# KirillKryukov/naf

Hardware: AMD Instinct MI355X
Metric: unnaf GB/s (uncompressed bases out) on 100 GB synthetic FASTA (higher is better)
Workload: dtype u8; 1 GPU; unnaf decode of a 100.0 GB synthetic-ACGT FASTA archive on one GPU (the size BASELINE.json's metric is quoted on; configs[1] at 10 GB rides along as cfg10_*), 100 records, 80-col lines; archive made in-run by the GPU ennaf; .naf 24739662224 B -> FASTA 99999995684 B, text + archive + decoded text resident in HBM; parallelism=one archive, one GPU, no data-path collective

## Files before the change

### naf_amd/csrc/ctx.h

```cpp
#pragma once
#include "common.h"
#include "../../include/naf_gpu.h"
#include <hip/hip_runtime.h>
#include <stdio.h>
#include <stdarg.h>
#include <vector>
#include <functional>
#include <string>

struct ArenaChunk { u8 *base; size_t cap, used; };

struct KTime { const char *name; hipEvent_t a, b; };

#define ZSPLIT_MAX 8
struct ZSplit { int parts; hipEvent_t ev[ZSPLIT_MAX]; u64 out_end[ZSPLIT_MAX]; int done; void *status; };
struct FlatStream { u64 q0, A; };
#define FLAT_DECODED (~0ull)
struct ZFlat { const u8 *src; const FlatStream *si; u64 nslots; const u8 *sym; void *status; bool ready;
               const u8 *tail; u64 tail_q; u32 tail_n;
               const u8 *cls; u32 n_decoded; u32 n_walk;
               struct naf_gpu_ctx *aux; hipEvent_t decoded_ev; void *later; };
struct CtxOpts { std::vector<std::pair<std::string, std::string>> kv; std::string trace; bool tracing = false; };
struct naf_gpu_ctx {
    int device = 0;
    CtxOpts *opts = nullptr;
    naf_gpu_ctx *root = nullptr;
    hipStream_t stream = nullptr;
    bool own_stream = false;
    std::vector<ArenaChunk> chunks;
    size_t high_water = 0;
    u8 *h_stage = nullptr;
    size_t h_stage_cap = 0;
    void *d_predef = nullptr;
    void *d_seqctab = nullptr;
    char err[512] = {0};
    bool timing = false;
    std::vector<KTime> ktimes;
    std::vector<hipEvent_t> ev_pool;
    size_t ev_used = 0;
    std::vector<std::string> agg_names; std::vector<float> agg_ms; std::vector<int> agg_n;
    float stream_ms[5] = { 0, 0, 0, 0, 0 };
    naf_gpu_ctx *side = nullptr;
    naf_gpu_ctx *side2 = nullptr;
    naf_gpu_ctx *side3 = nullptr;
    naf_gpu_ctx *side4 = nullptr;
    void *sides_thread = nullptr; int sides_rc = 0;
    hipEvent_t fork_ev = nullptr;
    struct ZSplit *zsplit = nullptr;
    hipEvent_t split_ev[ZSPLIT_MAX + 2] = {};
    struct ZFlat *zflat = nullptr;
    void *io_pool = nullptr;
    void *shard_state = nullptr;
    struct HostWorker *worker = nullptr;
};

void ctx_worker_start(naf_gpu_ctx *x, std::function<void()> job);
void ctx_worker_join(naf_gpu_ctx *x);
int  ctx_sides_ready(naf_gpu_ctx *c);

int  ctx_fail(naf_gpu_ctx *c, int code, const char *fmt, ...);
const char *ctx_opt(const naf_gpu_ctx *c, const char *name);
static inline bool ctx_opt_is(const naf_gpu_ctx *c, const char *name, char v) { const char *e = ctx_opt(c, name); return e && e[0] == v; }
bool ctx_tracing(const naf_gpu_ctx *c);
void ctx_trace(naf_gpu_ctx *c, const char *fmt, ...);
#define HIP_TRY(c, call) do { hipError_t e_ = (call); if (e_ != hipSuccess) return ctx_fail((c), NAF_GPU_EHIP, "%s: %s (%s:%d)", #call, hipGetErrorString(e_), __FILE__, __LINE__); } while (0)

void  arena_reset(naf_gpu_ctx *c);
void *arena_alloc(naf_gpu_ctx *c, size_t bytes);
void  arena_settle(naf_gpu_ctx *c);
template <typename T> T *arena_new(naf_gpu_ctx *c, size_t n) { return (T *)arena_alloc(c, n * sizeof(T)); }
static inline std::vector<size_t> arena_mark(const naf_gpu_ctx *c) { std::vector<size_t> m; for (auto &ch : c->chunks) m.push_back(ch.used); return m; }
static inline void arena_release(naf_gpu_ctx *c, const std::vector<size_t> &m) { for (size_t k = 0; k < c->chunks.size(); k++) c->chunks[k].used = k < m.size() ? m[k] : 0; }

int ctx_readback(naf_gpu_ctx *c, void *h_dst, const void *d_src, size_t bytes);
int ctx_readback2(naf_gpu_ctx *c, void *h1, const void *d1, size_t n1, void *h2, const void *d2, size_t n2);
int ctx_readbackv(naf_gpu_ctx *c, int n, void *const *h, const void *const *d, const size_t *bytes);

void ktime_begin(naf_gpu_ctx *c, const char *name);
void ktime_end(naf_gpu_ctx *c);

#define LAUNCH(c, name, kern, grid, block, shmem, ...) do { \
    ktime_begin((c), name); \
    hipLaunchKernelGGL(kern, dim3(grid), dim3(block), (shmem), (c)->stream, __VA_ARGS__); \
    ktime_end((c)); } while (0)

static inline u32 cdiv(u64 a, u64 b) { return (u32)((a + b - 1) / b); }

int scan_exclusive_u64(naf_gpu_ctx *c, u64 *d_vals, size_t n, u64 *d_total);
int scan_inclusive_max_i32(naf_gpu_ctx *c, i32 *d_vals, size_t n);
int scan_inclusive_max_i64(naf_gpu_ctx *c, i64 *d_vals, size_t n);
int scan_exclusive_u64_multi(naf_gpu_ctx *c, u64 *const *arrs, int k, size_t n, u64 *const *totals);
int scan_inclusive_max_i64_multi(naf_gpu_ctx *c, i64 *const *arrs, int k, size_t n);

int zstd_decode(naf_gpu_ctx *c, const u8 *d_src, size_t src_len, int has_magic, u8 *d_dst, size_t dst_cap, size_t *out_len, const u8 *head = nullptr);
int zstd_init_tables(naf_gpu_ctx *c);
void ennaf_shard_state_free(naf_gpu_ctx *c);
void io_pool_free(naf_gpu_ctx *c);
struct EmitP;
int zstd_decode_fused_fasta(naf_gpu_ctx *c, const u8 *d_src, size_t src_len, int has_magic, size_t *out_len, const EmitP *P, u8 *text);
struct ZRange { u64 want_lo, want_hi, got_lo, got_hi; bool ranged; u8 *own_buf; };
int zstd_decode_range(naf_gpu_ctx *c, const u8 *d_src, size_t src_len, int has_magic, u8 *d_dst, size_t dst_cap, size_t *out_len, ZRange *rg, const u8 *head = nullptr);
int zstd_split_status(naf_gpu_ctx *c, const ZSplit *sp);
int zstd_flat_later(naf_gpu_ctx *c, ZFlat *zf);
void zstd_flat_drop(ZFlat *zf);
int zstd_small_batch(naf_gpu_ctx *c, int n, const u8 *const *src, const size_t *len, u8 *const *dst, const size_t *cap, bool *ok);
bool zstd_small_fits(size_t len, size_t cap);
int zstd_small_launch(naf_gpu_ctx *c, int n, const u8 *const *src, const size_t *len, u8 *const *dst, const size_t *cap, u32 **d_res_out);
enum { ZENC_PART = 16, ZENC_PART_FIRST = 32, ZENC_PART_LAST = 64, ZENC_PREFER_RAW = 128, ZENC_PREFER_FLAT = 256, ZENC_SHORT_CODES = 512, ZENC_FRAME_TREE = 1024 };
int zenc_level_window(int level);
int zenc_repeat_probe(naf_gpu_ctx *c, const u8 *d_src, size_t n, u32 *share_1024);
static inline u32 zenc_probe_every(u64 n) { u32 e = 64; while (((n >> 20) / e) > 128) e <<= 1; return e; }
struct ZencPlace { u8 *(*fn)(void *ud, size_t frame_len); void *ud; };
struct ZencJob;
#define ZENC_LOC_BND 20
struct ZencLoc { const u8 *loc; const i32 *blk_bnd; const u32 *blk_t0; u64 tiles; };
int zstd_encode_begin(naf_gpu_ctx *c, const u8 *d_src, size_t n, int level, int with_magic, int lz, int block_log_hint, int window_log, ZencJob **job, const u8 *direct = nullptr, u32 nd = 0, const ZencLoc *dloc = nullptr);
int zstd_encode_finish(naf_gpu_ctx *c, ZencJob *job, u8 *d_dst, size_t cap, size_t *out_len, const ZencPlace *place);
void zstd_encode_drop(ZencJob *job);
int zstd_encode_size(naf_gpu_ctx *c, ZencJob *job, size_t *frame_len);
const u64 *zstd_encode_total_ptr(const ZencJob *job);
void zstd_encode_set_total(ZencJob *job, u64 total);
int zstd_encode(naf_gpu_ctx *c, const u8 *d_src, size_t n, int level, u8 *d_dst, size_t cap, size_t *out_len, int with_magic, int lz = 0, int block_log_hint = 0, int window_log = 0, const ZencPlace *place = nullptr);
```

### naf_amd/csrc/emit.hip

```cpp
#include "ctx.h"
#include "wgscan.h"
#include "emit_core.h"
#include <thread>

__device__ __forceinline__ void st_text16(u8 *p, const uint4 &v, int nt)
{
    if (nt) {
        typedef unsigned int u32x4_t __attribute__((ext_vector_type(4)));
        u32x4_t nv; nv.x = v.x; nv.y = v.y; nv.z = v.z; nv.w = v.w;
        __builtin_nontemporal_store(nv, (u32x4_t *)p);
    } else *(uint4 *)p = v;
}

__global__ void k_len_flags(const u32 *units, u64 n, u64 *flag)
{
    u64 i = (u64)blockIdx.x * blockDim.x + threadIdx.x;
    if (i < n) flag[i] = units[i] != 0xFFFFFFFFu;
}
__global__ void k_len_acc(const u32 *units, u64 n, const u64 *ridx, u64 *rec_len, u64 N)
{
    u64 i = (u64)blockIdx.x * blockDim.x + threadIdx.x;
    if (i < n && ridx[i] < N) atomicAdd((unsigned long long *)&rec_len[ridx[i]], (unsigned long long)units[i]);
}

// ... 407 lines not shown
            if (FOURBIT) { const u8 *s = P.seq + (k.g0 >> 1); a = ld64(s); b = s[8]; }
            else { a = ld64(P.seq + k.g0); b = ld64(P.seq + k.g0 + 8); }
        }
    };
    auto finish = [&](const Chunk &k, u64 a, u64 b) {
        if (!k.live) return;
        u8 *o = out + (k.p0 - P.out_begin);
        if (k.qual_copy) { uint4 v; v.x = (u32)a; v.y = (u32)(a >> 32); v.z = (u32)b; v.w = (u32)(b >> 32); memcpy(o, &v, 16); return; }
        if (k.fast) {
            u64 lo, hi, g0 = k.g0;
            if (FOURBIT) { u64 nib = a; if (g0 & 1) nib = (nib >> 4) | (b << 60); expand16(P.lut, nib, lo, hi); }
            else {
                lo = a; hi = b;
                if (P.upper) {
                    auto up = [](u64 v) { u64 r = 0; for (int i = 0; i < 8; i++) { u32 c = (v >> (8 * i)) & 0xFF; if (c >= 'a' && c <= 'z') c -= 32; r |= (u64)c << (8 * i); } return r; };
                    lo = up(lo); hi = up(hi);
                }
            }
            if (any_toggle) {
                u64 kk = upper_bound_u64(P.toggles, klo, khi, g0);
                u32 state = (u32)(kk & 1), m16 = 0; u64 pos = g0;
                for (;;) {
                    u64 nxt = kk < khi ? P.toggles[kk] : ~0ull;
                    u64 end = nxt < g0 + 16 ? nxt : g0 + 16;
                    if (state && end > pos) m16 |= (u32)(((1u << (end - pos)) - 1) << (pos - g0));
                    if (nxt >= g0 + 16) break;
                    pos = nxt; state ^= 1; kk++;
                }
                lo += spread_bits8(m16 & 0xFF); hi += spread_bits8(m16 >> 8);
            } else if (P.masking && (klo & 1)) { lo += 0x2020202020202020ull; hi += 0x2020202020202020ull; }
            if (k.nl_b < 16) splice_newline(lo, hi, k.nl_b);
            u64 j15 = k.j0 + 15 - (15 > k.nl_b ? 1 : 0);
            if (j15 >= k.len) hi = (hi & 0x00FFFFFFFFFFFFFFull) | ((u64)'\n' << 56);
            uint4 v; v.x = (u32)lo; v.y = (u32)(lo >> 32); v.z = (u32)hi; v.w = (u32)(hi >> 32);
            memcpy(o, &v, 16);
            return;
        }
        for (u32 bb = 0; bb < k.nbytes; bb++) o[bb] = (u8)emit_byte<FOURBIT>(P, k.p0 + bb, rlo, rhi, klo, khi);
    };
    for (u64 tile = span_first; tile <= span_last; tile += 8192) {
        Chunk ka = prep(tile), kb = prep(tile + 4096);
        u64 a0, a1, b0, b1;
        fetch(ka, a0, a1); fetch(kb, b0, b1);
        finish(ka, a0, a1); finish(kb, b0, b1);
    }
}

#define ES_SPAN (32u * 1024u)
#define ES_CAP 1024

__device__ __forceinline__ void place16(u64 &lo, u64 &hi, u64 slo, u64 shi, u32 pos, u32 n)
{
    if (n <= 8) { shi = 0; slo &= low_bytes_mask((int)n); } else if (n < 16) shi &= low_bytes_mask((int)n - 8);
    if (pos == 0) { lo |= slo; hi |= shi; }
    else if (pos < 8) { lo |= slo << (8 * pos); hi |= (shi << (8 * pos)) | (slo >> (64 - 8 * pos)); }
    else if (pos == 8) hi |= slo;
    else hi |= slo << (8 * (pos - 8));
}

__device__ __forceinline__ void mask16_from(const u64 *tog, u32 n, u64 klo, u64 g0, u64 &lo, u64 &hi)
{
    u32 a = 0, b = n;
    while (a < b) { u32 mid = (a + b) >> 1; if (tog[mid] <= g0) a = mid + 1; else b = mid; }
    u32 kk = a, state = (u32)((klo + kk) & 1), m16 = 0; u64 pos = g0;
    for (;;) {
        u64 nxt = kk < n ? tog[kk] : ~0ull;
        u64 end = nxt < g0 + 16 ? nxt : g0 + 16;
        if (state && end > pos) m16 |= (u32)(((1u << (end - pos)) - 1) << (pos - g0));
        if (nxt >= g0 + 16) break;
        pos = nxt; state ^= 1; kk++;
    }
    lo += spread_bits8(m16 & 0xFF); hi += spread_bits8(m16 >> 8);
}
__device__ __forceinline__ void mask16(const EmitP &P, u64 klo, u64 khi, bool any_toggle, u64 g0, u64 &lo, u64 &hi)
{
    if (any_toggle) {
        if (khi - klo <= 0x7FFFFFFFull) mask16_from(P.toggles + klo, (u32)(khi - klo), klo, g0, lo, hi);
        else {
            u64 kk = upper_bound_u64(P.toggles, klo, khi, g0);
            u32 state = (u32)(kk & 1), m16 = 0; u64 pos = g0;
            for (;;) {
                u64 nxt = kk < khi ? P.toggles[kk] : ~0ull;
                u64 end = nxt < g0 + 16 ? nxt : g0 + 16;
                if (state && end > pos) m16 |= (u32)(((1u << (end - pos)) - 1) << (pos - g0));
                if (nxt >= g0 + 16) break;
                pos = nxt; state ^= 1; kk++;
            }
            lo += spread_bits8(m16 & 0xFF); hi += spread_bits8(m16 >> 8);
        }
    } else if (P.masking && (klo & 1)) { lo += 0x2020202020202020ull; hi += 0x2020202020202020ull; }
}

__device__ __forceinline__ void span_windows(const EmitP &P, u64 span_first, u64 span_last, u64 *sh)
{
    if (threadIdx.x < 2 && P.mode != EM_SEQ) {
        u64 p = threadIdx.x == 0 ? span_first : span_last;
        sh[threadIdx.x] = upper_bound_u64(P.rec_out, 0, P.N + 1, p) - 1;
    }
    __syncthreads();
    if (threadIdx.x < 2) {
        u64 k = 0;
        if (P.masking) {
            u64 g;
            if (P.mode == EM_SEQ) g = threadIdx.x == 0 ? span_first : span_last + 1;
            else g = threadIdx.x == 0 ? P.rec_base[sh[0]] : P.rec_base[sh[1] + 1];
            if (P.mode != EM_SEQ && threadIdx.x == 0) {
                u64 r = sh[0], off = span_first - P.rec_out[r], hl = P.hdr_len[r];
                if (off > hl) { u64 q = off - hl; u64 j = (P.mode == EM_FASTA && P.L) ? (q / (P.L + 1)) * P.L : (P.mode == EM_FASTQ ? 0 : q); if (j > P.rec_len[r]) j = P.rec_len[r]; g += j; }
            }
            k = upper_bound_u64(P.toggles, 0, P.n_toggles, g);
        }
        sh[2 + threadIdx.x] = k;
    }
    __syncthreads();
}

__global__ void k_hdr_len64(const u32 *hdr_len, u64 r0, u64 n, u64 *out)
{
    u64 i = (u64)blockIdx.x * blockDim.x + threadIdx.x;
    if (i < n) out[i] = hdr_len[r0 + i];
}
__device__ __forceinline__ void store_upto16(u8 *p, u64 lo, u64 hi, u32 n)
{
    if (n >= 16) { uint4 v; v.x = (u32)lo; v.y = (u32)(lo >> 32); v.z = (u32)hi; v.w = (u32)(hi >> 32); memcpy(p, &v, 16); return; }
    if (n & 8) { st64(p, lo); p += 8; lo = hi; }
    if (n & 4) { st32(p, (u32)lo); p += 4; lo >>= 32; }
    if (n & 2) { p[0] = (u8)lo; p[1] = (u8)(lo >> 8); p += 2; lo >>= 16; }
    if (n & 1) p[0] = (u8)lo;
}
template <u32 LANES = 16>
__device__ __forceinline__ void group_copy(u8 *dst, const u8 *src, u64 n, u32 g)
{
    for (u64 i = (u64)g * 16; i < n; i += LANES * 16) {
        u64 lo = ld64(src + i), hi = ld64(src + i + 8);
        store_upto16(dst + i, lo, hi, n - i < 16 ? (u32)(n - i) : 16u);
    }
}

__global__ __launch_bounds__(256) void k_hdr_build(EmitP P, u64 r0, u64 n, const u64 *hdr_off, u8 *text)
{
    u64 i = (u64)blockIdx.x * 32 + (threadIdx.x >> 3);
    u32 g = threadIdx.x & 7;
    if (i >= n) return;
    u64 r = r0 + i; u32 hl = P.hdr_len[r];
    u8 *o = text + hdr_off[i];
    u64 ids0 = 0, idl = 0, nm0 = 0, nml = 0;
    if (P.has_ids) { ids0 = r ? P.idz[r - 1] + 1 : 0; idl = P.idz[r] - ids0; }
    if (P.has_names) { nm0 = r ? P.nmz[r - 1] + 1 : 0; nml = P.nmz[r] - nm0; }
    if (g == 0) { o[0] = P.hdr_char; o[hl - 1] = '\n'; }
    if (P.has_ids) {
        group_copy<8>(o + 1, P.ids + ids0, idl, g);
        if (P.has_names && nml) { if (g == 0) o[1 + idl] = P.sep; group_copy<8>(o + 2 + idl, P.names + nm0, nml, g); }
    } else group_copy<8>(o + 1, P.names + nm0, nml, g);
}

template <bool FOURBIT, typename Geo>
__device__ __forceinline__ void compose_chunk(const EmitP &P, Geo &geo, u64 p0, u32 nbytes, u64 r, u64 klo, u64 khi, bool any_toggle, u32 Lp1_32, u8 *o)
{
    const bool hdrs = P.hdr_text != nullptr;
    u64 ro, rn, len, base, ho; u32 hl;
    geo(r, ro, rn, len, base, ho, hl);
    u64 lo = 0, hi = 0; u32 pos = 0;
    while (pos < nbytes) {
        u64 p = p0 + pos;
        while (p >= rn) { r++; geo(r, ro, rn, len, base, ho, hl); }
        u64 off = p - ro;
        const u8 *src = nullptr; u64 g = 0; bool is_bases = false;
        u64 n_main = 0; u32 tc = 0, n_tc = 0;
        if (off < hl) { src = P.hdr_text + ho + off; n_main = hl - off; }
        else {
            u64 q = off - hl;
            if (P.mode == EM_FASTQ) {
                if (q < len + 3) {
                    u64 skip = 0;
                    if (q < len) { is_bases = true; g = base + q; n_main = len - q; } else skip = q - len;
                    tc = 0x0A2B0Au >> (8 * (u32)skip); n_tc = 3 - (u32)skip;
                } else { src = P.qual + base + (q - len - 3); n_main = 2 * len + 3 - q; tc = '\n'; n_tc = 1; }
            } else {
                tc = '\n'; n_tc = 1;
                if (P.mode == EM_SEQUENCES || P.L == 0) { if (q < len) { is_bases = true; g = base + q; n_main = len - q; } }
                else {
                    u64 line, col;
                    if (Lp1_32 && (q >> 32) == 0) { u32 l32 = (u32)q / Lp1_32; line = l32; col = (u32)q - l32 * Lp1_32; }
                    else { line = q / (P.L + 1); col = q - line * (P.L + 1); }
                    u64 j = line * P.L + col;
                    if (col != P.L && j < len) { is_bases = true; g = base + j; n_main = len - j < P.L - col ? len - j : P.L - col; }
                }
            }
        }
        u32 rem = nbytes - pos;
        u32 n1 = n_main < rem ? (u32)n_main : rem;
        if (n1) {
            u64 slo, shi;
            if (is_bases) { bases16<FOURBIT>(P, g, slo, shi); if (P.mode != EM_FASTQ) mask16(P, klo, khi, any_toggle, g, slo, shi); }
            else if (!hdrs && off < hl) {
                slo = shi = 0;
                for (u32 b = 0; b < n1; b++) { u64 ch = header_char(P, r, off + b, hl); if (b < 8) slo |= ch << (8 * b); else shi |= ch << (8 * (b - 8)); }
            }
            else { slo = ld64(src); shi = n1 > 8 ? ld64(src + 8) : 0; }
            place16(lo, hi, slo, shi, pos, n1);
            pos += n1; rem -= n1;
        }
        if (n1 == n_main && rem && n_tc) { u32 n2 = n_tc < rem ? n_tc : rem; place16(lo, hi, tc, 0, pos, n2); pos += n2; }
    }
    if (nbytes == 16) { uint4 v; v.x = (u32)lo; v.y = (u32)(lo >> 32); v.z = (u32)hi; v.w = (u32)(hi >> 32); memcpy(o, &v, 16); }
    else for (u32 b = 0; b < nbytes; b++) o[b] = (u8)((b < 8 ? lo >> (8 * b) : hi >> (8 * (b - 8))) & 0xFF);
}

struct GeoGlobal {
    const EmitP &P;
    __device__ GeoGlobal(const EmitP &p) : P(p) {}
    __device__ __forceinline__ void operator()(u64 r, u64 &ro, u64 &rn, u64 &len, u64 &base, u64 &ho, u32 &hl) const
    { ro = P.rec_out[r]; rn = P.rec_out[r + 1]; len = P.rec_len[r]; base = P.rec_base[r]; hl = P.hdr_len[r]; ho = P.hdr_text ? P.hdr_off[r - P.hdr_r0] : 0; }
};

template <bool FOURBIT>
__global__ __launch_bounds__(256) void k_emit_short(EmitP P, u8 *out)
{
    __shared__ u64 sh[4];
    __shared__ u64 s_ro[ES_CAP + 1], s_len[ES_CAP], s_base[ES_CAP], s_ho[ES_CAP];
    __shared__ u32 s_hl[ES_CAP];
    u64 span_first = P.out_begin + (u64)blockIdx.x * ES_SPAN, span_last = span_first + ES_SPAN - 1;
    if (span_last >= P.out_end) span_last = P.out_end - 1;
    span_windows(P, span_first, span_last, sh);
    const u64 rlo = sh[0], rhi = sh[1], klo = sh[2], khi = sh[3];
    const bool any_toggle = P.masking && klo < khi;
    const u64 nrec = rhi - rlo + 1;
    const bool in_lds = nrec <= ES_CAP;
    const bool hdrs = P.hdr_text != nullptr;
    if (in_lds) {
        for (u32 i = threadIdx.x; i < (u32)nrec; i += 256) {
            u64 r = rlo + i; s_ro[i] = P.rec_out[r]; s_len[i] = P.rec_len[r]; s_base[i] = P.rec_base[r]; s_hl[i] = P.hdr_len[r];
            s_ho[i] = hdrs ? P.hdr_off[r - P.hdr_r0] : 0;
        }
        if (threadIdx.x == 0) s_ro[nrec] = P.rec_out[rhi + 1];
        __syncthreads();
    }
    const u32 Lp1_32 = (P.L + 1) >> 32 ? 0 : (u32)(P.L + 1);
    auto geo_lds = [&](u64 r, u64 &ro, u64 &rn, u64 &len, u64 &base, u64 &ho, u32 &hl) {
        u32 i = (u32)(r - rlo); ro = s_ro[i]; rn = s_ro[i + 1]; len = s_len[i]; base = s_base[i]; hl = s_hl[i]; ho = s_ho[i];
    };
    GeoGlobal geo_g(P);
    for (u64 tile = span_first; tile <= span_last; tile += 4096) {
        u64 p0 = tile + (u64)threadIdx.x * 16;
        if (p0 > span_last) continue;
        u32 nbytes = P.out_end - p0 < 16 ? (u32)(P.out_end - p0) : 16;
        u8 *o = out + (p0 - P.out_begin);
        if (in_lds) {
            u32 lo_ = 0, hi_ = (u32)nrec; while (lo_ < hi_) { u32 mid = (lo_ + hi_) >> 1; if (s_ro[mid] <= p0) lo_ = mid + 1; else hi_ = mid; }
            compose_chunk<FOURBIT>(P, geo_lds, p0, nbytes, rlo + lo_ - 1, klo, khi, any_toggle, Lp1_32, o);
        } else {
            u64 r = upper_bound_u64(P.rec_out, rlo, rhi + 1, p0) - 1;
            compose_chunk<FOURBIT>(P, geo_g, p0, nbytes, r, klo, khi, any_toggle, Lp1_32, o);
        }
    }
}

#define ER_STAGE 24576u
template <bool FOURBIT, u32 ER_LANES, u32 WGT>
__global__ __launch_bounds__(WGT) void k_emit_fastq_records(EmitP P, u8 *out)
{
    constexpr u32 ER_READS = WGT / ER_LANES, STAGE = ER_STAGE / (256u / WGT);
    __shared__ __attribute__((aligned(16))) u8 stage[STAGE + 32];
    const u32 g = threadIdx.x & (ER_LANES - 1);
    const u64 r0 = (u64)blockIdx.x * ER_READS, r = r0 + threadIdx.x / ER_LANES;
    const u64 rend = r0 + ER_READS < P.N ? r0 + ER_READS : P.N;
    const u64 wbase = P.rec_out[r0], wspan = P.rec_out[rend] - wbase;
    const bool in_lds = wspan <= STAGE;
    if (r < P.N) {
        const u64 len = P.rec_len[r], base = P.rec_base[r];
        const u32 hl = P.hdr_len[r];
        u8 *o = in_lds ? stage + (P.rec_out[r] - wbase) : out + P.rec_out[r];
        u64 ids0 = 0, idl = 0, nm0 = 0, nml = 0;
        if (P.has_ids) { ids0 = r ? P.idz[r - 1] + 1 : 0; idl = P.idz[r] - ids0; }
        if (P.has_names) { nm0 = r ? P.nmz[r - 1] + 1 : 0; nml = P.nmz[r] - nm0; }
        if (g == 0) { o[0] = P.hdr_char; o[hl - 1] = '\n'; }
        if (P.has_ids) {
            group_copy<ER_LANES>(o + 1, P.ids + ids0, idl, g);
            if (P.has_names && nml) { if (g == 0) o[1 + idl] = P.sep; group_copy<ER_LANES>(o + 2 + idl, P.names + nm0, nml, g); }
        } else group_copy<ER_LANES>(o + 1, P.names + nm0, nml, g);
        u8 *os = o + hl;
        for (u64 i = (u64)g * 16; i < len; i += 16 * ER_LANES) {
            u64 lo, hi; bases16<FOURBIT>(P, base + i, lo, hi);
            store_upto16(os + i, lo, hi, len - i < 16 ? (u32)(len - i) : 16u);
        }
        if (g == 0) { os[len] = '\n'; os[len + 1] = '+'; os[len + 2] = '\n'; os[2 * len + 3] = '\n'; }
        group_copy<ER_LANES>(os + len + 3, P.qual + base, len, g);
    }
    if (!in_lds) return;
    __syncthreads();
    u8 *dst = out + wbase; const u32 n = (u32)wspan;
    u32 head = (u32)((16 - ((uintptr_t)dst & 15)) & 15); if (head > n) head = n;
    if (threadIdx.x < head) dst[threadIdx.x] = stage[threadIdx.x];
    u32 words = (n - head) >> 4;
    for (u32 w = threadIdx.x; w < words; w += WGT) {
        u64 a, b2; __builtin_memcpy(&a, stage + head + 16 * w, 8); __builtin_memcpy(&b2, stage + head + 16 * w + 8, 8);
        uint4 v; v.x = (u32)a; v.y = (u32)(a >> 32); v.z = (u32)b2; v.w = (u32)(b2 >> 32);
        st_text16(dst + head + 16 * w, v, P.nt_store);
    }
    for (u32 k = head + 16 * words + threadIdx.x; k < n; k += WGT) dst[k] = stage[k];
}

#define EMIT_TOG_LDS 256u
struct TileIdx { u64 gline, k, khi; u32 col, fast; };
#define TI_HDR 0xFFFFFFFFu
struct TileFlat { u64 q0, A, q1, A1, q2, qf; };
struct TileFlatE { u64 base, a1_addr; u32 a1_sh, K0, K1, d1, d2, qoff, par0, pad; };
static_assert(sizeof(TileFlatE) == sizeof(TileFlat), "the derived record replaces the raw one in place");
#define FLAT_QM 4096
#define TILE_WG 255
__global__ __launch_bounds__(256) void k_tile_index(EmitP P, u64 ntiles, TileIdx *ti, u64 *tr, u32 *list, u32 *count, TileFlat *tsig, u32 spare, u32 *list2)
{
    __shared__ u64 s_k[256], s_r[256];
    const u64 t = (u64)blockIdx.x * TILE_WG + threadIdx.x;
    const u64 p = P.out_begin + t * 4096;
    TileIdx x; x.fast = 0; x.gline = 0; x.khi = 0; x.k = P.n_toggles; x.col = TI_HDR;
    TileFlat f; f.q0 = f.A = f.q1 = f.A1 = f.q2 = f.qf = 0;
    u64 r = ~0ull; u32 cbits = 1;
    const bool inside = t < ntiles && p < P.out_end;
    if (inside) {
        u64 g;
        if (P.mode == EM_SEQ) { r = 0; x.col = 0; g = p; x.gline = p; }
        else {
            r = upper_bound_u64(P.rec_out, 0, P.N + 1, p) - 1;
            u64 off = p - P.rec_out[r], hl = P.hdr_len[r], len = P.rec_len[r], j = 0;
            if (off >= hl) {
                u64 q = off - hl;
                if (P.mode == EM_FASTA && P.L) {
                    u64 line = q / (P.L + 1), col = q - line * (P.L + 1);
                    j = line * P.L + (col < P.L ? col : P.L);
                    if (P.L < 0xFFFFFFF0ull) { x.gline = P.rec_base[r] + line * P.L; x.col = (u32)col; }
                } else if (P.mode != EM_FASTQ) { j = q; x.col = 0; x.gline = P.rec_base[r] + q; }
                if (j > len) j = len;
            }
            g = P.rec_base[r] + j;
        }
        x.k = P.masking ? upper_bound_u64(P.toggles, 0, P.n_toggles, g) : 0;
        if (tsig) {
            const FlatStream *si = (const FlatStream *)P.fsi;
            const u64 q = g >> 1;
            u64 lo, hi, gs = q >> 13; if (gs >= P.fslots) gs = P.fslots - 1;
            if (si[gs].q0 <= q) { lo = gs; hi = gs + 1; u64 st = 1; while (hi < P.fslots && si[hi].q0 <= q) { lo = hi; st <<= 1; hi = lo + st; } if (hi > P.fslots) hi = P.fslots; }
            else { hi = gs; u64 st = 1; lo = gs - 1; while (lo > 0 && si[lo].q0 > q) { hi = lo; st <<= 1; lo = lo > st ? lo - st : 0; } }
            while (hi - lo > 1) { const u64 mid = (lo + hi) >> 1; if (si[mid].q0 <= q) lo = mid; else hi = mid; }
            f.q0 = si[lo].q0; f.A = si[lo].A; f.qf = q;
            if (P.fcls) {
                u32 c = 3; u64 b = lo >> 2; const u64 nb = P.fslots >> 2, qe = q + 2048 + 16;
                for (u32 k = 0; k < 6 && b < nb && si[4 * b].q0 <= qe; k++, b++) c &= P.fcls[b];
                if (b < nb && si[4 * b].q0 <= qe) c = 0;
                cbits = c;
            }
            u64 cs = lo + 1;
            while (cs < P.fslots && si[cs + 1].q0 == si[cs].q0) cs++;
            f.q1 = si[cs].q0; f.A1 = cs < P.fslots ? si[cs].A : 0;
            u64 ce = cs < P.fslots ? cs + 1 : cs;
            while (ce < P.fslots && si[ce + 1].q0 == si[ce].q0) ce++;
            f.q2 = si[ce].q0;
        }
    }
    s_k[threadIdx.x] = x.k; s_r[threadIdx.x] = r;
    __syncthreads();
    if (threadIdx.x == TILE_WG) return;
    TileFlatE e; e.base = (u64)P.fsrc; e.a1_addr = (u64)P.fsrc; e.a1_sh = 4; e.K0 = e.K1 = 0; e.d1 = e.d2 = 0x7FFFFFFFu; e.qoff = 0; e.par0 = 0; e.pad = 0;
    if (t >= ntiles) {
        if (t == ntiles) { tr[t] = ~0ull; ti[t] = x; if (tsig && spare) *(TileFlatE *)&tsig[t] = e; }
        else if (tsig && t < ntiles + spare) { ti[t].fast = 0; *(TileFlatE *)&tsig[t] = e; }
        return;
    }
    tr[t] = r;
    if (!inside) { ti[t] = x; if (tsig) *(TileFlatE *)&tsig[t] = e; list[atomicAdd(count, 1u)] = (u32)t; return; }
    const u64 r_next = s_r[threadIdx.x + 1];
    x.khi = s_k[threadIdx.x + 1];
    const bool wrap = P.mode == EM_FASTA && P.L != 0;
    bool fast = x.col != TI_HDR && r == r_next && P.out_begin + (t + 1) * 4096 <= P.out_end && !P.force_slow && (!wrap || P.L >= 16);
    bool packed = false;
    if (tsig) {
        packed = fast && (cbits & 2);
        if (fast && !(cbits & 1)) fast = false;
        if (fast) {
            fast = f.qf + 2048 + 16 < f.q2 || f.q2 == f.q1;
            if (P.ftail && f.qf + 2048 + 16 >= P.ftail_q) fast = false;
            if (f.q2 != f.q1 && (f.A1 > f.A ? f.A1 - f.A : f.A - f.A1) >= (1ull << 29)) fast = false;
        }
        if (fast) {
            const u64 gline = x.gline;
            const u64 dd1 = f.q1 - f.qf, dd2 = f.q2 - f.qf;
            e.d1 = dd1 > 0x7FFFFFFFull ? 0x7FFFFFFFu : (u32)dd1; e.d2 = dd2 > 0x7FFFFFFFull ? 0x7FFFFFFFu : (u32)dd2;
            const u64 T0 = f.A - 4 * (f.qf - f.q0), T1 = f.A1 + 4 * (u64)e.d1;
            const bool two = f.q2 != f.q1;
            const u64 tmin = two && T1 < T0 ? T1 : T0;
            const u64 ub = (tmin - 40 - 4 * (u64)FLAT_QM) & ~7ull;
            e.base = (u64)P.fsrc + (u64)((i64)ub >> 3);
            e.K0 = (u32)(T0 - 40 - ub); e.K1 = two ? (u32)(T1 - 40 - ub) : e.K0;
            e.qoff = (u32)((gline >> 1) - f.qf); e.par0 = (u32)gline & 1u;
            const u64 t1 = (f.A1 < 40 ? 40 : f.A1) - 40;
            e.a1_addr = (u64)P.fsrc + (t1 >> 3); e.a1_sh = (u32)(t1 & 7) + 4;
        }
        *(TileFlatE *)&tsig[t] = e;
    }
    x.fast = fast ? 1u : (packed ? 2u : 0u);
    ti[t] = x;
    if (!fast) { if (packed) list2[atomicAdd(count + 1, 1u)] = (u32)t; else list[atomicAdd(count, 1u)] = (u32)t; }
}

template <bool FOURBIT>
__device__ __forceinline__ void emit_tile_body(const EmitP &P, const TileIdx &a, u8 *out_tile)
{
    __shared__ u64 s_tog[EMIT_TOG_LDS];
    const u32 ntog = (u32)(a.khi - a.k < EMIT_TOG_LDS ? a.khi - a.k : EMIT_TOG_LDS);
    const bool use_tog = P.masking && a.k < a.khi && a.khi - a.k <= EMIT_TOG_LDS;
    if (use_tog) { for (u32 i = threadIdx.x; i < ntog; i += 256) s_tog[i] = P.toggles[a.k + i]; __syncthreads(); }
    const u32 lane16 = threadIdx.x * 16;
    u64 g0; u32 nl_b = 64;
    if (P.mode == EM_FASTA && P.L != 0) {
        const u32 Lp1 = (u32)P.L + 1;
        u32 c = a.col + lane16, dl;
        if (Lp1 < 32768) dl = __umulhi(c, P.Ldiv_magic); else dl = c >= Lp1 ? 1u : 0u;
        u32 col = c - dl * Lp1;
        g0 = a.gline + (u64)dl * (u32)P.L + col;
        u32 d = (u32)P.L - col;
        nl_b = d < 16 ? d : 64;
    } else g0 = a.gline + lane16;
    u64 lo, hi;
    if (FOURBIT) {
        u64 addr = (u64)P.seq + (g0 >> 1);
        const uint4 q = ldg_at<uint4>(addr & ~7ull);
        u64 q0 = (u64)q.x | ((u64)q.y << 32), q1 = (u64)q.z | ((u64)q.w << 32);
        u32 sh = (u32)(addr & 7) * 8 + (u32)(g0 & 1) * 4;
        expand16(P.lut, sh ? (q0 >> sh) | (q1 << (64 - sh)) : q0, lo, hi);
    } else bases16<false>(P, g0, lo, hi);
    if (use_tog) mask16_from(s_tog, ntog, a.k, g0, lo, hi);
    else mask16(P, a.k, a.khi, P.masking && a.k < a.khi, g0, lo, hi);
    if (nl_b < 16) splice_newline(lo, hi, (int)nl_b);
    uint4 v; v.x = (u32)lo; v.y = (u32)(lo >> 32); v.z = (u32)hi; v.w = (u32)(hi >> 32);
    st_text16(out_tile + lane16, v, P.nt_store);
}
template <bool FOURBIT>
__global__ __launch_bounds__(256) void k_emit_tile(EmitP P, const TileIdx *ti, u8 *out)
{
    const TileIdx a = ti[blockIdx.x];
    if (a.fast != 1) return;
    emit_tile_body<FOURBIT>(P, a, out + (u64)blockIdx.x * 4096);
}
template <bool FOURBIT, u32 TW>
__device__ __forceinline__ void emit_tiles_wave(const EmitP &P, const TileIdx *ti, u8 *out, const u64 (&tn)[TW], u32 want, u64 (*s_tog)[EMIT_TOG_LDS])
{
    const u32 lane = threadIdx.x;
    TileIdx A[TW]; bool live[TW];
#pragma unroll
    for (u32 j = 0; j < TW; j++) { A[j] = ti[tn[j] == ~0ull ? 0 : tn[j]]; live[j] = tn[j] != ~0ull && A[j].fast == want; }
    u64 g0s[TW][4]; u32 nls[TW][4]; uint4 Q[TW][4];
#pragma unroll
    for (u32 j = 0; j < TW; j++) {
        const TileIdx &a = A[j];
#pragma unroll
        for (u32 r = 0; r < 4; r++) {
            const u32 lane16 = (r * 64 + lane) * 16;
            u64 g0; u32 nl_b = 64;
            if (P.mode == EM_FASTA && P.L != 0) {
                const u32 Lp1 = (u32)P.L + 1;
                u32 c = a.col + lane16, dl;
                if (Lp1 < 32768) dl = __umulhi(c, P.Ldiv_magic); else dl = c >= Lp1 ? 1u : 0u;
                u32 col = c - dl * Lp1;
                g0 = a.gline + (u64)dl * (u32)P.L + col;
                u32 d = (u32)P.L - col;
                nl_b = d < 16 ? d : 64;
            } else g0 = a.gline + lane16;
            g0s[j][r] = g0; nls[j][r] = nl_b;
            if (FOURBIT) Q[j][r] = live[j] ? ldg_at<uint4>(((u64)P.seq + (g0 >> 1)) & ~7ull) : make_uint4(0, 0, 0, 0);
        }
    }
    if (P.masking) {
#pragma unroll
        for (u32 j = 0; j < TW; j++) {
            const u64 nt = A[j].khi - A[j].k;
            for (u32 i = lane; i < EMIT_TOG_LDS; i += 64) s_tog[j][i] = (live[j] && i < nt && nt <= EMIT_TOG_LDS) ? P.toggles[A[j].k + i] : 0ull;
        }
        __syncthreads();
    }
#pragma unroll
    for (u32 j = 0; j < TW; j++) {
        if (!live[j]) continue;
        const TileIdx &a = A[j];
        const u32 ntog = (u32)(a.khi - a.k < EMIT_TOG_LDS ? a.khi - a.k : EMIT_TOG_LDS);
        const bool use_tog = P.masking && a.k < a.khi && a.khi - a.k <= EMIT_TOG_LDS;
#pragma unroll
        for (u32 r = 0; r < 4; r++) {
            const u64 g0 = g0s[j][r];
            u64 lo, hi;
            if (FOURBIT) {
                const u64 addr = (u64)P.seq + (g0 >> 1);
                const uint4 q = Q[j][r];
                const u64 q0 = (u64)q.x | ((u64)q.y << 32), q1 = (u64)q.z | ((u64)q.w << 32);
                const u32 sh = (u32)(addr & 7) * 8 + (u32)(g0 & 1) * 4;
                expand16(P.lut, sh ? (q0 >> sh) | (q1 << (64 - sh)) : q0, lo, hi);
            } else bases16<false>(P, g0, lo, hi);
            if (use_tog) mask16_from(s_tog[j], ntog, a.k, g0, lo, hi);
            else mask16(P, a.k, a.khi, P.masking && a.k < a.khi, g0, lo, hi);
            if (nls[j][r] < 16) splice_newline(lo, hi, (int)nls[j][r]);
            uint4 v; v.x = (u32)lo; v.y = (u32)(lo >> 32); v.z = (u32)hi; v.w = (u32)(hi >> 32);
            st_text16(out + tn[j] * 4096 + (r * 64 + lane) * 16, v, P.nt_store);
        }
    }
}
template <bool FOURBIT, u32 TW>
__global__ __launch_bounds__(64) void k_emit_tile_wave(EmitP P, const TileIdx *ti, u8 *out, u64 ntiles)
{
    __shared__ u64 s_tog[TW][EMIT_TOG_LDS];
    u64 tn[TW];
#pragma unroll
    for (u32 j = 0; j < TW; j++) { const u64 t = (u64)blockIdx.x * TW + j; tn[j] = t < ntiles ? t : ~0ull; }
    emit_tiles_wave<FOURBIT, TW>(P, ti, out, tn, 1u, s_tog);
}
template <bool FOURBIT>
__global__ __launch_bounds__(64) void k_emit_tile_list_wave(EmitP P, const TileIdx *ti, const u32 *list, const u32 *count, u8 *out)
{
    __shared__ u64 s_tog[1][EMIT_TOG_LDS];
    const u32 n = *count;
    for (u32 i = blockIdx.x; i < n; i += gridDim.x) {
        const u64 tn[1] = { list[i] };
        emit_tiles_wave<FOURBIT, 1>(P, ti, out, tn, 2u, s_tog);
        __syncthreads();
    }
}
template <bool FOURBIT>
__global__ __launch_bounds__(256) void k_emit_tile_list(EmitP P, const TileIdx *ti, const u32 *list, const u32 *count, u8 *out)
{
    const u32 n = *count;
    for (u32 i = blockIdx.x; i < n; i += gridDim.x) {
        const u32 t = list[i];
        const TileIdx a = ti[t];
        emit_tile_body<FOURBIT>(P, a, out + (u64)t * 4096);
        __syncthreads();
    }
}

__global__ void k_flat_pair(EmitP P, u32 *pair)
{
    const u32 t = threadIdx.x;
    {
        const u32 pa = P.fsym[t >> 4], pb = P.fsym[t & 15];
        pair[16 + t] = expand_codes4(P.lut, (pa & 15u) | ((pa >> 4) << 8) | ((pb & 15u) << 16) | ((pb >> 4) << 24));
        if (t < 16) {
            const u32 d = t; u32 sel[4], orv[4];
            for (u32 i = 0; i < 4; i++) {
                sel[i] = 0; orv[i] = 0;
                for (u32 j = 0; j < 4; j++) { const u32 q = 4 * i + j; sel[i] |= (q < d ? 4 + j : (q == d ? 0x0Cu : 3 + j)) << (8 * j); if (q == d) orv[i] |= 0x0Au << (8 * j); }
            }
            for (u32 i = 0; i < 4; i++) { pair[272 + 8 * d + i] = sel[i]; pair[272 + 8 * d + 4 + i] = orv[i]; }
        }
    }
    if (t >= 12) return;
    const u8 *lut = (const u8 *)P.lut;
    u32 v = 0;
    for (u32 k = 0; k < 4; k++) {
        const u32 pk = P.fsym[4 * (t & 3) + k];
        const u32 b = t < 4 ? pk : (t < 8 ? lut[pk & 15] : lut[pk >> 4]);
        v |= b << (8 * k);
    }
    pair[t] = v;
}
#define FLAT_TPW 8
template <u32 TPW>
__global__ __launch_bounds__(256) void k_emit_tile_flat(EmitP P, const TileIdx *ti, const TileFlat *tsig, u8 *out, u64 ntiles, u32 xcd_chunk)
{
    u32 wg = blockIdx.x;
    if (xcd_chunk) { wg = (blockIdx.x & 7u) * xcd_chunk + (blockIdx.x >> 3); if ((u64)wg * TPW >= ntiles) return; }
    __shared__ u64 s_tog[TPW][EMIT_TOG_LDS];
    __shared__ uint4 s_spl[32];
    if (threadIdx.x < 16) {
        const u32 d = threadIdx.x; u32 sel[4], orv[4];
        for (u32 i = 0; i < 4; i++) {
            sel[i] = 0; orv[i] = 0;
            for (u32 j = 0; j < 4; j++) { const u32 p = 4 * i + j; sel[i] |= (p < d ? 4 + j : (p == d ? 0x0Cu : 3 + j)) << (8 * j); if (p == d) orv[i] |= 0x0Au << (8 * j); }
        }
        s_spl[2 * d] = make_uint4(sel[0], sel[1], sel[2], sel[3]); s_spl[2 * d + 1] = make_uint4(orv[0], orv[1], orv[2], orv[3]);
    }
    __shared__ u32 s_pair[256];
    {
        const u32 pa = P.fsym[threadIdx.x >> 4], pb = P.fsym[threadIdx.x & 15];
        s_pair[threadIdx.x] = expand_codes4(P.lut, (pa & 15u) | ((pa >> 4) << 8) | ((pb & 15u) << 16) | ((pb >> 4) << 24));
    }
    const u32 lane16 = threadIdx.x * 16;
    TileIdx A[TPW]; TileFlatE F[TPW]; bool live[TPW];
    {
        static_assert(sizeof(TileIdx) == 32 && sizeof(TileFlatE) == 48, "records are read as 16-byte words");
        const u64 t0 = (u64)wg * TPW;
        const uint4 *pa = (const uint4 *)(ti + t0), *pf = (const uint4 *)(tsig + t0);
        uint4 ra[2 * TPW], rf[3 * TPW];
#pragma unroll
        for (u32 i = 0; i < 2 * TPW; i++) ra[i] = pa[i];
#pragma unroll
        for (u32 i = 0; i < 3 * TPW; i++) rf[i] = pf[i];
#pragma unroll
        for (u32 j = 0; j < TPW; j++) {
            __builtin_memcpy(&A[j], &ra[2 * j], 32); __builtin_memcpy(&F[j], &rf[3 * j], 48);
            live[j] = t0 + j < ntiles && A[j].fast == 1;
        }
    }
    u64 X[TPW]; u32 offs[TPW], grels[TPW], nls[TPW], haves[TPW];
#pragma unroll
    for (u32 j = 0; j < TPW; j++) {
        const TileIdx &a = A[j]; const TileFlatE &e = F[j];
        u32 grel, nl_b = 64;
        if (P.mode == EM_FASTA && P.L != 0) {
            const u32 Lp1 = (u32)P.L + 1;
            u32 c = a.col + lane16, dl;
            if (Lp1 < 32768) dl = __umulhi(c, P.Ldiv_magic); else dl = c >= Lp1 ? 1u : 0u;
            u32 col = c - dl * Lp1;
            grel = dl * (u32)P.L + col;
            u32 d = (u32)P.L - col;
            nl_b = d < 16 ? d : 64;
        } else grel = lane16;
        grels[j] = grel; nls[j] = nl_b;
        const u32 par = e.par0 + grel;
        const u32 need = 8 + (par & 1u);
        const u32 qrel = (par >> 1) + e.qoff;
        const bool second = qrel >= e.d1;
        const u32 qm = live[j] ? ~0u : 0u;
        const u32 off = (second ? e.K1 : e.K0) - ((4 * qrel) & qm);
        const u32 rem = (second ? e.d2 : e.d1) - qrel;
        X[j] = ldg_at_unaligned<u64>(e.base + (off >> 3));
        offs[j] = off;
        haves[j] = need > rem ? rem : 16u;
    }
    if (P.masking) {
        u64 tg[TPW];
#pragma unroll
        for (u32 j = 0; j < TPW; j++) {
            const u64 nt = A[j].khi - A[j].k;
            tg[j] = (live[j] && threadIdx.x < nt && nt <= EMIT_TOG_LDS) ? P.toggles[A[j].k + threadIdx.x] : 0ull;
        }
#pragma unroll
        for (u32 j = 0; j < TPW; j++) s_tog[j][threadIdx.x] = tg[j];
    }
    __syncthreads();
#pragma unroll
    for (u32 j = 0; j < TPW; j++) {
        const u64 t = (u64)wg * TPW + j;
        if (!live[j]) continue;
        const TileIdx &a = A[j];
        const u64 g0 = a.gline + grels[j];
        u64 h36 = X[j] >> ((offs[j] & 7) + 4);
        if (haves[j] < 9) {
            const u64 y = ldg_at_unaligned<u64>(F[j].a1_addr);
            const u64 n36 = (y >> F[j].a1_sh) & 0xFFFFFFFFFull;
            const u32 keep = 4 * haves[j];
            h36 = (h36 & ~(0xFFFFFFFFFull >> keep)) | (n36 >> keep);
        }
        const u32 h = (u32)(h36 >> 4), n9 = (u32)h36 & 15u;
        u64 lo, hi;
        {
            u32 w0 = s_pair[h >> 24], w1 = s_pair[(h >> 16) & 0xFFu], w2 = s_pair[(h >> 8) & 0xFFu], w3 = s_pair[h & 0xFFu];
            if (g0 & 1) {
                const u32 c9 = s_pair[n9 << 4];
                w0 = __builtin_amdgcn_alignbyte(w1, w0, 1); w1 = __builtin_amdgcn_alignbyte(w2, w1, 1);
                w2 = __builtin_amdgcn_alignbyte(w3, w2, 1); w3 = __builtin_amdgcn_alignbyte(c9, w3, 1);
            }
            lo = (u64)w0 | ((u64)w1 << 32); hi = (u64)w2 | ((u64)w3 << 32);
        }
        const u32 ntog = (u32)(a.khi - a.k < EMIT_TOG_LDS ? a.khi - a.k : EMIT_TOG_LDS);
        const bool use_tog = P.masking && a.k < a.khi && a.khi - a.k <= EMIT_TOG_LDS;
        if (use_tog) mask16_from(s_tog[j], ntog, a.k, g0, lo, hi);
        else mask16(P, a.k, a.khi, P.masking && a.k < a.khi, g0, lo, hi);
        uint4 v; v.x = (u32)lo; v.y = (u32)(lo >> 32); v.z = (u32)hi; v.w = (u32)(hi >> 32);
        if (nls[j] < 16) {
            const uint4 sel = s_spl[2 * nls[j]], orv = s_spl[2 * nls[j] + 1];
            const u32 x0 = v.x, x1 = v.y, x2 = v.z, x3 = v.w;
            v.x = __builtin_amdgcn_perm(x0, 0u, sel.x) | orv.x; v.y = __builtin_amdgcn_perm(x1, x0, sel.y) | orv.y;
            v.z = __builtin_amdgcn_perm(x2, x1, sel.z) | orv.z; v.w = __builtin_amdgcn_perm(x3, x2, sel.w) | orv.w;
        }
        st_text16(out + t * 4096 + lane16, v, P.nt_store);
    }
}

template <u32 TW>
__global__ __launch_bounds__(64) void k_emit_tile_flat_wave(EmitP P, const TileIdx *ti, const TileFlat *tsig, u8 *out, u64 ntiles, u32 xcd_chunk)
{
    u32 wg = blockIdx.x;
    if (xcd_chunk) { wg = (blockIdx.x & 7u) * xcd_chunk + (blockIdx.x >> 3); if ((u64)wg * TW >= ntiles) return; }
    __shared__ u64 s_tog[TW][EMIT_TOG_LDS];
    __shared__ uint4 s_spl[32];
    __shared__ u32 s_pair[256];
    const u32 lane = threadIdx.x;
    if (lane < 32) s_spl[lane] = ((const uint4 *)(P.fpair + 272))[lane];
    ((uint4 *)s_pair)[lane] = ((const uint4 *)(P.fpair + 16))[lane];
    TileIdx A[TW]; TileFlatE F[TW]; bool live[TW];
    {
        const u64 t0 = (u64)wg * TW;
        const uint4 *pa = (const uint4 *)(ti + t0), *pf = (const uint4 *)(tsig + t0);
        uint4 ra[2 * TW], rf[3 * TW];
#pragma unroll
        for (u32 i = 0; i < 2 * TW; i++) ra[i] = pa[i];
#pragma unroll
        for (u32 i = 0; i < 3 * TW; i++) rf[i] = pf[i];
#pragma unroll
        for (u32 j = 0; j < TW; j++) {
            __builtin_memcpy(&A[j], &ra[2 * j], 32); __builtin_memcpy(&F[j], &rf[3 * j], 48);
            live[j] = t0 + j < ntiles && A[j].fast == 1;
        }
    }
    u64 X[TW][4]; u32 grels[TW][4], pk[TW][4];
#pragma unroll
    for (u32 j = 0; j < TW; j++) {
        const TileIdx &a = A[j]; const TileFlatE &e = F[j];
#pragma unroll
        for (u32 r = 0; r < 4; r++) {
            const u32 lane16 = (r * 64 + lane) * 16;
            u32 grel, nl_b = 64;
            if (P.mode == EM_FASTA && P.L != 0) {
                const u32 Lp1 = (u32)P.L + 1;
                u32 c = a.col + lane16, dl;
                if (Lp1 < 32768) dl = __umulhi(c, P.Ldiv_magic); else dl = c >= Lp1 ? 1u : 0u;
                u32 col = c - dl * Lp1;
                grel = dl * (u32)P.L + col;
                u32 d = (u32)P.L - col;
                nl_b = d < 16 ? d : 64;
            } else grel = lane16;
            grels[j][r] = grel;
            const u32 par = e.par0 + grel;
            const u32 need = 8 + (par & 1u);
            const u32 qrel = (par >> 1) + e.qoff;
            const bool second = qrel >= e.d1;
            const u32 qm = live[j] ? ~0u : 0u;
            const u32 off = (second ? e.K1 : e.K0) - ((4 * qrel) & qm);
            const u32 rem = (second ? e.d2 : e.d1) - qrel;
            X[j][r] = ldg_at_unaligned<u64>(e.base + (off >> 3));
            pk[j][r] = nl_b | ((need > rem ? rem : 16u) << 8) | ((off & 7u) << 16);
        }
    }
    if (P.masking) {
#pragma unroll
        for (u32 j = 0; j < TW; j++) {
            const u64 nt = A[j].khi - A[j].k;
            for (u32 i = lane; i < EMIT_TOG_LDS; i += 64) s_tog[j][i] = (live[j] && i < nt && nt <= EMIT_TOG_LDS) ? P.toggles[A[j].k + i] : 0ull;
        }
    }
    __syncthreads();
#pragma unroll
    for (u32 j = 0; j < TW; j++) {
        const u64 t = (u64)wg * TW + j;
        if (!live[j]) continue;
        const TileIdx &a = A[j];
        const u32 ntog = (u32)(a.khi - a.k < EMIT_TOG_LDS ? a.khi - a.k : EMIT_TOG_LDS);
        const bool use_tog = P.masking && a.k < a.khi && a.khi - a.k <= EMIT_TOG_LDS;
#pragma unroll
        for (u32 r = 0; r < 4; r++) {
            const u64 g0 = a.gline + grels[j][r];
            const u32 nl = pk[j][r] & 0xFFu, have = (pk[j][r] >> 8) & 0xFFu;
            u64 h36 = X[j][r] >> ((pk[j][r] >> 16) + 4);
            if (have < 9) {
                const u64 y = ldg_at_unaligned<u64>(F[j].a1_addr);
                const u64 n36 = (y >> F[j].a1_sh) & 0xFFFFFFFFFull;
                const u32 keep = 4 * have;
                h36 = (h36 & ~(0xFFFFFFFFFull >> keep)) | (n36 >> keep);
            }
            const u32 h = (u32)(h36 >> 4), n9 = (u32)h36 & 15u;
            u64 lo, hi;
            {
                u32 w0 = s_pair[h >> 24], w1 = s_pair[(h >> 16) & 0xFFu], w2 = s_pair[(h >> 8) & 0xFFu], w3 = s_pair[h & 0xFFu];
                if (g0 & 1) {
                    const u32 c9 = s_pair[n9 << 4];
                    w0 = __builtin_amdgcn_alignbyte(w1, w0, 1); w1 = __builtin_amdgcn_alignbyte(w2, w1, 1);
                    w2 = __builtin_amdgcn_alignbyte(w3, w2, 1); w3 = __builtin_amdgcn_alignbyte(c9, w3, 1);
                }
                lo = (u64)w0 | ((u64)w1 << 32); hi = (u64)w2 | ((u64)w3 << 32);
            }
            if (use_tog) mask16_from(s_tog[j], ntog, a.k, g0, lo, hi);
            else mask16(P, a.k, a.khi, P.masking && a.k < a.khi, g0, lo, hi);
            uint4 v; v.x = (u32)lo; v.y = (u32)(lo >> 32); v.z = (u32)hi; v.w = (u32)(hi >> 32);
            if (nl < 16) {
                const uint4 sel = s_spl[2 * nl], orv = s_spl[2 * nl + 1];
                const u32 x0 = v.x, x1 = v.y, x2 = v.z, x3 = v.w;
                v.x = __builtin_amdgcn_perm(x0, 0u, sel.x) | orv.x; v.y = __builtin_amdgcn_perm(x1, x0, sel.y) | orv.y;
                v.z = __builtin_amdgcn_perm(x2, x1, sel.z) | orv.z; v.w = __builtin_amdgcn_perm(x3, x2, sel.w) | orv.w;
            }
            st_text16(out + t * 4096 + (r * 64 + lane) * 16, v, P.nt_store);
        }
    }
}

template <bool FOURBIT>
__device__ __forceinline__ void emit_rest_tile(const EmitP &P, const TileIdx *ti, const u64 *tr, u64 t, u8 *out, u32 chunk)
{
    const TileIdx a = ti[t];
    u64 p0 = P.out_begin + t * 4096 + chunk * 16;
    if (p0 >= P.out_end) return;
    u32 nbytes = P.out_end - p0 < 16 ? (u32)(P.out_end - p0) : 16;
    const u32 Lp1_32 = (P.L + 1) >> 32 ? 0 : (u32)(P.L + 1);
    u8 *o = out + (p0 - P.out_begin);
    if (P.mode == EM_SEQ) {
        for (u32 bb = 0; bb < nbytes; bb++) o[bb] = (u8)emit_byte<FOURBIT>(P, p0 + bb, 0, 0, a.k, a.khi);
        return;
    }
    u64 rlo = tr[t], rhi = tr[t + 1] == ~0ull ? P.N - 1 : tr[t + 1];
    u64 r = upper_bound_u64(P.rec_out, rlo, rhi + 1, p0) - 1;
    GeoGlobal geo_g(P);
    compose_chunk<FOURBIT>(P, geo_g, p0, nbytes, r, a.k, a.khi, P.masking && a.k < a.khi, Lp1_32, o);
}
#define EMIT_REST_GRID 4096
template <bool FOURBIT>
__global__ __launch_bounds__(64) void k_emit_rest(EmitP P, const TileIdx *ti, const u64 *tr, const u32 *list, const u32 *count, u8 *out)
{
    const u32 n = *count;
    for (u32 i = blockIdx.x; i < 4 * n; i += gridDim.x) emit_rest_tile<FOURBIT>(P, ti, tr, list[i >> 2], out, (i & 3) * 64 + threadIdx.x);
}

__global__ void k_range_bases(EmitP P, u64 *out2)
{
    if (threadIdx.x || blockIdx.x) return;
    if (P.mode == EM_SEQ) { out2[0] = P.out_begin; out2[1] = P.out_end; out2[2] = out2[3] = 0; return; }
    u64 pb = P.out_begin, pe = P.out_end - 1;
    u64 r0 = upper_bound_u64(P.rec_out, 0, P.N + 1, pb) - 1, r1 = upper_bound_u64(P.rec_out, 0, P.N + 1, pe) - 1;
    out2[2] = r0; out2[3] = r1;
    auto lower = [&](u64 r, u64 p) -> u64 {
        u64 off = p - P.rec_out[r], hl = P.hdr_len[r], len = P.rec_len[r];
        if (off <= hl) return 0;
        u64 q = off - hl, j;
        if (P.mode == EM_FASTQ) j = 0;
        else if (P.mode == EM_FASTA && P.L) j = (q / (P.L + 1)) * P.L;
        else j = q;
        return j > len ? len : j;
    };
    auto upper = [&](u64 r, u64 p) -> u64 {
        u64 off = p - P.rec_out[r], hl = P.hdr_len[r], len = P.rec_len[r];
        if (off < hl) return 0;
        u64 q = off - hl, j;
        if (P.mode == EM_FASTQ) j = len;
        else if (P.mode == EM_FASTA && P.L) j = (q / (P.L + 1) + 1) * P.L;
        else j = q + 1;
        return j > len ? len : j;
    };
    out2[0] = P.rec_base[r0] + lower(r0, pb);
    out2[1] = P.rec_base[r1] + upper(r1, pe);
}

__global__ void k_last_nonempty(const u64 *rec_len, u64 N, unsigned long long *out)
{
    u64 r = (u64)blockIdx.x * blockDim.x + threadIdx.x;
    if (r < N && rec_len[r]) atomicMax(out, (unsigned long long)(r + 1));
}
template <bool FOURBIT>
__global__ void k_emit_surplus(EmitP P, u64 base0, u64 S, u64 cc, u64 L, int wrap, u64 lo, u64 hi, u8 *out)
{
    const u64 j = lo + (u64)blockIdx.x * blockDim.x + threadIdx.x;
    if (j >= hi) return;
    u64 g; bool nl = false;
    if (!wrap || L == 0 || S <= cc) g = base0 + j;
    else if (j < cc) g = base0 + j;
    else if (j == cc) { nl = true; g = 0; }
    else { const u64 j2 = j - cc - 1, line = j2 / (L + 1), col = j2 - line * (L + 1); if (col == L) { nl = true; g = 0; } else g = base0 + cc + line * L + col; }
    u32 ch = '\n';
    if (!nl) { ch = base_char<FOURBIT>(P, g); if (P.masking && base_masked(P, g, 0, P.n_toggles)) ch += 32; }
    out[j - lo] = (u8)ch;
}

static int zero_positions(naf_gpu_ctx *c, const u8 *d_buf, u64 n, u64 N, u64 **out, bool names)
{
    u64 *pos = arena_new<u64>(c, N + 1);
    if (!pos) return NAF_GPU_ENOMEM;
    u64 tiles = (n + ZT_TILE - 1) / ZT_TILE;
    u64 *cnt = arena_new<u64>(c, tiles + 2);
    if (!cnt) return NAF_GPU_ENOMEM;
    u64 *d_total = cnt + tiles + 1;
    if (tiles) LAUNCH(c, "unnaf_zero_count", k_zero_count, tiles, 256, 0, d_buf, n, cnt);
    int rc = scan_exclusive_u64(c, cnt, tiles, d_total); if (rc) return rc;
    u64 total = 0;
    rc = ctx_readback(c, &total, d_total, 8); if (rc) return rc;
    if (total < N) return ctx_fail(c, NAF_GPU_EFORMAT, names ? "corrupted names - can't read name %llu\n" : "currupted ids - can't read id %llu\n", (unsigned long long)total);
    if (tiles) LAUNCH(c, "unnaf_zero_scatter", k_zero_scatter, tiles, 256, 0, d_buf, n, (const u64 *)cnt, pos, N);
    *out = pos;
    return 0;
}

enum { H_OK = 0, H_EMPTY, H_TRUNC, H_MAGIC, H_VERSION, H_SEQTYPE, H_SEPARATOR, H_VLE_LEAD, H_VLE_OVERFLOW, H_SANE_SECTION , H_SANE_COUNT = H_SANE_SECTION + 6 };
struct ContainerOut { naf_gpu_header h; int code; u8 frame_head[6][24]; };
NAF_HD int naf_parse_container(const u8 *p, size_t len, naf_gpu_header *h)
{
    size_t pos = 0;
    memset(h, 0, sizeof *h);
    if (len == 0) return H_EMPTY;
    if (len < 3) return H_TRUNC;
    if (p[0] != 0x01 || p[1] != 0xF9 || p[2] != 0xEC) return H_MAGIC;
    pos = 3;
    if (pos >= len) return H_TRUNC;
    h->version = p[pos++];
    if (h->version < 1 || h->version > 2) return H_VERSION;
    h->seq_type = NAF_SEQ_DNA;
    if (h->version > 1) {
        if (pos >= len) return H_TRUNC;
        int t = p[pos++];
        h->seq_type = t;
        if (t < 1 || t > 3) return H_SEQTYPE;
    }
    if (len - pos < 2) return H_TRUNC;
    h->flags = p[pos++]; h->separator = p[pos++];
    if (h->separator < 0x20 || h->separator > 0x7E) return H_SEPARATOR;
    int e = 0;
    auto rd = [&](u64 *v) -> int {
        u64 a = 0; if (pos >= len) return H_TRUNC;
        u8 ch = p[pos++];
        if (ch == 128) return H_VLE_LEAD;
        while (ch & 128) { if (a & (127ull << 57)) return H_VLE_OVERFLOW; a = (a << 7) | (ch & 127); if (pos >= len) return H_TRUNC; ch = p[pos++]; }
        if (a & (127ull << 57)) return H_VLE_OVERFLOW;
        *v = (a << 7) | ch; return 0;
    };
    if ((e = rd(&h->line_length)) || (e = rd(&h->n_sequences))) return e;
    if (h->flags & 0x40) { if ((e = rd(&h->title_len))) return e; h->title_off = pos; if (h->title_len > len - pos) return H_TRUNC; pos += h->title_len; }
    const int bit[6] = { 0x20, 0x10, 0x08, 0x04, 0x02, 0x01 };
    for (int i = 0; i < 6; i++) {
        if (!(h->flags & bit[i])) continue;
        if ((e = rd(&h->orig_size[i])) || (e = rd(&h->comp_size[i]))) return e;
        if (h->comp_size[i] > len - pos) return H_TRUNC;
        h->payload_off[i] = pos; pos += h->comp_size[i];
    }
    for (int i = 0; i < 6; i++) {
        const u64 cs = h->comp_size[i] + 4;
        const u64 lim = cs > (1ull << 46) ? ~0ull : cs << (i == 4 ? 17 : 16);
        if (h->orig_size[i] > lim) return H_SANE_SECTION + i;
    }
    if (h->n_sequences > ((u64)len << 16)) return H_SANE_COUNT;
    return H_OK;
}
static void container_error_text(int code, const naf_gpu_header *h, char *buf, size_t cap)
{
    static const char *what[6] = { "can't decompress ids\n", "can't decompress names\n", "can't decompress lengths\n", "can't decompress mask\n",
                                   "can't decompress sequence\n", "can't decompress quality\n" };
    switch (code) {
    case H_EMPTY: snprintf(buf, cap, "empty input"); break;
    case H_TRUNC: snprintf(buf, cap, "incomplete or truncated input\n"); break;
    case H_MAGIC: snprintf(buf, cap, "not a NAF format\n"); break;
    case H_VERSION: snprintf(buf, cap, "unknown version (%d) of NAF format\n", h->version); break;
    case H_SEQTYPE: snprintf(buf, cap, "unknown sequence type (%d) found in NAF file\n", h->seq_type); break;
    case H_SEPARATOR: snprintf(buf, cap, "unsupported name separator character\n"); break;
    case H_VLE_LEAD: snprintf(buf, cap, "invalid input: error parsing variable length encoded number\n"); break;
    case H_VLE_OVERFLOW: snprintf(buf, cap, "invalid input: overflow reading a variable length encoded number\n"); break;
    case H_SANE_COUNT: snprintf(buf, cap, "corrupted header: more sequences than the archive can describe\n"); break;
    default: if (code >= H_SANE_SECTION && code < H_SANE_SECTION + 6) snprintf(buf, cap, "%s", what[code - H_SANE_SECTION]); else snprintf(buf, cap, "malformed NAF header\n");
    }
}

extern "C" int naf_gpu_parse_header_host(const void *h_naf, size_t len, naf_gpu_header *h, char errbuf[128])
{
    if (!h) return NAF_GPU_EARG;
    const int code = naf_parse_container((const u8 *)h_naf, len, h);
    if (!code) return 0;
    if (errbuf) container_error_text(code, h, errbuf, 128);
    return NAF_GPU_EFORMAT;
}

__global__ void k_parse_container(const u8 *d, u64 len, ContainerOut *out)
{
    if (threadIdx.x || blockIdx.x) return;
    out->code = naf_parse_container(d, (size_t)len, &out->h);
    for (int i = 0; i < 6; i++) {
        const u64 n = out->code ? 0 : (out->h.comp_size[i] < 24 ? out->h.comp_size[i] : 24);
        for (u64 k = 0; k < 24; k++) out->frame_head[i][k] = k < n ? d[out->h.payload_off[i] + k] : 0;
    }
}

static int parse_container_device(naf_gpu_ctx *c, const void *d_naf, size_t len, ContainerOut *co)
{
    ContainerOut *d_co = arena_new<ContainerOut>(c, 1); if (!d_co) return NAF_GPU_ENOMEM;
    LAUNCH(c, "unnaf_parse_container", k_parse_container, 1, 64, 0, (const u8 *)d_naf, (u64)len, d_co);
    int rc = ctx_readback(c, co, d_co, sizeof *co); if (rc) return rc;
    if (co->code) { char buf[160]; container_error_text(co->code, &co->h, buf, sizeof buf); return ctx_fail(c, NAF_GPU_EFORMAT, "%s", buf); }
    return 0;
}

extern "C" int naf_gpu_parse_header(naf_gpu_ctx *c, const void *d_naf, size_t len, naf_gpu_header *h)
{
    if (!c || !h) return NAF_GPU_EARG;
    arena_reset(c);
    ContainerOut co;
    int rc = parse_container_device(c, d_naf, len, &co);
    *h = co.h;
    return rc;
}

enum { S_IDS = 0, S_NAMES, S_LEN, S_MASK, S_SEQ, S_QUAL };

struct UnnafPlan {
    naf_gpu_header h; u8 frame_head[6][24]; EmitP P; u64 total; bool fourbit; bool empty;
    u64 seq_bytes; bool need_qual;
    u64 main_total, surplus, sur_c, sur_base0;
};

static int load_section(naf_gpu_ctx *c, const u8 *d_naf, const naf_gpu_header &h, int i, u64 expect, const char *what, u8 **out, const u8 *head = nullptr)
{
    u8 *buf = (u8 *)arena_alloc(c, expect + 32);
    if (!buf) return NAF_GPU_ENOMEM;
    size_t n = 0;
    int rc = zstd_decode(c, d_naf + h.payload_off[i], h.comp_size[i], 0, buf, expect, &n, head);
    if (rc == NAF_GPU_ECAP || (rc == 0 && n != expect)) return ctx_fail(c, NAF_GPU_EFORMAT, "can't decompress %s\n", what);
    if (rc) return rc;
    *out = buf;
    return 0;
}

static int unnaf_prepare(naf_gpu_ctx *c, const u8 *d_naf, size_t naf_len, const naf_gpu_unnaf_opts *o, UnnafPlan &pl)
{
    ContainerOut co;
    int rc = parse_container_device(c, d_naf, naf_len, &co); if (rc) return rc;
    pl.h = co.h; memcpy(pl.frame_head, co.frame_head, sizeof pl.frame_head);
    const naf_gpu_header &h = pl.h;
    EmitP &P = pl.P; memset(&P, 0, sizeof P);
    int has_mask = (h.flags >> 2) & 1, has_data = (h.flags >> 1) & 1, has_qual = h.flags & 1;
    int mode = o->out_type == NAF_OUT_DEFAULT ? (has_qual ? NAF_OUT_FASTQ : NAF_OUT_FASTA) : o->out_type;
    pl.empty = false; pl.total = 0; pl.need_qual = false; pl.main_total = pl.surplus = pl.sur_c = pl.sur_base0 = 0;
    pl.fourbit = h.seq_type <= NAF_SEQ_RNA;
    u64 N = h.n_sequences, T = h.orig_size[S_SEQ];
    pl.seq_bytes = pl.fourbit ? (T + 1) / 2 : T;
    if (N == 0 || !has_data) { pl.empty = true; return 0; }
    if (mode == NAF_OUT_FASTQ && !has_qual) return ctx_fail(c, NAF_GPU_EFORMAT, "FASTQ output requested, but input has no qualities\n");
    if (mode == NAF_OUT_4BIT) {
        if (!pl.fourbit) return ctx_fail(c, NAF_GPU_EFORMAT, "input has no 4-bit encoded data, but %s sequences\n", h.seq_type == NAF_SEQ_PROTEIN ? "protein" : "text");
        P.mode = -1; pl.total = pl.main_total = pl.seq_bytes; return 0;
    }
    P.mode = mode == NAF_OUT_FASTA ? EM_FASTA : mode == NAF_OUT_FASTQ ? EM_FASTQ : mode == NAF_OUT_SEQ ? EM_SEQ : EM_SEQUENCES;
    P.N = N; P.T = T;
    P.L = o->line_length >= 0 ? (u64)o->line_length : h.line_length;
    P.sep = h.separator; P.hdr_char = P.mode == EM_FASTQ ? '@' : '>';
    P.masking = o->use_mask && has_mask && P.mode != EM_FASTQ && pl.fourbit;
    P.upper = !pl.fourbit && !o->use_mask;
    const char *tab = h.seq_type == NAF_SEQ_RNA ? "-UGKCYSBAWRDMHVN" : "-TGKCYSBAWRDMHVN";
    memcpy(P.lut, tab, 16);
    for (u32 k = 0; k < 16; k++) ((u8 *)P.lutc)[k] = (u8)tab[((k & 1) << 3) | ((k & 2) << 1) | ((k & 4) >> 1) | (k >> 3)];
    const char *fs = ctx_opt(c, "FORCE_SLOW"); P.force_slow = fs && fs[0] == '1';
    P.nt_store = 1;
    pl.need_qual = P.mode == EM_FASTQ;

    return 0;
}

template <typename Hook>
static int unnaf_sections_main(naf_gpu_ctx *c, const u8 *d_naf, UnnafPlan &pl, naf_gpu_ctx *aux, Hook early, bool early_has_work, naf_gpu_ctx *aux_names)
{
    const naf_gpu_header &h = pl.h;
    EmitP &P = pl.P;
    int has_ids = (h.flags >> 5) & 1, has_names = (h.flags >> 4) & 1, has_len = (h.flags >> 3) & 1;
    u64 N = h.n_sequences, T = h.orig_size[S_SEQ];
    int rc;
    if (P.mode == EM_SEQ) {
        pl.total = pl.main_total = T;
    } else {
        if (!has_len) return ctx_fail(c, NAF_GPU_EFORMAT, "archive has no lengths");
        P.has_ids = 0; P.has_names = 0;
        const bool want_names = P.mode == EM_FASTA || P.mode == EM_FASTQ;
        if (want_names) { P.has_ids = has_ids; P.has_names = has_names; }
        u8 *pre[3] = { nullptr, nullptr, nullptr };
        auto small3 = [&](naf_gpu_ctx *x) -> int {
            const int sec[3] = { S_IDS, S_NAMES, S_LEN }; const bool wanted[3] = { want_names && has_ids != 0, want_names && has_names != 0, true };
            const u8 *src[3]; size_t len[3], cap[3]; u8 *dst[3]; bool ok[3]; int idx[3], m = 0;
            for (int k = 0; k < 3; k++) {
                if (!wanted[k] || h.orig_size[sec[k]] == 0) continue;
                u8 *b = (u8 *)arena_alloc(x, h.orig_size[sec[k]] + 32); if (!b) return NAF_GPU_ENOMEM;
                src[m] = d_naf + h.payload_off[sec[k]]; len[m] = h.comp_size[sec[k]]; dst[m] = b; cap[m] = h.orig_size[sec[k]]; idx[m++] = k;
            }
            if (!m) return 0;
            int r = zstd_small_batch(x, m, src, len, dst, cap, ok); if (r) return r;
            for (int q = 0; q < m; q++) if (ok[q]) pre[idx[q]] = dst[q];
            return 0;
        };
        auto ids_names = [&](naf_gpu_ctx *x, int which = 3) -> int {
            int r;
            if ((which & 1) && want_names && has_ids) {
                u8 *b = pre[0]; u64 *z = nullptr;
                if (h.orig_size[S_IDS] == 0) return ctx_fail(x, NAF_GPU_EFORMAT, "corrupted ids - not 0-terminated\n");
                if (!b && (r = load_section(x, d_naf, h, S_IDS, h.orig_size[S_IDS], "ids", &b, pl.frame_head[S_IDS]))) return r;
                if ((r = zero_positions(x, b, h.orig_size[S_IDS], N, &z, false))) return r;
                P.ids = b; P.idz = z;
            }
            if ((which & 2) && want_names && has_names) {
                u8 *b = pre[1]; u64 *z = nullptr;
                if (h.orig_size[S_NAMES] == 0) return ctx_fail(x, NAF_GPU_EFORMAT, "corrupted names - not 0-terminated\n");
                if (!b && (r = load_section(x, d_naf, h, S_NAMES, h.orig_size[S_NAMES], "names", &b, pl.frame_head[S_NAMES]))) return r;
                if ((r = zero_positions(x, b, h.orig_size[S_NAMES], N, &z, true))) return r;
                P.names = b; P.nmz = z;
            }
            return 0;
        };
        u64 *rec_len = nullptr;
// ... 37 lines not shown
                    J.res = d_res; J.n_jobs = (u32)m;
                    J.ids = buf[0]; J.ids_n = h.orig_size[S_IDS]; J.names = buf[1]; J.names_n = h.orig_size[S_NAMES];
                    J.lens = (const u32 *)buf[2]; J.n_len = h.orig_size[S_LEN] / 4;
                    J.N = N; J.L = P.L; J.has_ids = P.has_ids; J.has_names = P.has_names; J.mode = P.mode;
                    J.idz = P.has_ids ? arena_new<u64>(x, N + 1) : nullptr; J.nmz = P.has_names ? arena_new<u64>(x, N + 1) : nullptr;
                    J.rec_len = arena_new<u64>(x, N + 1); J.hdr_len = arena_new<u32>(x, N + 1);
                    J.rec_out = arena_new<u64>(x, N + 2); J.rec_base = arena_new<u64>(x, N + 2); J.status = arena_new<u64>(x, 8);
                    if ((P.has_ids && !J.idz) || (P.has_names && !J.nmz) || !J.rec_len || !J.hdr_len || !J.rec_out || !J.rec_base || !J.status) return NAF_GPU_ENOMEM;
                    LAUNCH(x, "unnaf_side_tables", k_side_tables, 1, 256, 0, J);
                    if ((r = ctx_readback(x, st, J.status, sizeof st))) return r;
                    if (st[0] != 1) return 0;
                    P.ids = buf[0]; P.idz = J.idz; P.names = buf[1]; P.nmz = J.nmz;
                    P.rec_len = J.rec_len; P.hdr_len = J.hdr_len; P.rec_out = J.rec_out; P.rec_base = J.rec_base;
                    fused_done = true;
                    return 0;
                };
                int rf = 0;
                if (aux) { ctx_worker_start(aux, [&] { rf = fused(aux); }); early(); ctx_worker_join(aux); if (rf) memcpy(c->err, aux->err, sizeof c->err); }
                else rf = fused(c);
                if (rf) return rf;
                if (fused_done) {
                    if (st[3] < N) return ctx_fail(c, NAF_GPU_EFORMAT, "corrupted lengths: %llu records described, %llu expected", (unsigned long long)st[3], (unsigned long long)N);
                    if (P.has_ids && st[1] < N) return ctx_fail(c, NAF_GPU_EFORMAT, "currupted ids - can't read id %llu\n", (unsigned long long)st[1]);
                    if (P.has_names && st[2] < N) return ctx_fail(c, NAF_GPU_EFORMAT, "corrupted names - can't read name %llu\n", (unsigned long long)st[2]);
                    tot[0] = st[4]; tot[1] = st[5];
                }
            }
        }
        if (fused_done) rec_len = (u64 *)P.rec_len;
        else {
        const bool aux_run = aux && want_names && (has_ids || has_names);
        int rc_aux = 0, rc_len = 0;
        const bool len_on_aux = aux_run && early_has_work;
        int rc_small = 0;
        if (aux_run && !len_on_aux) rc_small = small3(c);
        bool names_beside = aux_run && aux_names && !len_on_aux && has_ids && has_names && h.orig_size[S_IDS] >= (1u << 20) && h.orig_size[S_NAMES] >= (1u << 20);
        { const char *nb = ctx_opt(c, "NAMES_BESIDE"); if (nb && nb[0] == '0') names_beside = false; }
        int rc_names = 0;
        if (names_beside) ctx_worker_start(aux_names, [&] { rc_names = ids_names(aux_names, 2); });
        if (aux_run) ctx_worker_start(aux, [&] { if (len_on_aux) rc_small = small3(aux); rc_aux = rc_small ? rc_small : ids_names(aux, names_beside ? 1 : 3); if (len_on_aux && !rc_small) rc_len = lengths(aux); });
        early();
        if (!aux_run) rc_small = small3(c);
        if (!len_on_aux) rc_len = rc_small ? rc_small : lengths(c);
        if (aux_run) { ctx_worker_join(aux); hipStreamSynchronize(aux->stream); }
        if (names_beside) { ctx_worker_join(aux_names); hipStreamSynchronize(aux_names->stream); }
        if (rc_len) { if (len_on_aux) memcpy(c->err, aux->err, sizeof c->err); return rc_len; }
        if (!aux_run) rc_aux = ids_names(c);
        else if (rc_aux) memcpy(c->err, aux->err, sizeof c->err);
        if (rc_aux) return rc_aux;
        if (rc_names) { memcpy(c->err, aux_names->err, sizeof c->err); return rc_names; }
        P.rec_len = rec_len;
        u32 *hdr_len = arena_new<u32>(c, N + 1);
        u64 *rec_out = arena_new<u64>(c, N + 2), *rec_base = arena_new<u64>(c, N + 2);
        if (!hdr_len || !rec_out || !rec_base) return NAF_GPU_ENOMEM;
        LAUNCH(c, "unnaf_rec_sizes", k_rec_sizes, cdiv(N, 256), 256, 0, N, (const u64 *)rec_len, P.idz, P.nmz, P.has_ids, P.has_names, P.mode, P.L, hdr_len, rec_out, rec_base);
        HIP_TRY(c, hipMemsetAsync(rec_out + N, 0, 8, c->stream));
        HIP_TRY(c, hipMemsetAsync(rec_base + N, 0, 8, c->stream));
        if ((rc = scan_exclusive_u64(c, rec_out, N + 1, (u64 *)nullptr))) return rc;
        if ((rc = scan_exclusive_u64(c, rec_base, N + 1, (u64 *)nullptr))) return rc;
        if ((rc = ctx_readback2(c, &tot[0], rec_out + N, 8, &tot[1], rec_base + N, 8))) return rc;
        P.hdr_len = hdr_len; P.rec_out = rec_out; P.rec_base = rec_base;
        }
        if (tot[1] > T) return ctx_fail(c, NAF_GPU_EFORMAT, "sum of lengths (%llu) exceeds the stored sequence length (%llu)", (unsigned long long)tot[1], (unsigned long long)T);
        if (P.mode == EM_FASTQ && h.orig_size[S_QUAL] < tot[1])
            return ctx_fail(c, NAF_GPU_EFORMAT, "corrupted quality: %llu quality codes stored for %llu bases\n", (unsigned long long)h.orig_size[S_QUAL], (unsigned long long)tot[1]);
        if (P.mode == EM_SEQUENCES && T == 0) tot[0] = 0;
        pl.total = pl.main_total = tot[0]; pl.surplus = 0; pl.sur_c = 0;
        if (tot[1] < T && P.mode != EM_FASTQ) {
            const u64 S = T - tot[1];
            u64 tail = S;
            if (P.mode == EM_FASTA) {
                unsigned long long *d_last = arena_new<unsigned long long>(c, 2); if (!d_last) return NAF_GPU_ENOMEM;
                HIP_TRY(c, hipMemsetAsync(d_last, 0, 16, c->stream));
                LAUNCH(c, "unnaf_last_nonempty", k_last_nonempty, cdiv(N, 256), 256, 0, (const u64 *)rec_len, N, d_last);
                u64 last1 = 0; if ((rc = ctx_readback(c, &last1, d_last, 8))) return rc;
                if (last1 == 0) tail = 0;
                else {
                    u64 len_last = 0; if ((rc = ctx_readback(c, &len_last, rec_len + (last1 - 1), 8))) return rc;
                    const u64 L = P.L;
                    const u64 cc = L ? ((len_last % L) ? L - len_last % L : 0) : 0;
                    pl.sur_c = cc;
                    if (L && S > cc) { const u64 R = S - cc; tail = cc + 1 + R + (R - 1) / L; }
                }
            }
            pl.surplus = tail ? S : 0; pl.sur_base0 = tot[1];
            pl.total = pl.main_total + tail;
        }
    }
    return 0;
}

static int unnaf_sections(naf_gpu_ctx *c, const u8 *d_naf, UnnafPlan &pl, naf_gpu_ctx *aux = nullptr, naf_gpu_ctx *aux_mask = nullptr, naf_gpu_ctx *aux_names = nullptr)
{
    const naf_gpu_header &h = pl.h;
    EmitP &P = pl.P;
    auto mask_part = [&](naf_gpu_ctx *x) -> int {
        int r;
        u8 *mu = nullptr; u64 n_mask = h.orig_size[S_MASK];
        {
            const char *mr = ctx_opt(c, "MASK_RLE");
            const u64 cs = h.comp_size[S_MASK];
            if (cs >= 4 && cs <= MASK_RLE_SRC && n_mask >= 2 * cs && !(mr && mr[0] == '0')) {
                const u8 fhd = pl.frame_head[S_MASK][0];
                const u32 fcs_flag = fhd >> 6, single = (fhd >> 5) & 1;
                struct { u32 hdr_size; bool ok; } fh;
                fh.hdr_size = 1 + (single ? 0 : 1) + (fcs_flag == 0 ? single : (fcs_flag == 1 ? 2 : (fcs_flag == 2 ? 4 : 8)));
                fh.ok = !(fhd & 0x0F);
                if (fh.ok && fh.hdr_size < cs) {
                    u64 *tg = arena_new<u64>(x, MASK_RLE_TOG + 1), *d_res = arena_new<u64>(x, 4);
                    if (!tg || !d_res) return NAF_GPU_ENOMEM;
                    LAUNCH(x, "unnaf_mask_rle", k_mask_rle_frame, 1, 256, (u32)((cs + 15) & ~15ull), d_naf + h.payload_off[S_MASK], (u32)cs, fh.hdr_size, n_mask, tg, MASK_RLE_TOG, d_res);
                    u64 res[3] = { 0, 0, 0 };
                    if ((r = ctx_readback(x, res, d_res, 24))) return r;
                    if (res[0] == 1) { P.toggles = tg; P.n_toggles = res[1]; return 0; }
                }
            }
        }
        if ((r = load_section(x, d_naf, h, S_MASK, n_mask, "mask", &mu, pl.frame_head[S_MASK]))) return r;
        u64 tiles = (n_mask + MT_TILE - 1) / MT_TILE;
        u64 *ts = arena_new<u64>(x, tiles + 2), *tc = arena_new<u64>(x, tiles + 2);
        if (!ts || !tc) return NAF_GPU_ENOMEM;
        if (tiles) LAUNCH(x, "unnaf_mask_count", k_mask_count, tiles, 256, 0, (const u8 *)mu, n_mask, ts, tc);
        if ((r = scan_exclusive_u64(x, ts, tiles, (u64 *)nullptr))) return r;
        if ((r = scan_exclusive_u64(x, tc, tiles, tc + tiles + 1))) return r;
        u64 ntog = 0;
        if ((r = ctx_readback(x, &ntog, tc + tiles + 1, 8))) return r;
        u64 *tg = arena_new<u64>(x, ntog + 1);
        if (!tg) return NAF_GPU_ENOMEM;
        if (tiles) LAUNCH(x, "unnaf_mask_scatter", k_mask_scatter, tiles, 256, 0, (const u8 *)mu, n_mask, (const u64 *)ts, (const u64 *)tc, tg, ntog);
        P.toggles = tg; P.n_toggles = ntog;
        return 0;
    };
    int rc_mask = 0;
    const bool mask_started = P.masking && aux_mask;
    if (mask_started) ctx_worker_start(aux_mask, [&] { rc_mask = mask_part(aux_mask); });
    bool mask_early = false; char mask_err[sizeof c->err];
    auto early = [&]() {
        if (P.masking && !mask_started && P.mode != EM_SEQ && aux) { mask_early = true; rc_mask = mask_part(c); if (rc_mask) memcpy(mask_err, c->err, sizeof c->err); }
    };
    int rc = unnaf_sections_main(c, d_naf, pl, aux, early, P.masking && !mask_started && P.mode != EM_SEQ && aux != nullptr, aux_names);
    if (mask_started) { ctx_worker_join(aux_mask); hipStreamSynchronize(aux_mask->stream); }
    if (rc) return rc;
    if (mask_started && rc_mask) { memcpy(c->err, aux_mask->err, sizeof c->err); return rc_mask; }
    if (mask_early) { if (rc_mask) { memcpy(c->err, mask_err, sizeof c->err); return rc_mask; } }
    else if (P.masking && !mask_started && (rc = mask_part(c))) return rc;
    return 0;
}

#include "payload.h"

static int unnaf_run(naf_gpu_ctx *c, const u8 *d_naf, size_t naf_len, const naf_gpu_unnaf_opts *o,
                     u64 out_begin, u64 out_end, bool whole, u8 *d_out, size_t out_cap, size_t *out_len, bool size_only)
{
    if (!c || !d_naf || !o || !out_len) return NAF_GPU_EARG;
    arena_reset(c);
    if (whole && !size_only) { int rs = ctx_sides_ready(c); if (rs) return rs; }
    UnnafPlan pl;
    int rc = unnaf_prepare(c, d_naf, naf_len, o, pl); if (rc) return rc;
    if (pl.empty) { *out_len = 0; return 0; }
    const naf_gpu_header &h = pl.h;
    bool ranged = false; u64 s_lo = 0, s_hi = 0, q_lo = 0, q_hi = 0;
    auto payload_seq = [&]() -> int {
        PayloadSpan sp;
        int r = payload_range(c, d_naf, pl, S_SEQ, s_lo, s_hi, ranged ? PAYLOAD_RANGE : PAYLOAD_WHOLE, &sp);
        if (!r) pl.P.seq = sp.base;
        return r;
    };
    auto payload_qual = [&](naf_gpu_ctx *qc) -> int {
        PayloadSpan sp;
        int r = payload_range(qc, d_naf, pl, S_QUAL, q_lo, q_hi, ranged ? PAYLOAD_RANGE : PAYLOAD_WHOLE, &sp);
        if (!r) pl.P.qual = sp.base;
        return r;
    };
    auto payload = [&]() -> int { int r = payload_seq(); if (r) return r; return pl.need_qual ? payload_qual(c) : 0; };
    const char *fuse = ctx_opt(c, "FUSE");
    const bool fuse_on = fuse && fuse[0] == '1';
    const bool par = whole && !size_only && pl.P.mode != -1 && c->side && !fuse_on;
    bool payload_done = false;
    ZSplit split; split.parts = 0; split.done = 0; split.status = nullptr;
    ZFlat zflat; memset(&zflat, 0, sizeof zflat);
    struct FlatGuard { ZFlat *z; ~FlatGuard() { zstd_flat_drop(z); } } flat_guard{ &zflat };
    const char *ff = ctx_opt(c, "FLAT_FUSE"), *ek0 = ctx_opt(c, "EMIT");
    const bool try_flat = !size_only && pl.fourbit && !fuse_on && !pl.P.force_slow && !(ff && ff[0] == '0') && !(ek0 && ek0[0]) &&
                          (pl.P.mode == EM_FASTA || pl.P.mode == EM_SEQ || pl.P.mode == EM_SEQUENCES) && pl.P.N && h.orig_size[S_SEQ] / pl.P.N >= 16384 &&
                          (pl.P.mode != EM_FASTA || pl.P.L == 0 || pl.P.L >= 16);
    if (par) {
        arena_reset(c->side);
        HIP_TRY(c, hipEventRecord(c->fork_ev, c->stream));
        HIP_TRY(c, hipStreamWaitEvent(c->side->stream, c->fork_ev, 0));
        int rc_side = 0, rc_q = 0;
        const bool qpar = pl.need_qual && c->side2;
        if (qpar) { arena_reset(c->side2); HIP_TRY(c, hipStreamWaitEvent(c->side2->stream, c->fork_ev, 0)); }
        if (c->side3) { arena_reset(c->side3); HIP_TRY(c, hipStreamWaitEvent(c->side3->stream, c->fork_ev, 0)); }
        if (c->side4) { arena_reset(c->side4); HIP_TRY(c, hipStreamWaitEvent(c->side4->stream, c->fork_ev, 0)); }
        ctx_worker_start(c->side, [&] { rc_side = unnaf_sections(c->side, d_naf, pl, c->side3, nullptr, c->side4); });
        if (qpar) ctx_worker_start(c->side2, [&] { rc_q = payload_qual(c->side2); });
        const char *nsp = ctx_opt(c, "SPLIT");
        const int nparts = nsp ? atoi(nsp) : 4;
        if (!pl.need_qual && c->side2 && nparts >= 2 && nparts <= ZSPLIT_MAX && pl.P.mode != -1) {
            split.parts = nparts; split.done = 0;
            for (int k = 0; k < nparts; k++) split.ev[k] = c->split_ev[k];
            c->zsplit = &split;
            arena_reset(c->side2);
        }
        if (try_flat) { zflat.ready = false; zflat.aux = c->zsplit ? c->side2 : nullptr; c->zflat = &zflat; }
        rc = payload_seq();
        c->zsplit = nullptr; c->zflat = nullptr;
        if (!rc && pl.need_qual && !qpar) rc = payload_qual(c);
        ctx_worker_join(c->side);
        if (qpar) ctx_worker_join(c->side2);
        if (rc_side) { memcpy(c->err, c->side->err, sizeof c->err); return rc_side; }
        if (rc) return rc;
        if (rc_q) { memcpy(c->err, c->side2->err, sizeof c->err); return rc_q; }
        HIP_TRY(c, hipStreamSynchronize(c->side->stream));
        if (qpar) HIP_TRY(c, hipStreamSynchronize(c->side2->stream));
        payload_done = true;
    } else if (pl.P.mode != -1) {
        if ((rc = unnaf_sections(c, d_naf, pl))) return rc;
    }
    if (whole) { out_begin = 0; out_end = pl.total; }
    if (out_end > pl.total) out_end = pl.total;
    if (out_begin > out_end) out_begin = out_end;
    *out_len = out_end - out_begin;
    if (size_only) { *out_len = pl.total; return 0; }
    if (*out_len > out_cap) return ctx_fail(c, NAF_GPU_ECAP, "unnaf output needs %llu bytes, capacity %zu", (unsigned long long)*out_len, out_cap);
    if (*out_len == 0) return 0;
    const u64 m_begin = out_begin < pl.main_total ? out_begin : pl.main_total, m_end = out_end < pl.main_total ? out_end : pl.main_total;
    const bool has_main = m_end > m_begin, has_tail = out_end > pl.main_total;
    pl.P.out_begin = m_begin; pl.P.out_end = m_end;
    u64 rec0 = 0, rec1 = pl.P.N ? pl.P.N - 1 : 0;
    if (!whole && pl.P.mode != -1) {
        u64 g[4] = { pl.sur_base0, pl.sur_base0, rec1, rec1 };
        if (has_main) {
            u64 *d_g = arena_new<u64>(c, 4); if (!d_g) return NAF_GPU_ENOMEM;
            LAUNCH(c, "unnaf_range_bases", k_range_bases, 1, 64, 0, pl.P, d_g);
            if ((rc = ctx_readback(c, g, d_g, 32))) return rc;
        }
        rec0 = g[2]; rec1 = g[3];
        if (g[1] < g[0]) g[1] = g[0];
        if (has_tail) g[1] = pl.P.T;
        s_lo = pl.fourbit ? g[0] / 2 : g[0]; s_hi = pl.fourbit ? (g[1] + 1) / 2 : g[1];
        q_lo = g[0]; q_hi = g[1];
        ranged = true;
    }
    if (whole && pl.P.mode == EM_FASTA && pl.fourbit && (pl.P.L == 0 || pl.P.L >= 16) && !pl.P.force_slow && fuse_on && !pl.surplus) {
        size_t n2 = 0;
        rc = zstd_decode_fused_fasta(c, d_naf + h.payload_off[S_SEQ], h.comp_size[S_SEQ], 0, &n2, &pl.P, d_out);
        if (rc == 0) {
            if (n2 != pl.seq_bytes) return ctx_fail(c, NAF_GPU_EFORMAT, "can't decompress sequence\n");
            return 0;
        }
        if (rc != -100) return rc;
    }
    if (!payload_done) {
        if (try_flat) { zflat.ready = false; c->zflat = &zflat; }
        rc = payload();
        c->zflat = nullptr;
        if (rc) return rc;
    }
    if (zflat.ready) { pl.P.fsrc = zflat.src; pl.P.fsi = zflat.si; pl.P.fslots = zflat.nslots; pl.P.fsym = zflat.sym; pl.P.ftail = zflat.tail; pl.P.ftail_q = zflat.tail_q; pl.P.ftail_n = zflat.tail_n; pl.P.fcls = zflat.cls; }
    if (pl.P.mode == -1) {
        HIP_TRY(c, hipMemcpyAsync(d_out, pl.P.seq + out_begin, out_end - out_begin, hipMemcpyDeviceToDevice, c->stream));
        return 0;
    }
    if (has_main) {
        const char *ek = ctx_opt(c, "EMIT");
        bool short_rec = pl.P.mode != EM_SEQ && pl.total / pl.P.N < 16384;
        if (ek && !strcmp(ek, "short")) short_rec = pl.P.mode != EM_SEQ;
        if (ek && !strcmp(ek, "long")) short_rec = false;
        if (pl.P.force_slow) { short_rec = false; ek = "span"; }
        const bool emit_wave = !ctx_opt_is(c, "EMIT_WAVE", '0');
        if (whole && pl.P.mode == EM_FASTQ && !pl.P.force_slow && !(ek && ek[0])) {
            {
                const u64 avg = pl.P.N ? (pl.P.out_end - pl.P.out_begin) / pl.P.N + 1 : 1;
                const u32 lanes = avg * 64 <= ER_STAGE * 7 / 8 ? 4u : avg * 32 <= ER_STAGE * 7 / 8 ? 8u : 16u;
                const bool w1 = emit_wave;
                const u32 wgt = w1 ? 64u : 256u, grid = (u32)cdiv(pl.P.N, wgt / lanes);
#define ER_LAUNCH(FB, LN) do { if (w1) LAUNCH(c, "unnaf_emit_records", (k_emit_fastq_records<FB, LN, 64>), grid, 64, 0, pl.P, d_out); \
                               else LAUNCH(c, "unnaf_emit_records", (k_emit_fastq_records<FB, LN, 256>), grid, 256, 0, pl.P, d_out); } while (0)
                if (pl.fourbit) { if (lanes == 4) ER_LAUNCH(true, 4); else if (lanes == 8) ER_LAUNCH(true, 8); else ER_LAUNCH(true, 16); }
                else { if (lanes == 4) ER_LAUNCH(false, 4); else if (lanes == 8) ER_LAUNCH(false, 8); else ER_LAUNCH(false, 16); }
#undef ER_LAUNCH
            }
        } else if (short_rec) {
            if (pl.P.mode == EM_FASTA || pl.P.mode == EM_FASTQ) {
                u64 nr = rec1 - rec0 + 1, htot = 0;
                u64 *ho = arena_new<u64>(c, nr + 2); if (!ho) return NAF_GPU_ENOMEM;
                LAUNCH(c, "unnaf_hdr_len64", k_hdr_len64, cdiv(nr, 256), 256, 0, pl.P.hdr_len, rec0, nr, ho);
                if ((rc = scan_exclusive_u64(c, ho, nr, ho + nr + 1))) return rc;
                if ((rc = ctx_readback(c, &htot, ho + nr + 1, 8))) return rc;
                u8 *ht = (u8 *)arena_alloc(c, htot + 32); if (!ht) return NAF_GPU_ENOMEM;
                LAUNCH(c, "unnaf_hdr_build", k_hdr_build, cdiv(nr, 32), 256, 0, pl.P, rec0, nr, (const u64 *)ho, ht);
                pl.P.hdr_off = ho; pl.P.hdr_text = ht; pl.P.hdr_r0 = rec0;
            }
            u32 grid = cdiv(m_end - m_begin, ES_SPAN);
            if (pl.fourbit) LAUNCH(c, "unnaf_emit_short", k_emit_short<true>, grid, 256, 0, pl.P, d_out);
            else LAUNCH(c, "unnaf_emit_short", k_emit_short<false>, grid, 256, 0, pl.P, d_out);
        } else if (ek && !strcmp(ek, "span")) {
            u32 grid = cdiv(m_end - m_begin, EMIT_SPAN);
            if (pl.fourbit) LAUNCH(c, "unnaf_emit", k_emit<true>, grid, 256, 0, pl.P, d_out);
            else LAUNCH(c, "unnaf_emit", k_emit<false>, grid, 256, 0, pl.P, d_out);
        } else {
            u64 ntiles = cdiv(m_end - m_begin, 4096);
            TileIdx *ti = arena_new<TileIdx>(c, ntiles + 2 + FLAT_TPW); u64 *tr = arena_new<u64>(c, ntiles + 2);
            u32 *list = arena_new<u32>(c, ntiles + 1), *cnt = arena_new<u32>(c, 2);
            u32 *list2 = (zflat.ready && zflat.cls) ? arena_new<u32>(c, ntiles + 1) : list;
            if (!ti || !tr || !list || !cnt || !list2) return NAF_GPU_ENOMEM;
            if (!split.done) HIP_TRY(c, hipMemsetAsync(cnt, 0, 8, c->stream));
            u64 Lp1 = pl.P.L + 1;
            pl.P.Ldiv_magic = (Lp1 >= 2 && Lp1 < 32768) ? (u32)((1ull << 32) / Lp1 + 1) : 0;
            naf_gpu_ctx *ic = split.done ? c->side2 : c;
            auto emit_tiles = [&](naf_gpu_ctx *x, u64 t0, u64 t1) {
                if (emit_wave && pl.fourbit) LAUNCH(x, "unnaf_emit", (k_emit_tile_wave<true, 2>), cdiv(t1 - t0, 2u), 64, 0, pl.P, (const TileIdx *)(ti + t0), d_out + t0 * 4096, (u64)(t1 - t0));
                else if (emit_wave) LAUNCH(x, "unnaf_emit", (k_emit_tile_wave<false, 2>), cdiv(t1 - t0, 2u), 64, 0, pl.P, (const TileIdx *)(ti + t0), d_out + t0 * 4096, (u64)(t1 - t0));
                else if (pl.fourbit) LAUNCH(x, "unnaf_emit", k_emit_tile<true>, (u32)(t1 - t0), 256, 0, pl.P, (const TileIdx *)(ti + t0), d_out + t0 * 4096);
                else LAUNCH(x, "unnaf_emit", k_emit_tile<false>, (u32)(t1 - t0), 256, 0, pl.P, (const TileIdx *)(ti + t0), d_out + t0 * 4096);
            };
            if (split.done) HIP_TRY(c, hipMemsetAsync(cnt, 0, 8, ic->stream));
            TileFlat *tsig = nullptr;
            if (zflat.ready) {
                tsig = arena_new<TileFlat>(c, ntiles + 2 + FLAT_TPW); u32 *fpair = arena_new<u32>(c, 400); if (!tsig || !fpair) return NAF_GPU_ENOMEM;
                LAUNCH(ic, "unnaf_flat_pair", k_flat_pair, 1, 256, 0, pl.P, fpair);
                pl.P.fpair = fpair;
            }
            LAUNCH(ic, "unnaf_tile_index", k_tile_index, cdiv(ntiles + 1 + FLAT_TPW, TILE_WG), 256, 0, pl.P, ntiles, ti, tr, list, cnt, tsig, (u32)FLAT_TPW, list2);
            naf_gpu_ctx *xc = c;
            const bool flat_job = zflat.ready && zflat.later;
            if (zflat.ready && zflat.aux) {
                HIP_TRY(c, hipEventRecord(c->split_ev[0], c->stream));
                if (!flat_job) { HIP_TRY(c, hipStreamWaitEvent(zflat.aux->stream, c->split_ev[0], 0)); xc = zflat.aux; }
            }
            u64 t_done = 0;
            if (split.done) {
                HIP_TRY(c, hipEventRecord(c->split_ev[ZSPLIT_MAX], ic->stream));
                for (int k = 0; k + 1 < split.parts; k++) {
                    u64 bases_ready = split.out_end[k] * (pl.fourbit ? 2u : 1u);
                    u64 t_hi = bases_ready / 4096; t_hi = t_hi > 1 ? t_hi - 1 : 0;
                    if (t_hi > ntiles) t_hi = ntiles;
                    if (t_hi <= t_done) continue;
                    HIP_TRY(c, hipStreamWaitEvent(ic->stream, split.ev[k], 0));
                    emit_tiles(ic, t_done, t_hi);
                    t_done = t_hi;
                }
                HIP_TRY(c, hipEventRecord(c->split_ev[ZSPLIT_MAX + 1], ic->stream));
                HIP_TRY(c, hipStreamWaitEvent(c->stream, c->split_ev[ZSPLIT_MAX], 0));
            }
            if (zflat.ready) {
                const u32 nwg = cdiv(ntiles, 4u), chunk = (nwg + 7) / 8;
                const bool mixed = flat_job || (zflat.cls && zflat.n_decoded);
                const bool wave = emit_wave && (!mixed || zflat.n_walk == 0);
                if (wave && pl.P.masking && pl.P.n_toggles >= ntiles) { const u32 ch = ((u32)ntiles + 7) / 8; LAUNCH(c, "unnaf_emit_flat", k_emit_tile_flat_wave<1>, ch * 8, 64, 0, pl.P, (const TileIdx *)ti, (const TileFlat *)tsig, d_out, (u64)ntiles, ch); }
                else if (wave) { const u32 ch = (cdiv(ntiles, 2u) + 7) / 8; LAUNCH(c, "unnaf_emit_flat", k_emit_tile_flat_wave<2>, ch * 8, 64, 0, pl.P, (const TileIdx *)ti, (const TileFlat *)tsig, d_out, (u64)ntiles, ch); }
                else
                LAUNCH(c, "unnaf_emit_flat", k_emit_tile_flat<4>, chunk * 8, 256, 0, pl.P, (const TileIdx *)ti, (const TileFlat *)tsig, d_out, (u64)ntiles, chunk);
                if (flat_job) {
                    if ((rc = zstd_flat_later(c, &zflat))) return rc;
                    if (zflat.aux) xc = zflat.aux;
                }
                if (zflat.cls && zflat.n_decoded) {
                    const u64 est = (u64)zflat.n_decoded * 64 + 64;
                    const u32 lgrid = (u32)(est < ntiles ? (est < 16384 ? est : 16384) : (ntiles < 16384 ? ntiles : 16384));
                    if (wave) LAUNCH(xc, "unnaf_emit", k_emit_tile_list_wave<true>, lgrid, 64, 0, pl.P, (const TileIdx *)ti, (const u32 *)list2, (const u32 *)(cnt + 1), d_out);
                    else LAUNCH(xc, "unnaf_emit", k_emit_tile_list<true>, lgrid, 256, 0, pl.P, (const TileIdx *)ti, (const u32 *)list2, (const u32 *)(cnt + 1), d_out);
                }
            }
            else if (t_done < ntiles) emit_tiles(c, t_done, ntiles);
            const u32 rest_grid = 4u * (u32)(ntiles < EMIT_REST_GRID ? ntiles : EMIT_REST_GRID);
            if (pl.fourbit) LAUNCH(xc, "unnaf_emit_rest", k_emit_rest<true>, rest_grid, 64, 0, pl.P, (const TileIdx *)ti, (const u64 *)tr, (const u32 *)list, (const u32 *)cnt, d_out);
            else LAUNCH(xc, "unnaf_emit_rest", k_emit_rest<false>, rest_grid, 64, 0, pl.P, (const TileIdx *)ti, (const u64 *)tr, (const u32 *)list, (const u32 *)cnt, d_out);
            if (xc != c) { HIP_TRY(c, hipEventRecord(c->split_ev[1], xc->stream)); HIP_TRY(c, hipStreamWaitEvent(c->stream, c->split_ev[1], 0)); }
            if (split.done) HIP_TRY(c, hipStreamWaitEvent(c->stream, c->split_ev[ZSPLIT_MAX + 1], 0));
            if (zflat.ready && ctx_tracing(c)) {
                u32 hc[2] = { 0, 0 };
                if (!ctx_readback(c, hc, cnt, 8)) ctx_trace(c, "[flat tiles] total %llu rest %u decoded %u\n", (unsigned long long)ntiles, hc[0], hc[1]);
            }
        }
    }
    if (has_tail) {
        const u64 lo = (out_begin > pl.main_total ? out_begin : pl.main_total) - pl.main_total, hi = out_end - pl.main_total;
        u8 *dst = d_out + (pl.main_total + lo - out_begin);
        const int wrap = pl.P.mode == EM_FASTA;
        if (pl.fourbit) LAUNCH(c, "unnaf_emit_surplus", k_emit_surplus<true>, cdiv(hi - lo, 256), 256, 0, pl.P, pl.sur_base0, pl.surplus, pl.sur_c, pl.P.L, wrap, lo, hi, dst);
        else LAUNCH(c, "unnaf_emit_surplus", k_emit_surplus<false>, cdiv(hi - lo, 256), 256, 0, pl.P, pl.sur_base0, pl.surplus, pl.sur_c, pl.P.L, wrap, lo, hi, dst);
    }
    HIP_TRY(c, hipGetLastError());
    if ((rc = zstd_split_status(c, &split))) return rc;
    if (zflat.ready) { ZSplit fs; fs.parts = 0; fs.done = 1; fs.status = zflat.status; if ((rc = zstd_split_status(c, &fs))) return rc; }
    return 0;
}

extern "C" int naf_gpu_unnaf_size(naf_gpu_ctx *c, const void *d_naf, size_t naf_len, const naf_gpu_unnaf_opts *o, size_t *out_len)
{
    return unnaf_run(c, (const u8 *)d_naf, naf_len, o, 0, 0, true, nullptr, 0, out_len, true);
}
extern "C" int naf_gpu_unnaf(naf_gpu_ctx *c, const void *d_naf, size_t naf_len, const naf_gpu_unnaf_opts *o, void *d_out, size_t out_cap, size_t *out_len)
{
    int rc = unnaf_run(c, (const u8 *)d_naf, naf_len, o, 0, 0, true, (u8 *)d_out, out_cap, out_len, false);
    if (c) arena_settle(c);
    return rc;
}
extern "C" int naf_gpu_unnaf_range(naf_gpu_ctx *c, const void *d_naf, size_t naf_len, const naf_gpu_unnaf_opts *o,
                                   uint64_t out_begin, uint64_t out_end, void *d_out, size_t out_cap, size_t *out_len)
{
    int rc = unnaf_run(c, (const u8 *)d_naf, naf_len, o, out_begin, out_end, false, (u8 *)d_out, out_cap, out_len, false);
    if (c) arena_settle(c);
    return rc;
}

#include "emit_select.h"
#include "locate.h"
#include "composition.h"

__global__ __launch_bounds__(256) void k_histogram(const u8 *p, u64 n, unsigned long long *counts)
{
    __shared__ u32 h[4][256];
    for (u32 i = threadIdx.x; i < 1024; i += 256) ((u32 *)h)[i] = 0;
    __syncthreads();
    u32 *my = h[threadIdx.x >> 6];
    const u64 per = 65536;
    u64 lo = (u64)blockIdx.x * per, hi = lo + per < n ? lo + per : n;
    for (u64 i = lo + (u64)threadIdx.x * 8; i < hi; i += 256 * 8) {
        if (i + 8 <= hi) { u64 w = ld64(p + i); for (int k = 0; k < 8; k++) atomicAdd(&my[(w >> (8 * k)) & 0xFF], 1u); }
        else for (u64 k = i; k < hi; k++) atomicAdd(&my[p[k]], 1u);
    }
    __syncthreads();
    u32 v = h[0][threadIdx.x] + h[1][threadIdx.x] + h[2][threadIdx.x] + h[3][threadIdx.x];
    if (v) atomicAdd(&counts[threadIdx.x], (unsigned long long)v);
}
extern "C" int naf_gpu_histogram(naf_gpu_ctx *c, const void *d_buf, size_t n, uint64_t counts[256])
{
    if (!c || !counts || (!d_buf && n)) return NAF_GPU_EARG;
    arena_reset(c);
    unsigned long long *d = arena_new<unsigned long long>(c, 256); if (!d) return NAF_GPU_ENOMEM;
    HIP_TRY(c, hipMemsetAsync(d, 0, 256 * 8, c->stream));
    if (n) LAUNCH(c, "histogram", k_histogram, cdiv(n, 65536), 256, 0, (const u8 *)d_buf, (u64)n, d);
    return ctx_readback(c, counts, d, 256 * 8);
}
```

### naf_amd/csrc/zstd_dec.hip

```cpp
#include <type_traits>
#include "ctx.h"
#include "wgscan.h"
#include "zstd_dec_core.h"
#include "emit_core.h"

struct ZStat {
    u32 nblk; u32 err; u64 end_off;
    u32 n_huf_def, n_seq_blk, max_huf_log, rep_slow;
    u32 huf_pool_used, fse_pool_used;
    u64 total_seq, total_out;
    u32 ticket, n_plain_huf;
    u32 max_seq_regen, n_flat;
    u32 n_huf_distinct, n_huf_built;
    u32 max_lit_regen, n_huf_pending;
    u32 last_raw, flat_main_inv;
    u32 n_exec_done, n_wave;
#ifdef NAF_EXEC_PROF
    unsigned long long prof[8];
#endif
};

static __device__ __forceinline__ void set_err(ZStat *st, u32 e) { if (e) atomicMax(&st->err, e); }
static __device__ __forceinline__ u64 shfl_u64(u64 v, int l) { u32 lo = __shfl((u32)v, l, 64), hi = __shfl((u32)(v >> 32), l, 64); return ((u64)hi << 32) | lo; }

// ... 3086 lines not shown
}

#define SMALL_SRC 16384u
#define SMALL_OUT 32768u
#define SMALL_SEQ 2048u
#define SMALL_TOO_BIG 100u
struct SmallRes { u32 err, out, pos; };
struct SmallWS { HufLdsWS H; ZBlock b; ZStat st; };
__device__ void small_frame_decode(const u8 *src, u32 len, u8 *dst, u32 cap, u8 *lit, u32 *sll, u32 *sml, u32 *sof, const FseE *predef,
                                   SmallWS &W, u16 *huf, FseE *fse, i16 *norm, u16 *nx, SmallRes *res, const u32 *llt, const u32 *mlt)
{
    const u32 lane = threadIdx.x;
    u32 err = 0, out = 0, pos = 0;
    ZFrameHdr fh = zstd_parse_frame_header(src, len);
    if (fh.err) { res->err = (u32)fh.err; res->out = 0; res->pos = 0; return; }
    pos = fh.hdr_size;
    u32 huf_log = 0; bool have_huf = false;
    SeqTab tab[3]; bool have_tab[3] = { false, false, false };
    const u32 fo[3] = { 0, 512, 768 }, po[3] = { 0, 64, 96 }, pl[3] = { 6, 5, 6 }, max_log[3] = { 9, 8, 9 }, max_sym[3] = { 35, 31, 52 };
    u32 rep[3] = { 1, 4, 8 };
    for (;;) {
        if (pos + 3 > len) { err = ZE_TRUNC; break; }
        const u32 h = ld24(src + pos), last = h & 1, type = (h >> 1) & 3, size = h >> 3;
        if (type == 3 || size > ZBLOCK_MAX) { err = ZE_CORRUPT; break; }
        const u32 csize = type == BT_RLE ? 1 : size;
        if (pos + 3 + csize > len) { err = ZE_TRUNC; break; }
        const u8 *c = src + pos + 3;
        pos += 3 + csize;
        if (type != BT_COMP) {
            if ((u64)out + size > cap) { err = SMALL_TOO_BIG; break; }
            if (type == BT_RAW) for (u32 k = lane; k < size; k += 64) dst[out + k] = c[k];
            else { const u8 v = c[0]; for (u32 k = lane; k < size; k += 64) dst[out + k] = v; }
            __syncthreads();
            out += size;
            if (last) break;
            continue;
        }
        ZBlock b; b.src_off = 0; b.bsize = size; b.btype = BT_COMP; b.last = (u8)last;
        zstd_parse_block(c, b);
        if (b.err) { err = b.err; break; }
        if ((u64)out + b.lit_regen > cap) { err = SMALL_TOO_BIG; break; }
        u8 *lp = b.nseq ? lit : dst + out;
        if (b.lit_type == LIT_RAW) for (u32 k = lane; k < b.lit_regen; k += 64) lp[k] = c[b.lit_off + k];
        else if (b.lit_type == LIT_RLE) { const u8 v = c[b.lit_off]; for (u32 k = lane; k < b.lit_regen; k += 64) lp[k] = v; }
        else {
            if (b.lit_type == LIT_HUF) {
                __syncthreads();
                if (lane == 0) { W.b = b; W.b.src_off = 0; }
                __syncthreads();
                build_huf_one_lds(c, &W.b, 0, nullptr, 0, &W.st, W.H, (u8 *)huf);
                __syncthreads();
                const u32 lg = W.H.log;
                if (!lg) { err = ZE_CORRUPT; break; }
                huf_log = lg; have_huf = true;
            } else if (!have_huf) { err = ZE_CORRUPT; break; }
            const u8 *sp = c + b.huf_streams_off;
            bool bad = false;
            if (b.nstreams == 1) { if (lane == 0) bad = huf_decode_stream(sp, b.huf_streams_size, (const u16 *)huf, huf_log, lp, b.lit_regen) != 0; }
            else {
                const u32 s1 = ld16(sp), s2 = ld16(sp + 2), s3 = ld16(sp + 4), tot = b.huf_streams_size - 6, per = (b.lit_regen + 3) / 4;
                if (s1 + s2 + s3 >= tot || !s1 || !s2 || !s3 || per * 3 > b.lit_regen) { err = ZE_CORRUPT; break; }
                if (lane < 4) {
                    const u32 k = lane;
                    const u32 o = k == 0 ? 0 : (k == 1 ? s1 : (k == 2 ? s1 + s2 : s1 + s2 + s3)), z = k == 0 ? s1 : (k == 1 ? s2 : (k == 2 ? s3 : tot - s1 - s2 - s3));
                    bad = huf_decode_stream(sp + 6 + o, z, (const u16 *)huf, huf_log, lp + k * per, k < 3 ? per : b.lit_regen - 3 * per) != 0;
                }
            }
            if (__ballot(bad)) { err = ZE_CORRUPT; break; }
        }
        __syncthreads();
        if (!b.nseq) { out += b.lit_regen; if (last) break; continue; }
        if (b.nseq > SMALL_SEQ) { err = SMALL_TOO_BIG; break; }
        u32 p = b.seq_off; bool tbad = false;
        for (int k = 0; k < 3 && !tbad; k++) {
            const u32 m = b.modes[k];
            if (m == SM_PREDEF) { tab[k].t = predef + po[k]; tab[k].log = pl[k]; tab[k].rle = false; tab[k].rle_sym = 0; have_tab[k] = true; }
            else if (m == SM_RLE) { tab[k].t = predef; tab[k].log = 0; tab[k].rle = true; tab[k].rle_sym = b.fse_tab[k]; have_tab[k] = true; p++; }
            else if (m == SM_FSE) {
                u32 nsym, lg;
                const u32 d = fse_read_ncount(c + p, b.bsize - p, max_log[k], max_sym[k], norm, &nsym, &lg);
                if (!d || lg != b.fse_log[k] || !fse_build_table(fse + fo[k], norm, nsym, lg, nx)) { tbad = true; break; }
                p += d; tab[k].t = fse + fo[k]; tab[k].log = lg; tab[k].rle = false; tab[k].rle_sym = 0; have_tab[k] = true;
            } else if (!have_tab[k]) tbad = true;
        }
        if (tbad || p != b.seq_bits_off) { err = ZE_CORRUPT; break; }
        u64 tl = 0, tm = 0; u32 ro[3];
        u8 e = 0xFF;
        if (b.modes[0] == SM_PREDEF && b.modes[1] == SM_PREDEF && b.modes[2] == SM_PREDEF)
            e = zstd_decode_sequences_predef<const FseE *, const u32 *, false>(c + b.seq_bits_off, b.seq_bits_size, b.nseq, predef, predef + 64, predef + 96, llt, mlt, sll, sml, sof, ro, &tl, &tm, nullptr);
        if (e == 0xFF) e = zstd_decode_sequences(c + b.seq_bits_off, b.seq_bits_size, b.nseq, tab, sll, sml, sof, ro, &tl, &tm);
        if (e) { err = e; break; }
        if (tl > b.lit_regen) { err = ZE_CORRUPT; break; }
        const u64 regen = b.lit_regen + tm;
        if (regen > ZBLOCK_MAX) { err = ZE_CORRUPT; break; }
        if ((u64)out + regen > cap) { err = SMALL_TOO_BIG; break; }
        __syncthreads();
        u32 op = out, l = 0; bool xbad = false;
        for (u32 q0 = 0; q0 < b.nseq && !xbad; q0 += 64) {
            const u32 q = q0 + lane; const bool on = q < b.nseq;
            const u32 ll = on ? sll[q] : 0, ml = on ? sml[q] : 0;
            const u32 ill = wave_scan_inclusive<u32, OpAdd>(ll), iml = wave_scan_inclusive<u32, OpAdd>(ml);
            const u32 my_l = l + ill - ll, my_op = op + (ill - ll) + (iml - ml);
            { u32 k = 0; for (; k + 8 <= ll; k += 8) st64(dst + my_op + k, ld64(lit + my_l + k)); for (; k < ll; k++) dst[my_op + k] = lit[my_l + k]; }
            __syncthreads();
            const u32 cnt = b.nseq - q0 < 64 ? b.nseq - q0 : 64;
            for (u32 j = 0; j < cnt; j++) {
                const u32 mop = (u32)__shfl((int)(my_op + ll), (int)j, 64), mlj = (u32)__shfl((int)ml, (int)j, 64), of = sym_resolve(sof[q0 + j], rep);
                if (of == 0 || of > mop) { xbad = true; break; }
                if (of >= mlj || of >= 64) for (u32 k0 = 0; k0 < mlj; k0 += 64) { const u32 k = k0 + lane; if (k < mlj) { const u8 v = dst[mop + k - of]; dst[mop + k] = v; } __syncthreads(); }
                else { for (u32 k = lane; k < mlj; k += 64) dst[mop + k] = dst[mop - of + k % of]; __syncthreads(); }
            }
            op += (u32)__shfl((int)(ill + iml), 63, 64); l += (u32)__shfl((int)ill, 63, 64);
        }
        if (xbad) { err = ZE_CORRUPT; break; }
        { const u32 rest = b.lit_regen - l; for (u32 k = lane; k < rest; k += 64) dst[op + k] = lit[l + k]; op += rest; }
        __syncthreads();
        { const u32 r0 = sym_resolve(ro[0], rep), r1 = sym_resolve(ro[1], rep), r2 = sym_resolve(ro[2], rep); rep[0] = r0; rep[1] = r1; rep[2] = r2; }
        out = op;
        if (last) break;
    }
    if (!err && fh.checksum) { if (pos + 4 > len) err = ZE_TRUNC; else pos += 4; }
    if (!err && fh.has_fcs && fh.content_size != out) err = ZE_CORRUPT;
    res->err = err; res->out = out; res->pos = pos;
}
__global__ __launch_bounds__(64) void k_small_frame(const u8 *src, u32 len, u8 *dst, u32 cap, const FseE *predef, u32 *res)
{
    __builtin_amdgcn_s_setprio(3);
    __shared__ __attribute__((aligned(16))) u8 s_src[SMALL_SRC + 16], s_out[SMALL_OUT + 16], s_lit[SMALL_OUT + 16];
    __shared__ u32 s_ll[SMALL_SEQ], s_ml[SMALL_SEQ], s_of[SMALL_SEQ];
    __shared__ SmallWS W;
    __shared__ __attribute__((aligned(16))) u16 huf[HUF_TAB_MAX / 2];
    __shared__ FseE fse[512 + 256 + 512];
    __shared__ FseE s_predef[160];
    __shared__ i16 norm[64];
    __shared__ u16 nx[64];
    __shared__ SmallRes r;
    __shared__ u32 s_llt[36], s_mlt[53];
    zstd_seq_code_tables(s_llt, s_mlt, threadIdx.x, 64);
    for (u32 k = threadIdx.x; k < len; k += 64) s_src[k] = src[k];
    for (u32 k = threadIdx.x; k < 16; k += 64) s_src[len + k] = 0;
    for (u32 k = threadIdx.x; k < 160; k += 64) s_predef[k] = predef[k];
    __syncthreads();
    small_frame_decode(s_src, len, s_out, cap < SMALL_OUT ? cap : SMALL_OUT, s_lit, s_ll, s_ml, s_of, s_predef, W, huf, fse, norm, nx, &r, s_llt, s_mlt);
    __syncthreads();
    if (r.err == 0) for (u32 k = threadIdx.x; k < r.out; k += 64) dst[k] = s_out[k];
    if (threadIdx.x == 0) { res[0] = r.err; res[1] = r.out; res[2] = r.pos; }
}

struct SmallJobs { const u8 *src[4]; u8 *dst[4]; u32 len[4], cap[4]; };
__global__ __launch_bounds__(64) void k_small_frames(SmallJobs J, const FseE *predef, u32 *res)
{
    __builtin_amdgcn_s_setprio(3);
    __shared__ __attribute__((aligned(16))) u8 s_src[SMALL_SRC + 16], s_out[SMALL_OUT + 16], s_lit[SMALL_OUT + 16];
    __shared__ u32 s_ll[SMALL_SEQ], s_ml[SMALL_SEQ], s_of[SMALL_SEQ];
    __shared__ SmallWS W;
    __shared__ __attribute__((aligned(16))) u16 huf[HUF_TAB_MAX / 2];
    __shared__ FseE fse[512 + 256 + 512];
    __shared__ FseE s_predef[160];
    __shared__ i16 norm[64];
    __shared__ u16 nx[64];
    __shared__ SmallRes r;
    __shared__ u32 s_llt[36], s_mlt[53];
    zstd_seq_code_tables(s_llt, s_mlt, threadIdx.x, 64);
    const u32 j = blockIdx.x;
    const u8 *src = J.src[j]; const u32 len = J.len[j], cap = J.cap[j]; u8 *dst = J.dst[j];
    for (u32 k = threadIdx.x; k < len; k += 64) s_src[k] = src[k];
    for (u32 k = threadIdx.x; k < 16; k += 64) s_src[len + k] = 0;
    for (u32 k = threadIdx.x; k < 160; k += 64) s_predef[k] = predef[k];
    __syncthreads();
    small_frame_decode(s_src, len, s_out, cap < SMALL_OUT ? cap : SMALL_OUT, s_lit, s_ll, s_ml, s_of, s_predef, W, huf, fse, norm, nx, &r, s_llt, s_mlt);
    __syncthreads();
    if (r.err == 0) for (u32 k = threadIdx.x; k < r.out; k += 64) dst[k] = s_out[k];
    if (threadIdx.x == 0) { res[4 * j] = r.err; res[4 * j + 1] = r.out; res[4 * j + 2] = r.pos; }
}
int zstd_small_batch(naf_gpu_ctx *c, int n, const u8 *const *src, const size_t *len, u8 *const *dst, const size_t *cap, bool *ok)
{
    SmallJobs J; memset(&J, 0, sizeof J); int m = 0, map[4];
    for (int k = 0; k < n && k < 4; k++) {
        ok[k] = false;
        if (len[k] == 0 || len[k] > SMALL_SRC || cap[k] > SMALL_OUT) continue;
        J.src[m] = src[k]; J.len[m] = (u32)len[k]; J.dst[m] = dst[k]; J.cap[m] = (u32)cap[k]; map[m++] = k;
    }
    if (!m) return 0;
    u32 *d_res = arena_new<u32>(c, 16); if (!d_res) return NAF_GPU_ENOMEM;
    LAUNCH(c, "zstd_small_frame", k_small_frames, m, 64, 0, J, (const FseE *)c->d_predef, d_res);
    u32 res[16]; int rc = ctx_readback(c, res, d_res, 16 * (size_t)m); if (rc) return rc;
    for (int q = 0; q < m; q++) ok[map[q]] = res[4 * q] == 0 && res[4 * q + 1] == J.cap[q] && res[4 * q + 2] == J.len[q];
    return 0;
}
bool zstd_small_fits(size_t len, size_t cap) { return len != 0 && len <= SMALL_SRC && cap <= SMALL_OUT; }
int zstd_small_launch(naf_gpu_ctx *c, int n, const u8 *const *src, const size_t *len, u8 *const *dst, const size_t *cap, u32 **d_res_out)
{
    SmallJobs J; memset(&J, 0, sizeof J);
    if (n < 1 || n > 4) return NAF_GPU_EARG;
    for (int k = 0; k < n; k++) { if (!zstd_small_fits(len[k], cap[k])) return NAF_GPU_EARG; J.src[k] = src[k]; J.len[k] = (u32)len[k]; J.dst[k] = dst[k]; J.cap[k] = (u32)cap[k]; }
    u32 *d_res = arena_new<u32>(c, 16); if (!d_res) return NAF_GPU_ENOMEM;
    LAUNCH(c, "zstd_small_frame", k_small_frames, n, 64, 0, J, (const FseE *)c->d_predef, d_res);
    *d_res_out = d_res;
    return 0;
}

int zstd_init_tables(naf_gpu_ctx *c)
{
    static const i16 LL[36] = { 4,3,2,2,2,2,2,2,2,2,2,2,2,1,1,1,2,2,2,2,2,2,2,2,2,3,2,1,1,1,1,1,-1,-1,-1,-1 };
    static const i16 OF[29] = { 1,1,1,1,1,1,2,2,2,1,1,1,1,1,1,1,1,1,1,1,1,1,1,1,-1,-1,-1,-1,-1 };
    static const i16 ML[53] = { 1,4,3,2,2,2,2,2,2,1,1,1,1,1,1,1,1,1,1,1,1,1,1,1,1,1,1,1,1,1,1,1,1,1,1,1,1,1,1,1,1,1,1,1,1,1,-1,-1,-1,-1,-1,-1,-1 };
    FseE tabs[64 + 32 + 64]; u16 next[64];
    if (!fse_build_table(tabs, LL, 36, 6, next) || !fse_build_table(tabs + 64, OF, 29, 5, next) || !fse_build_table(tabs + 96, ML, 53, 6, next))
        return ctx_fail(c, NAF_GPU_EZSTD, "predefined FSE tables");
    HIP_TRY(c, hipMalloc(&c->d_predef, sizeof tabs));
    HIP_TRY(c, hipMemcpy(c->d_predef, tabs, sizeof tabs, hipMemcpyHostToDevice));
    return 0;
}


static u32 huf_par_plog(const naf_gpu_ctx *c, u32 max_lit_regen, u64 n_blocks)
{
    const char *e = ctx_opt(c, "HUF_PAR");
    if (e && e[0] == '0') return 0;
    const char *t = ctx_opt(c, "HUF_PART");
    u32 target = t ? (u32)atoi(t) : 128u; if (target < 64) target = 64;
    const u32 nmax = (max_lit_regen + 3) / 4;
    u32 plog = 0;
    while (plog < 6 && (nmax >> (plog + 1)) >= target) plog++;
    if (e && e[0] >= '1' && e[0] <= '6') { const u32 f = (u32)(e[0] - '0'); return f < plog ? f : plog; }
    if (n_blocks * (u64)max_lit_regen >= (u64)nmax * 86016) return 0;
    const char *ll = ctx_opt(c, "HUF_LANES_LOG");
    const u32 lanes_log = ll && atoi(ll) >= 10 && atoi(ll) <= 24 ? (u32)atoi(ll) : (nmax >= 16384 ? 20u : 18u);
    while (plog && ((n_blocks * 4) << plog) > (1ull << lanes_log)) plog--;
    return plog;
}
static u32 huf_par_margin_env(const naf_gpu_ctx *c) { const char *m = ctx_opt(c, "HUF_MARGIN"); return m ? (u32)atoi(m) : 0u; }

#define ZSTD_NEED_TWO_PASS (-100)
static int launch_build_huf(naf_gpu_ctx *c, u32 count, const u8 *src, ZBlock *blk, u32 nblk, u8 *pool, u32 pool_cap, ZStat *st, u32 first, const u64 *range4, u32 always_table, const i32 *own_huf, u32 gate, u32 phase)
{
    const char *e = ctx_opt(c, "HUF_BUILD16");
    if (e && e[0] == '0') LAUNCH(c, "zstd_build_huf", k_build_huf, cdiv(count, 64), 64, 0, src, blk, nblk, pool, pool_cap, st, first, range4, always_table, own_huf, gate, phase);
    else if (ctx_opt_is(c, "HUF_BUILD_WG", '1')) LAUNCH(c, "zstd_build_huf", k_build_huf16<16>, cdiv(count, 16), 256, 0, src, blk, nblk, pool, pool_cap, st, first, range4, always_table, own_huf, gate, phase);
    else LAUNCH(c, "zstd_build_huf", k_build_huf16<4>, cdiv(count, 4), 64, 0, src, blk, nblk, pool, pool_cap, st, first, range4, always_table, own_huf, gate, phase);
    return 0;
}
static int zerr(naf_gpu_ctx *c, u32 e, const char *where)
{
    const char *m = e == ZE_TRUNC ? "truncated" : e == ZE_CORRUPT ? "corrupt" : e == ZE_UNSUP ? "unsupported feature" : "table pool";
    return ctx_fail(c, NAF_GPU_EZSTD, "zstd frame %s (%s)", m, where);
}

struct ZFrame {
    naf_gpu_ctx *c; const u8 *src; size_t src_len; u8 *dst; size_t dst_cap; size_t *out_len, *consumed; ZRange *rg; const EmitP *fuse; u8 *text;
    ZFrameHdr fh; u8 hb[18]; size_t hl;
    u32 always_table, spec_min; bool uni_wanted;
    ZStat *st, hs; ZBlock *blk; u32 nblk, g;
    i32 *own_huf, *own_ll, *own_of, *own_ml; u64 *seq_cnt, *sizes, *d_total_out; u32 n_seq_blk, n_huf_def, max_seq_regen;
    u8 *huf_pool; u32 pool_cap; bool spec, lit_only_spec, tables_built, ranged_build, two_phase, have_ends;
    u64 h4[5], hends[ZSPLIT_MAX];
    FseE *fse_pool; u32 *o_ll, *o_ml, *o_of, *seq_list; u64 *seq_rank;
    u32 b_first, b_count, huf_first, seq_t0, seq_t1; u64 bias; u32 *done; u8 *lit_scratch;
};
static_assert(std::is_trivially_copyable<ZFrame>::value, "ZFrame is copied into the deferred job");
#define Z_HANDED 1
[[maybe_unused]] static const void *const driver_kernels[] = { (const void *)k_spec_walk<false>, (const void *)k_spec_walk<true>, (const void *)k_copy_fill<64>, (const void *)k_flat_literals<64>,
    (const void *)k_huf_literals<false>, (const void *)k_huf_literals<true>, (const void *)k_copy_fill<256>, (const void *)k_flat_literals<256>, (const void *)k_huf_literals<false, true> };

struct LitPlan { u8 *dst, *lits; const u8 *cls; u8 *redo; bool wide, serial;
                 u32 flat_on, plog, slot, ipitch, generic, pending; };
static int launch_literals(naf_gpu_ctx *c, const ZFrame &F, u32 lo, u32 hi, const LitPlan &p)
{
    if (hi <= lo) return 0;
    const u32 n = hi - lo, huf_lds = p.slot * HUF_BLOCKS_PER_WG + 64 * p.ipitch + 64 * HUF_OROW + 512;
    const ZBlock *blk = F.blk; const i32 *own_huf = F.own_huf; const u8 *pool = F.huf_pool;
    EmitP ep; memset(&ep, 0, sizeof ep);
    if (p.flat_on && !p.wide) LAUNCH(c, "zstd_flat_literals", k_flat_literals<64>, 4 * n, 64, 0, F.src, blk, hi, own_huf, pool, p.dst, p.lits, F.st, lo, p.cls);
    else if (p.flat_on) LAUNCH(c, "zstd_flat_literals", k_flat_literals<256>, n, 256, 0, F.src, blk, hi, own_huf, pool, p.dst, p.lits, F.st, lo, p.cls);
    if (p.serial && p.plog)
        LAUNCH(c, "zstd_huf_literals", k_huf_par, cdiv((u64)n << (p.plog + 2), 64), 64, (p.plog >= 4 ? 1u : 16u >> p.plog) * p.slot,
               F.src, blk, hi, own_huf, pool, p.slot, p.dst, p.lits, F.st, lo, p.plog, p.cls, p.flat_on, huf_par_margin_env(c), p.pending, (u64)F.src_len);
    else if (p.serial) {
        if (p.redo) LAUNCH(c, "zstd_huf_literals", (k_huf_literals<false, true>), cdiv(n, HUF_BLOCKS_PER_WG), 64, huf_lds - p.slot * (HUF_BLOCKS_PER_WG - 1u),
               F.src, blk, hi, own_huf, pool, p.slot, p.dst, p.lits, F.st, lo, ep, (u8 *)nullptr, p.ipitch | p.generic, (u64)F.src_len, p.flat_on, p.cls, p.redo);
        LAUNCH(c, "zstd_huf_literals", (k_huf_literals<false>), cdiv(n, HUF_BLOCKS_PER_WG), 64, huf_lds,
               F.src, blk, hi, own_huf, pool, p.slot, p.dst, p.lits, F.st, lo, ep, (u8 *)nullptr, p.ipitch | p.generic, (u64)F.src_len, p.flat_on, p.redo ? (const u8 *)p.redo : p.cls);
    }
    return 0;
}
static int launch_exec(naf_gpu_ctx *c, const ZFrame &F, const u32 *list, u32 nx, const u8 *lits, u8 *dst, u32 *done)
{
    const u32 cap = (F.max_seq_regen + 1023u) & ~1023u;
    if (F.max_seq_regen > EXEC_LDS || ctx_opt_is(c, "EXEC_LDS", '0'))
        return launch_lz_exec(c, (const ZBlock *)F.blk, list, nx, (const u64 *)F.sizes, (const u64 *)F.seq_cnt, F.nblk, F.hs.total_seq, F.o_ll, F.o_ml, F.o_of, lits, dst, done, F.st);
    LAUNCH(c, "zstd_exec_seq", k_exec_seq_lds, nx, 64, cap + 64u + 2u * EXEC_PJ_MAX, (const ZBlock *)F.blk, list, nx, (const u64 *)F.sizes, F.nblk,
           (const u32 *)F.o_ll, (const u32 *)F.o_ml, (const u32 *)F.o_of, lits, dst, done, F.st, cap);
    return 0;
}
static int build_huf_rest(naf_gpu_ctx *c, const ZFrame &F, ZStat *hs)
{
    int rc = launch_build_huf(c, F.nblk, F.src, F.blk, F.nblk, F.huf_pool, F.pool_cap, F.st, 0u, (const u64 *)nullptr, 0u, (const i32 *)F.own_huf, 1u, 2u);
    if (rc || (rc = ctx_readback(c, hs, F.st, sizeof *hs))) return rc;
    return hs->err ? zerr(c, hs->err, "Huffman tables") : 0;
}
static u32 split_part_end(u32 n, int parts, int k) { return k + 1 == parts ? n : (u32)((u64)n * (k + 1) / parts) & ~(HUF_BLOCKS_PER_WG - 1u); }

struct FlatMixed { const u8 *cls; u32 n_decoded, n_walk; void *later; };
static int flat_handoff(const ZFrame &F, const FlatStream *si, u64 nslots, const u8 *sym, u64 end_off, u64 total_out, u32 last_raw, const FlatMixed *mixed)
{
    naf_gpu_ctx *c = F.c; ZFlat *zf = c->zflat;
    if (mixed) { zf->cls = mixed->cls; zf->n_decoded = mixed->n_decoded; zf->n_walk = mixed->n_walk; zf->decoded_ev = nullptr; zf->later = mixed->later; }
    const size_t frame_end = end_off + (F.fh.checksum ? 4 : 0);
    if (frame_end > F.src_len) return zerr(c, ZE_TRUNC, "checksum");
    *F.consumed = frame_end;
    const u32 tn = last_raw & 0x7FFFFFFFu; const bool rle = (last_raw >> 31) != 0;
    zf->src = F.src; zf->si = si; zf->nslots = nslots; zf->sym = sym; zf->status = F.st; zf->ready = true;
    zf->tail = last_raw ? F.src + (end_off - (rle ? 1u : tn)) : nullptr; zf->tail_q = total_out - (last_raw ? tn : 0u);
    zf->tail_n = last_raw ? (rle ? tn | 0x80000000u : tn) : 0u;
    if (F.rg) { F.rg->got_lo = 0; F.rg->got_hi = total_out; F.rg->ranged = false; }
    *F.out_len = total_out;
    if (F.fh.has_fcs && F.fh.content_size != total_out) return zerr(c, ZE_CORRUPT, "content size mismatch");
    return Z_HANDED;
}

static u32 first_block_header(const ZFrame &F) { const u8 *p = F.hb + F.fh.hdr_size; return (u32)p[0] | ((u32)p[1] << 8) | ((u32)p[2] << 16); }
struct SpecIdx { u32 chunk, win1, win2, nchunks; u64 *first, *land, *G, *start, *cnt; };
static void spec_geometry(const ZFrame &F, SpecIdx &X)
{
    X.chunk = SPEC_CHUNK; X.win1 = SPEC_WINDOW1; X.win2 = SPEC_WINDOW;
    if (F.src_len <= 4ull * SPEC_CHUNK) {
        X.chunk = 256; while (X.chunk < SPEC_CHUNK_SMALL && (u64)X.chunk * 128 < F.src_len) X.chunk *= 2;
        X.win1 = X.win2 = X.chunk;
    } else if (F.src_len <= 256ull * SPEC_CHUNK && F.fh.hdr_size + 3 <= F.hl) {
        const u32 h0 = first_block_header(F);
        const u32 b0 = ((h0 >> 1) & 3) == 1 ? 4u : (h0 >> 3) + 3;
        u32 want = SPEC_CHUNK_SMALL; while (want < SPEC_CHUNK && want < 16 * b0) want *= 2;
        if (want < SPEC_CHUNK) { X.chunk = want; if (X.win1 > X.chunk) X.win1 = X.chunk; if (X.win2 > X.chunk) X.win2 = X.chunk; }
    }
    X.nchunks = (u32)((F.src_len + X.chunk - 1) / X.chunk);
}
static int index_stride_runs(ZFrame &F, u32 S, u32 h0, u32 nmax, const u32 *sres)
{
    naf_gpu_ctx *c = F.c; int rc; const u8 *d_src = F.src;
    UniRuns *R = arena_new<UniRuns>(c, 1); ZBlock *odd = arena_new<ZBlock>(c, STRIDE_TAIL + 1), *ublk0 = arena_new<ZBlock>(c, 1);
    u32 *probe = arena_new<u32>(c, 2); UniInfo *U2 = arena_new<UniInfo>(c, 1);
    FlatStream *usi2 = arena_new<FlatStream>(c, 4 * ((size_t)nmax + USEG_MAX) + 1); u8 *usym2 = (u8 *)arena_alloc(c, 16);
    if (!R || !odd || !ublk0 || !probe || !U2 || !usi2 || !usym2) return NAF_GPU_ENOMEM;
    for (u32 r = 0; r <= URUN_MAX; r++) {
        LAUNCH(c, "zstd_index_stride", k_runs_next, 1, 64, 0, d_src, (u64)F.src_len, (u64)F.fh.hdr_size, S, h0, sres, R, odd, probe, r == 0 ? 1 : 0);
        if (r < URUN_MAX) LAUNCH(c, "zstd_index_stride", k_runs_probe, cdiv(nmax, 256), 256, 0, d_src, (u64)F.src_len, S, h0, (const UniRuns *)R, probe);
    }
    LAUNCH(c, "zstd_flat_uniform", k_uni_head_runs, 1, 64, 0, d_src, (u64)F.fh.hdr_size, h0, R, odd, U2, ublk0, F.spec_min);
    LAUNCH(c, "zstd_flat_uniform", k_uni_streams_runs, cdiv(4ull * ((u64)nmax + USEG_MAX) + 1, 256) + 1, 256, 0, d_src, S, (const UniRuns *)R, (const ZBlock *)odd, (const ZBlock *)ublk0, U2, usi2, usym2);
    UniInfo hu2; memset(&hu2, 0, sizeof hu2);
    if ((rc = ctx_readback(c, &hu2, U2, sizeof hu2))) return rc;
    if (ctx_tracing(c)) ctx_trace(c, "[runs?] ok %u bad %u first run %u blocks %u huffman %u total %llu\n", hu2.ok, hu2.bad, hu2.np, hu2.nblk, hu2.nhb, (unsigned long long)hu2.total_out);
    if (!(hu2.ok && !hu2.bad)) return 0;
    return flat_handoff(F, usi2, 4ull * hu2.nhb, usym2, hu2.end_off, hu2.total_out, hu2.last_raw, nullptr);
}
static int index_stride(ZFrame &F, const SpecIdx &X)
{
    naf_gpu_ctx *c = F.c; int rc; const u8 *d_src = F.src; const size_t src_len = F.src_len; const ZFrameHdr &fh = F.fh; ZStat *st = F.st;
    if (ctx_tracing(c)) ctx_trace(c, "[stride?] len %zu hdr %u hl %zu first %02x %02x %02x\n", src_len, fh.hdr_size, F.hl, F.hb[fh.hdr_size], F.hb[fh.hdr_size + 1], F.hb[fh.hdr_size + 2]);
    if (!(src_len > 4ull * SPEC_CHUNK && fh.hdr_size + 3 <= F.hl) || ctx_opt_is(c, "STRIDE_INDEX", '0')) return 0;
    const u32 h0 = first_block_header(F), S = 3 + (h0 >> 3);
    const u64 nmax64 = (src_len - fh.hdr_size) / S;
    if (!(((h0 >> 1) & 3) == BT_COMP && !(h0 & 1) && (h0 >> 3) <= ZBLOCK_MAX && S >= 256 && nmax64 >= 64 && nmax64 < 0x7FFFFF00ull)) return 0;
    const u32 nmax = (u32)nmax64;
    u32 *sres = (u32 *)(X.cnt + X.nchunks + 2); ZBlock *sblk = arena_new<ZBlock>(c, (size_t)nmax + STRIDE_TAIL);
    if (!sblk) return NAF_GPU_ENOMEM;
    HIP_TRY(c, hipMemsetAsync(sres, 0xFF, 8, c->stream));
    LAUNCH(c, "zstd_index_stride", k_stride_probe, cdiv(nmax, 256), 256, 0, d_src, (u64)src_len, (u64)fh.hdr_size, S, h0, nmax, sres);
    LAUNCH(c, "zstd_index_stride", k_stride_tail, 1, 64, 0, d_src, (u64)src_len, (u64)fh.hdr_size, S, nmax, sres, sblk, st);
    UniInfo *U = nullptr; FlatStream *usi = nullptr; u8 *usym = nullptr;
    if (F.uni_wanted) {
        U = arena_new<UniInfo>(c, 1); ZBlock *ublk = arena_new<ZBlock>(c, STRIDE_TAIL + 1);
        usi = arena_new<FlatStream>(c, 4 * ((size_t)nmax + STRIDE_TAIL) + 1); usym = (u8 *)arena_alloc(c, 16);
        if (!U || !ublk || !usi || !usym) return NAF_GPU_ENOMEM;
        LAUNCH(c, "zstd_flat_uniform", k_uni_head, 1, 64, 0, d_src, (u64)fh.hdr_size, S, h0, nmax, (const u32 *)sres, (const ZBlock *)sblk, (const ZStat *)st, U, ublk, F.spec_min);
        LAUNCH(c, "zstd_flat_uniform", k_uni_streams, cdiv(4ull * ((u64)nmax + STRIDE_TAIL) + 1, 256) + 1, 256, 0, d_src, (u64)fh.hdr_size, S, (const ZBlock *)ublk, U, usi, usym);
    }
    LAUNCH(c, "zstd_index_stride", k_stride_write, cdiv(nmax, 256), 256, 0, (u64)fh.hdr_size, S, h0, (const u32 *)sres, sblk, (const u32 *)U);
    u32 res2[2] = { 0, 0 }; UniInfo hu; memset(&hu, 0, sizeof hu); ZStat &hs = F.hs;
    if (U) { void *hp[3] = { &hs, res2, &hu }; const void *dp[3] = { st, sres, U }; const size_t nb[3] = { sizeof hs, 8, sizeof hu }; rc = ctx_readbackv(c, 3, hp, dp, nb); }
    else rc = ctx_readback2(c, &hs, st, sizeof hs, res2, sres, 8);
    if (rc) return rc;
    if (ctx_tracing(c)) ctx_trace(c, "[stride] len %zu S %u nmax %u prefix %u verdict %u err %u nblk %u\n", src_len, S, nmax, res2[0], res2[1], hs.err, hs.nblk);
    if (ctx_tracing(c) && U) ctx_trace(c, "[uniform?] ok %u bad %u prefix %u blocks %u huffman %u regen %u total %llu\n", hu.ok, hu.bad, hu.np, hu.nblk, hu.nhb, hu.regen0, (unsigned long long)hu.total_out);
    if (res2[1] == 1u && !hs.err && hs.nblk && hu.ok && !hu.bad) return flat_handoff(F, usi, 4ull * hu.nhb, usym, hs.end_off, hu.total_out, hu.last_raw, nullptr);
    if (res2[1] == 1u && !hs.err && hs.nblk) F.blk = sblk;
    if (res2[1] == 2u && !hs.err && F.uni_wanted && !ctx_opt_is(c, "STRIDE_RUNS", '0')) return index_stride_runs(F, S, h0, nmax, sres);
    return 0;
}
static int index_speculative(ZFrame &F, const SpecIdx &X)
{
    naf_gpu_ctx *c = F.c; int rc; const u8 *d_src = F.src; const u64 len = (u64)F.src_len; ZStat *st = F.st;
    const u32 nchunks = X.nchunks, chunk = X.chunk, win1 = X.win1, win2 = X.win2, gl = cdiv(nchunks, 64);
    u64 *first = X.first, *land = X.land, *G = X.G, *start = X.start, *cnt = X.cnt; const u32 *skip = nullptr;
    const u32 win0 = chunk == SPEC_CHUNK ? SPEC_WINDOW0 : win1;
    LAUNCH(c, "zstd_index_find", k_spec_find, cdiv(win0, 256 * 16) * (nchunks - 1), 256, 0, d_src, len, nchunks, first, 0u, win0, chunk, skip);
    if (win1 > win0) LAUNCH(c, "zstd_index_find2", k_spec_find, cdiv(win1 - win0, 256 * 16) * (nchunks - 1), 256, 0, d_src, len, nchunks, first, win0, win1, chunk, skip);
    if (win2 > win1) LAUNCH(c, "zstd_index_find2", k_spec_find, cdiv(win2 - win1, 256 * 16) * (nchunks - 1), 256, 0, d_src, len, nchunks, first, win1, win2, chunk, skip);
    LAUNCH(c, "zstd_index_land", k_spec_land, gl, 64, 0, d_src, len, (const u64 *)first, nchunks, land, chunk, skip);
    LAUNCH(c, "zstd_index_land2", k_spec_land2, gl, 64, 0, d_src, len, (const u64 *)first, (const u64 *)land, nchunks, G, chunk, skip);
    LAUNCH(c, "zstd_index_resolve", k_spec_resolve, 1, 64, 0, d_src, len, (const u64 *)land, (const u64 *)G, nchunks, start, st, chunk, skip);
    LAUNCH(c, "zstd_index_count", (k_spec_walk<false>), gl, 64, 0, d_src, len, (const u64 *)start, nchunks, cnt, (ZBlock *)nullptr, st, skip);
    u64 *d_tot = cnt + nchunks + 1, tot = 0;
    if ((rc = scan_exclusive_u64(c, cnt, nchunks, d_tot))) return rc;
    if ((rc = ctx_readback2(c, &F.hs, st, sizeof F.hs, &tot, d_tot, 8))) return rc;
    if (!F.hs.err && tot > 0 && tot < 0x7FFFFFFFull) {
        if (!(F.blk = arena_new<ZBlock>(c, tot))) return NAF_GPU_ENOMEM;
        LAUNCH(c, "zstd_index_write", (k_spec_walk<true>), gl, 64, 0, d_src, len, (const u64 *)start, nchunks, cnt, F.blk, st, (const u32 *)nullptr);
        F.hs.nblk = (u32)tot;
    } else HIP_TRY(c, hipMemsetAsync(st, 0, sizeof(ZStat), c->stream));
    return 0;
}
static int index_parallel(ZFrame &F)
{
    naf_gpu_ctx *c = F.c; int rc; SpecIdx X; spec_geometry(F, X);
    const u32 nchunks = X.nchunks;
    X.first = arena_new<u64>(c, nchunks + 1); X.land = arena_new<u64>(c, nchunks + 2); X.G = arena_new<u64>(c, nchunks + 1);
    X.start = arena_new<u64>(c, nchunks + 2); X.cnt = arena_new<u64>(c, (size_t)nchunks + 4);
    if (!X.first || !X.land || !X.G || !X.start || !X.cnt) return NAF_GPU_ENOMEM;
    HIP_TRY(c, hipMemsetAsync(X.first, 0xFF, (size_t)nchunks * 8, c->stream));
    u64 *h0 = (u64 *)c->h_stage; *h0 = F.fh.hdr_size;
    HIP_TRY(c, hipMemcpyAsync(X.first, h0, 8, hipMemcpyHostToDevice, c->stream));
    if ((rc = index_stride(F, X)) || F.blk) return rc;
    return index_speculative(F, X);
}
static int index_serial(ZFrame &F)
{
    naf_gpu_ctx *c = F.c; int rc;
    u32 cap = (u32)(F.src_len / 16 + 1024);
    for (int attempt = 0; attempt < 2; attempt++) {
        if (!(F.blk = arena_new<ZBlock>(c, cap))) return NAF_GPU_ENOMEM;
        const u32 win = F.src_len < SCAN_WIN ? (u32)((F.src_len + 15) & ~15ull) + 16 : SCAN_WIN;
        LAUNCH(c, "zstd_scan_blocks", k_scan_blocks, 1, 64, win + 16, F.src, (u64)F.src_len, (u64)F.fh.hdr_size, F.blk, cap, F.st, win);
        if ((rc = ctx_readback(c, &F.hs, F.st, sizeof F.hs))) return rc;
        if (F.hs.err) return zerr(c, F.hs.err, "block headers");
        if (F.hs.nblk <= cap) break;
        cap = F.hs.nblk;
    }
    return 0;
}
static int spec_continuation(ZFrame &F)
{
    naf_gpu_ctx *c = F.c; int rc; const u8 *d_src = F.src; ZBlock *blk = F.blk; const u32 nblk = F.nblk; ZStat *st = F.st; ZRange *rg = F.rg;
    u64 *r4 = nullptr; bool late_build = false;
    if ((rc = scan_exclusive_u64(c, F.sizes, nblk, F.d_total_out))) return rc;
    u64 *extra = arena_new<u64>(c, 8 + ZSPLIT_MAX); if (!extra) return NAF_GPU_ENOMEM;
    if (rg && rg->want_hi > rg->want_lo) {
        r4 = extra;
        LAUNCH(c, "zstd_find_range", k_find_range, 1, 64, 0, (const u64 *)F.sizes, nblk, (const u64 *)F.d_total_out, rg->want_lo, rg->want_hi, (const i32 *)F.own_huf, r4);
        F.ranged_build = true;
    }
    const u64 want_pool = (u64)nblk * HUF_TAB_MAX + 4096;
    F.pool_cap = want_pool > 0xFFFFF000ull ? 0xFFFFF000u : (u32)want_pool;
    if (!(F.huf_pool = (u8 *)arena_alloc(c, F.pool_cap))) return NAF_GPU_ENOMEM;
    if (nblk <= 16384) {
        LAUNCH(c, "zstd_build_huf", k_build_huf_lds, nblk, 64, 0, d_src, blk, nblk, F.huf_pool, F.pool_cap, st, 0u, (const i32 *)F.own_huf);
    } else {
        LAUNCH(c, "zstd_build_huf", k_build_huf_few, 1024, 64, 0, d_src, blk, nblk, F.huf_pool, F.pool_cap, st, (const u64 *)r4, (const i32 *)F.own_huf);
        F.two_phase = c->zflat && !rg && !F.always_table;
        if (F.two_phase) LAUNCH(c, "zstd_build_huf", k_flat_find_main, FIND_MAIN_TREES, 64, 0, d_src, blk, nblk, F.huf_pool, F.pool_cap, st, (const i32 *)F.own_huf);
        else late_build = true;
    }
    ZSplit *sp = c->zsplit;
    if (sp && !rg && sp->parts >= 2) {
        F.have_ends = true;
        for (int k = 0; k + 1 < sp->parts; k++)
            HIP_TRY(c, hipMemcpyAsync(extra + 8 + k, F.sizes + split_part_end(nblk, sp->parts, k), 8, hipMemcpyDeviceToDevice, c->stream));
    }
    u64 hx[8 + ZSPLIT_MAX];
    if ((rc = ctx_readback2(c, &F.hs, st, sizeof F.hs, hx, extra, sizeof hx))) return rc;
    memcpy(F.h4, hx, sizeof F.h4); memcpy(F.hends, hx + 8, sizeof F.hends);
    if (late_build && !F.hs.err && F.hs.n_huf_distinct > HUF_FEW &&
        ((rc = launch_build_huf(c, nblk, d_src, blk, nblk, F.huf_pool, F.pool_cap, st, 0u, (const u64 *)r4, F.always_table, (const i32 *)F.own_huf, 1u, 0u)) || (rc = ctx_readback(c, &F.hs, st, sizeof F.hs)))) return rc;
    F.tables_built = true;
    return 0;
}
static int parse_ownership(ZFrame &F)
{
    naf_gpu_ctx *c = F.c; int rc; const u32 nblk = F.nblk, g = F.g; ZStat *st = F.st;
    i32 *own = arena_new<i32>(c, (size_t)nblk * 4);
    F.seq_cnt = arena_new<u64>(c, (size_t)nblk + 1); F.sizes = arena_new<u64>(c, (size_t)nblk + 1);
    if (!own || !F.seq_cnt || !F.sizes) return NAF_GPU_ENOMEM;
    F.own_huf = own; F.own_ll = own + nblk; F.own_of = own + 2 * (size_t)nblk; F.own_ml = own + 3 * (size_t)nblk;
    LAUNCH(c, "zstd_parse_blocks", k_parse_blocks, g, 64, 0, F.src, F.blk, nblk, F.own_huf, F.own_ll, F.own_of, F.own_ml, F.seq_cnt, F.sizes, st);
    LAUNCH(c, "zstd_huf_dedup", k_huf_dedup, g, 64, 0, F.src, (const ZBlock *)F.blk, nblk, F.own_huf, st);
    if ((rc = scan_inclusive_max_i32(c, F.own_huf, nblk))) return rc;
    F.d_total_out = (u64 *)((u8 *)st + offsetof(ZStat, total_out));
    F.spec = nblk > F.spec_min && !F.fuse;
    if (F.spec) rc = spec_continuation(F);
    else rc = ctx_readback(c, &F.hs, st, sizeof F.hs);
    if (rc) return rc;
    if (F.hs.err) return zerr(c, F.hs.err, "block parse");
    F.n_seq_blk = F.hs.n_seq_blk; F.n_huf_def = F.hs.n_huf_def;
    if (F.fuse && !(F.n_seq_blk == 0 && F.hs.n_plain_huf == nblk && nblk > 0)) return ZSTD_NEED_TWO_PASS;
    F.lit_only_spec = F.spec && F.n_seq_blk == 0;
    if (F.spec && F.n_seq_blk && F.ranged_build) {
        F.tables_built = false;
        for (size_t o : { offsetof(ZStat, huf_pool_used), offsetof(ZStat, max_huf_log), offsetof(ZStat, n_flat), offsetof(ZStat, n_huf_built) })
            HIP_TRY(c, hipMemsetAsync((u8 *)st + o, 0, 4, c->stream));
    }
    return 0;
}
static int exit_all_flat(ZFrame &F)
{
    naf_gpu_ctx *c = F.c; const ZStat &hs = F.hs; const u32 nblk = F.nblk;
    const bool flat_tail = hs.last_raw != 0 && nblk >= 2 && hs.n_plain_huf == nblk - 1;
    if (ctx_tracing(c) && c->zflat) ctx_trace(c, "[flat?] spec %d nblk %u seq_blk %u distinct %u built %u n_flat %u log %u plain %u last_raw %u always %u\n", (int)F.spec, nblk, F.n_seq_blk, hs.n_huf_distinct, hs.n_huf_built, hs.n_flat, hs.max_huf_log, hs.n_plain_huf, hs.last_raw, F.always_table);
    if (!(c->zflat && F.lit_only_spec && nblk > 0 && hs.n_huf_distinct == 1 && hs.n_huf_built == 1 && hs.n_flat == 1 && hs.max_huf_log == 4 && (hs.n_plain_huf == nblk || flat_tail) && !F.always_table)) return 0;
    const u32 nhb = flat_tail ? nblk - 1 : nblk;
    FlatStream *si = arena_new<FlatStream>(c, 4 * (size_t)nhb + 1); u8 *d_sym = (u8 *)arena_alloc(c, 16);
    if (!si || !d_sym) return NAF_GPU_ENOMEM;
    LAUNCH(c, "zstd_set_offsets", k_set_offsets, F.g, 64, 0, F.blk, nblk, (const u64 *)F.sizes, (u32 *)nullptr, (u32 *)nullptr, (u32 *)nullptr);
    LAUNCH(c, "zstd_flat_streams", k_flat_streams, cdiv(4ull * nhb, 256), 256, 0, F.src, (const ZBlock *)F.blk, nhb, (const i32 *)F.own_huf, (const u8 *)F.huf_pool, si, d_sym, F.st, (const u64 *)F.d_total_out, flat_tail ? (u64)(hs.last_raw & 0x7FFFFFFFu) : 0ull);
    return flat_handoff(F, si, 4ull * nhb, d_sym, hs.end_off, hs.total_out, flat_tail ? hs.last_raw : 0u, nullptr);
}
struct FlatClass { FlatStream *si; u8 *sym, *cls, *lits; u32 *done2; u32 n_dec, n_walk; };
static int flat_classify(ZFrame &F, bool with_sequences, FlatClass &K)
{
    naf_gpu_ctx *c = F.c; int rc; const u32 nblk = F.nblk, g = F.g, main = 0xFFFFFFFFu - F.hs.flat_main_inv;
    K.si = arena_new<FlatStream>(c, 4 * (size_t)nblk + 1); K.sym = (u8 *)arena_alloc(c, 16);
    u8 *cls0 = (u8 *)arena_alloc(c, nblk); K.cls = (u8 *)arena_alloc(c, nblk); u32 *d_nx = arena_new<u32>(c, 2);
    K.done2 = with_sequences ? arena_new<u32>(c, nblk) : nullptr; K.lits = with_sequences ? (u8 *)arena_alloc(c, F.hs.total_out + 16) : nullptr;
    if (!K.si || !K.sym || !cls0 || !K.cls || !d_nx || (with_sequences && (!K.done2 || !K.lits))) return NAF_GPU_ENOMEM;
    HIP_TRY(c, hipMemsetAsync(d_nx, 0, 8, c->stream));
    LAUNCH(c, "zstd_set_offsets", k_set_offsets, g, 64, 0, F.blk, nblk, (const u64 *)F.sizes, K.done2, (u32 *)nullptr, (u32 *)nullptr);
    LAUNCH(c, "zstd_flat_class", k_flat_mark_owner, g, 64, 0, F.src, F.blk, nblk, (const i32 *)F.own_huf, main, !with_sequences && F.two_phase ? 1u : 0u);
    LAUNCH(c, "zstd_flat_class", k_flat_sym, 1, 256, 0, F.src, (const ZBlock *)F.blk, main, (const u8 *)F.huf_pool, K.sym);
    LAUNCH(c, "zstd_flat_class", k_flat_class, g, 64, 0, (const ZBlock *)F.blk, nblk, (const i32 *)F.own_huf, cls0, d_nx + 1);
    if (with_sequences) LAUNCH(c, "zstd_flat_class", k_seq_sources, cdiv(F.n_seq_blk, 64), 64, 0, (const ZBlock *)F.blk, (const u32 *)F.seq_list, F.n_seq_blk, (const u64 *)F.sizes, (const u32 *)F.o_ll, (const u32 *)F.o_ml, (const u32 *)F.o_of, cls0);
    LAUNCH(c, "zstd_flat_class", k_flat_class2, g, 64, 0, (const u8 *)cls0, nblk, K.cls, d_nx);
    u32 nx2[2] = { 0, 0 };
    if ((rc = ctx_readback(c, nx2, d_nx, 8))) return rc;
    K.n_dec = nx2[0]; K.n_walk = nx2[1];
    if (ctx_tracing(c) && with_sequences) ctx_trace(c, "[flat mixed] nblk %u decoded %u main %u (blocks with sequences %u)\n", nblk, K.n_dec, main, F.n_seq_blk);
    else if (ctx_tracing(c)) ctx_trace(c, "[flat mixed] nblk %u decoded %u main %u\n", nblk, K.n_dec, main);
    return 0;
}
struct FlatJob { ZFrame F; const u8 *cls; u8 *lits; u32 *done2; u32 n_walk; bool pending; };
static int flat_job_steps(naf_gpu_ctx *c, const FlatJob &J)
{
    const ZFrame &F = J.F; const ZStat &hs0 = F.hs; const u32 nblk = F.nblk; const bool with_sequences = F.n_seq_blk != 0; int rc;
    if (c != F.c) HIP_TRY(c, hipStreamWaitEvent(c->stream, F.c->split_ev[0], 0));
    const u32 plog = J.n_walk ? huf_par_plog(c, hs0.max_lit_regen, J.n_walk) : 0u;
    u32 max_log = hs0.max_huf_log;
    if (J.pending && J.n_walk && !plog) {
        ZStat h2; if ((rc = build_huf_rest(c, F, &h2))) return rc;
        max_log = h2.max_huf_log;
    }
    if (with_sequences || hs0.n_plain_huf != nblk) LAUNCH(c, "zstd_copy_fill", k_copy_fill<64>, 4 * nblk, 64, 0, F.src, (const ZBlock *)F.blk, nblk, F.dst, J.lits, 0u, J.cls);
    LitPlan p; memset(&p, 0, sizeof p);
    p.dst = F.dst; p.lits = J.lits; p.cls = J.cls; p.serial = J.n_walk != 0; p.flat_on = 1u; p.plog = plog; p.pending = J.pending ? 1u : 0u;
    p.slot = plog && J.pending ? (u32)HUF_TAB_MAX : huf_slot_bytes(max_log); p.ipitch = max_log > 7 ? HUF_IROW_BIG : HUF_IROW;
    if ((rc = launch_literals(c, F, 0u, nblk, p))) return rc;
    return with_sequences ? launch_exec(c, F, (const u32 *)F.seq_list, F.n_seq_blk, (const u8 *)J.lits, F.dst, J.done2) : 0;
}
int zstd_flat_later(naf_gpu_ctx *, ZFlat *zf)
{
    if (!zf || !zf->later) return 0;
    FlatJob *j = (FlatJob *)zf->later; zf->later = nullptr;
    naf_gpu_ctx *mc = j->F.c, *c = zf->aux ? zf->aux : mc;
    const int rc = flat_job_steps(c, *j); delete j;
    if (rc && c != mc) memcpy(mc->err, c->err, sizeof mc->err);
    return rc;
}
void zstd_flat_drop(ZFlat *zf) { if (zf && zf->later) { delete (FlatJob *)zf->later; zf->later = nullptr; } }
static bool mostly_flat_wanted(const ZFrame &F)
{
    return F.c->zflat && F.spec && !F.always_table && !F.rg && F.hs.flat_main_inv && F.dst && F.hs.total_out <= F.dst_cap && !ctx_opt_is(F.c, "FLAT_MIXED", '0');
}
static int exit_mostly_flat(ZFrame &F, bool with_sequences)
{
    naf_gpu_ctx *c = F.c; int rc; const u32 nblk = F.nblk; FlatClass K;
    if ((rc = flat_classify(F, with_sequences, K))) return rc;
    if ((u64)K.n_dec * 2 > nblk) return 0;
    LAUNCH(c, "zstd_flat_streams", k_flat_streams_mixed, cdiv(4ull * nblk, 256), 256, 0, F.src, (const ZBlock *)F.blk, nblk, (const u8 *)K.cls, K.si, F.st, (const u64 *)F.d_total_out);
    FlatMixed M = { K.cls, K.n_dec, K.n_walk, nullptr };
    if (with_sequences || K.n_dec) M.later = new FlatJob{ F, K.cls, K.lits, K.done2, K.n_walk, !with_sequences && F.two_phase && F.hs.n_huf_distinct > HUF_FEW };
    return flat_handoff(F, K.si, 4ull * nblk, K.sym, F.hs.end_off, F.hs.total_out, 0u, &M);
}

static int seq_tables(ZFrame &F)
{
    naf_gpu_ctx *c = F.c; int rc; const u32 nblk = F.nblk, g = F.g; ZStat *st = F.st;
    for (i32 *own : { F.own_ll, F.own_of, F.own_ml }) if ((rc = scan_inclusive_max_i32(c, own, nblk))) return rc;
    if ((rc = scan_exclusive_u64(c, F.seq_cnt, nblk, (u64 *)((u8 *)st + offsetof(ZStat, total_seq))))) return rc;
    u32 fse_cap = F.n_seq_blk * (512 + 256 + 512);
    if (!(F.fse_pool = arena_new<FseE>(c, fse_cap))) return NAF_GPU_ENOMEM;
    LAUNCH(c, "zstd_build_fse", k_build_fse, cdiv(3 * (u64)nblk, 64), 64, 0, F.src, F.blk, nblk, F.fse_pool, fse_cap, st);
    if ((rc = ctx_readback(c, &F.hs, st, sizeof F.hs))) return rc;
    if (F.hs.err) return zerr(c, F.hs.err, "table build");
    size_t ns = F.hs.total_seq ? F.hs.total_seq : 1;
    F.o_ll = arena_new<u32>(c, ns); F.o_ml = arena_new<u32>(c, ns); F.o_of = arena_new<u32>(c, ns);
    if (!F.o_ll || !F.o_ml || !F.o_of) return NAF_GPU_ENOMEM;
    F.seq_list = arena_new<u32>(c, F.n_seq_blk);
    u64 *flag = arena_new<u64>(c, (size_t)nblk + 1); F.seq_rank = flag;
    if (!F.seq_list || !flag) return NAF_GPU_ENOMEM;
    LAUNCH(c, "zstd_seq_flag", k_seq_flag, g, 64, 0, (const ZBlock *)F.blk, nblk, flag);
    if ((rc = scan_exclusive_u64(c, flag, nblk, (u64 *)nullptr))) return rc;
    LAUNCH(c, "zstd_seq_list", k_seq_list, g, 64, 0, (const ZBlock *)F.blk, nblk, (const u64 *)flag, F.seq_list);
    return 0;
}
static int sequences(ZFrame &F)
{
    naf_gpu_ctx *c = F.c; int rc; const u8 *d_src = F.src; ZBlock *blk = F.blk; const u32 nblk = F.nblk, n_seq_blk = F.n_seq_blk; ZStat *st = F.st;
    if (n_seq_blk && (rc = seq_tables(F))) return rc;
    if (F.lit_only_spec) return 0;
    const u32 dsl = nblk < 32768 ? 16u : 64u;
    const u32 all_wave = ctx_opt_is(c, "SEQ_WAVE", 'a') ? 1u : 0u;
    const u32 own_tabs = (n_seq_blk && !ctx_opt_is(c, "SEQ_WAVE", '0')) ? 1u + all_wave : 0u;
    u32 *wave_list = own_tabs ? arena_new<u32>(c, n_seq_blk) : nullptr;
    if (own_tabs && !wave_list) return NAF_GPU_ENOMEM;
    LAUNCH(c, "zstd_decode_seq", k_decode_seq, cdiv(nblk, dsl), dsl, 0, d_src, blk, nblk, (const i32 *)F.own_ll, (const i32 *)F.own_of, (const i32 *)F.own_ml,
           (const u64 *)F.seq_cnt, (const FseE *)F.fse_pool, (const FseE *)c->d_predef, F.o_ll, F.o_ml, F.o_of, F.sizes, st, own_tabs, wave_list);
    const u32 wgrid = n_seq_blk < 8192u ? n_seq_blk : 8192u;
    if (own_tabs && ctx_opt_is(c, "SEQ_WAVE", 'l'))
        LAUNCH(c, "zstd_decode_seq", k_decode_seq_wave, wgrid, 64, 0, d_src, blk, (const u32 *)wave_list, (const i32 *)F.own_ll, (const i32 *)F.own_of, (const i32 *)F.own_ml,
               (const u64 *)F.seq_cnt, (const FseE *)F.fse_pool, (const FseE *)c->d_predef, F.o_ll, F.o_ml, F.o_of, F.sizes, st);
    else if (own_tabs)
        LAUNCH(c, "zstd_decode_seq", k_decode_seq_wave2, wgrid, 64, 0, d_src, blk, (const u32 *)wave_list, (const i32 *)F.own_ll, (const i32 *)F.own_of, (const i32 *)F.own_ml,
               (const u64 *)F.seq_cnt, (const FseE *)F.fse_pool, (const FseE *)c->d_predef, F.o_ll, F.o_ml, F.o_of, F.sizes, st, all_wave | (ctx_opt_is(c, "SEQ_REP", 'w') ? 2u : 0u));
    if (n_seq_blk) LAUNCH(c, "zstd_rep_fast", k_rep_fast, cdiv(n_seq_blk, 256), 256, 0, blk, (const u32 *)F.seq_list, n_seq_blk, st);
    if ((rc = scan_exclusive_u64(c, F.sizes, nblk, F.d_total_out))) return rc;
    if ((rc = ctx_readback(c, &F.hs, st, sizeof F.hs))) return rc;
    return F.hs.err ? zerr(c, F.hs.err, "sequences") : 0;
}
static int range_select(ZFrame &F)
{
    naf_gpu_ctx *c = F.c; int rc; const u32 nblk = F.nblk, n_seq_blk = F.n_seq_blk; ZRange *rg = F.rg; const ZStat &hs = F.hs; u64 *h4 = F.h4;
    F.b_count = nblk; F.seq_t1 = n_seq_blk;
    if (F.fuse) { F.dst = nullptr; F.dst_cap = ~(size_t)0; }
    if (rg) { rg->got_lo = 0; rg->got_hi = hs.total_out; rg->ranged = false; rg->own_buf = nullptr; }
    if (rg && n_seq_blk == 0 && nblk > 0 && rg->want_hi > rg->want_lo) {
        if (!F.lit_only_spec) {
            u64 *r4b = arena_new<u64>(c, 5); if (!r4b) return NAF_GPU_ENOMEM;
            LAUNCH(c, "zstd_find_range", k_find_range, 1, 64, 0, (const u64 *)F.sizes, nblk, (const u64 *)F.d_total_out, rg->want_lo, rg->want_hi, (const i32 *)F.own_huf, r4b);
            if ((rc = ctx_readback(c, h4, r4b, 40))) return rc;
        }
        F.huf_first = (u32)h4[4];
        F.b_first = (u32)h4[0]; F.b_count = (u32)(h4[1] - h4[0]); F.bias = h4[2];
        rg->got_lo = h4[2]; rg->got_hi = h4[3]; rg->ranged = true;
        if (h4[3] - h4[2] > F.dst_cap) return ctx_fail(c, NAF_GPU_ECAP, "zstd range output needs %llu bytes, capacity %zu", (unsigned long long)(h4[3] - h4[2]), F.dst_cap);
        F.dst -= F.bias;
    } else if (rg && n_seq_blk && nblk > 0 && rg->want_hi > rg->want_lo && !ctx_opt_is(c, "RANGE_CLOSURE", '0')) {
        u32 *f = arena_new<u32>(c, nblk); u64 *r4b = arena_new<u64>(c, 5 + 8); if (!f || !r4b) return NAF_GPU_ENOMEM;
        LAUNCH(c, "zstd_find_range", k_find_range, 1, 64, 0, (const u64 *)F.sizes, nblk, (const u64 *)F.d_total_out, rg->want_lo, rg->want_hi, (const i32 *)F.own_huf, r4b);
        LAUNCH(c, "zstd_range_closure", k_iota_u32, F.g, 64, 0, f, nblk);
        LAUNCH(c, "zstd_range_closure", k_seq_reach, cdiv(n_seq_blk, 64), 64, 0, (const ZBlock *)F.blk, (const u32 *)F.seq_list, n_seq_blk, (const u64 *)F.sizes, (const u32 *)F.o_ll, (const u32 *)F.o_ml, (const u32 *)F.o_of, f);
        LAUNCH(c, "zstd_range_closure", k_range_closure, 1, 64, 0, (const u32 *)f, (const u64 *)F.sizes, nblk, (const u64 *)F.d_total_out, (const u64 *)r4b, (const i32 *)F.own_huf, (const u64 *)F.seq_rank, n_seq_blk, r4b + 5);
        u64 h7[7]; if ((rc = ctx_readback(c, h7, r4b + 5, sizeof h7))) return rc;
        const u64 need = h7[3] - h7[2];
        if (ctx_tracing(c)) ctx_trace(c, "[range] want %llu..%llu -> blocks %llu..%llu (bytes %llu..%llu of %llu), tables from %llu, seq blocks %llu..%llu of %u\n", (unsigned long long)rg->want_lo, (unsigned long long)rg->want_hi,
                    (unsigned long long)h7[0], (unsigned long long)h7[1], (unsigned long long)h7[2], (unsigned long long)h7[3], (unsigned long long)hs.total_out, (unsigned long long)h7[4], (unsigned long long)h7[5], (unsigned long long)h7[6], n_seq_blk);
        if (need < hs.total_out) {
            if (need > F.dst_cap) {
                F.dst = (u8 *)arena_alloc(c, need + 64); if (!F.dst) return NAF_GPU_ENOMEM;
                F.dst_cap = need; rg->own_buf = F.dst;
            }
            F.huf_first = (u32)h7[4];
            F.b_first = (u32)h7[0]; F.b_count = (u32)(h7[1] - h7[0]); F.bias = h7[2];
            F.seq_t0 = (u32)h7[5]; F.seq_t1 = (u32)h7[6];
            rg->got_lo = h7[2]; rg->got_hi = h7[3]; rg->ranged = true;
            F.dst -= F.bias;
        } else if (hs.total_out > F.dst_cap) return ctx_fail(c, NAF_GPU_ECAP, "zstd output needs %llu bytes, capacity %zu", (unsigned long long)hs.total_out, F.dst_cap);
    } else if (hs.total_out > F.dst_cap) return ctx_fail(c, NAF_GPU_ECAP, "zstd output needs %llu bytes, capacity %zu", (unsigned long long)hs.total_out, F.dst_cap);
    return 0;
}
static int literals_split(ZFrame &F, const LitPlan &p)
{
    naf_gpu_ctx *c = F.c; int rc; ZSplit *sp = c->zsplit; const u32 nblk = F.nblk;
    if (F.hs.n_plain_huf != nblk) LAUNCH(c, "zstd_copy_fill", k_copy_fill<256>, nblk, 256, 0, F.src, (const ZBlock *)F.blk, nblk, F.dst, F.lit_scratch, 0u, (const u8 *)nullptr);
    if (F.have_ends) for (int k = 0; k + 1 < sp->parts; k++) sp->out_end[k] = F.hends[k];
    else {
        u64 *e2 = arena_new<u64>(c, ZSPLIT_MAX); if (!e2) return NAF_GPU_ENOMEM;
        for (int k = 0; k + 1 < sp->parts; k++) HIP_TRY(c, hipMemcpyAsync(e2 + k, F.sizes + split_part_end(nblk, sp->parts, k), 8, hipMemcpyDeviceToDevice, c->stream));
        if ((rc = ctx_readback(c, sp->out_end, e2, 8 * (size_t)(sp->parts - 1)))) return rc;
    }
    sp->out_end[sp->parts - 1] = F.hs.total_out;
    u32 lo_b = 0;
    for (int k = 0; k < sp->parts; k++) {
        const u32 hi_b = split_part_end(nblk, sp->parts, k);
        if ((rc = launch_literals(c, F, lo_b, hi_b, p))) return rc;
        HIP_TRY(c, hipEventRecord(sp->ev[k], c->stream));
        lo_b = hi_b;
    }
    sp->done = 1;
    return 0;
}
static int literals(ZFrame &F)
// ... 172 lines not shown
```

Baseline: 4257 GB/s.

## Derive flat-emit tile records analytically per span instead of indexing every tile

Result: slower. 4106 GB/s (-3.6%).

```diff
diff --git a/naf_amd/csrc/ctx.h b/naf_amd/csrc/ctx.h
--- a/naf_amd/csrc/ctx.h
+++ b/naf_amd/csrc/ctx.h
@@ -1,5 +1,6 @@
 #pragma once
 #include "common.h"
+#include "emit_span.h"
 #include "../../include/naf_gpu.h"
 #include <hip/hip_runtime.h>
 #include <stdio.h>
@@ -19,7 +20,8 @@
 struct ZFlat { const u8 *src; const FlatStream *si; u64 nslots; const u8 *sym; void *status; bool ready;
                const u8 *tail; u64 tail_q; u32 tail_n;
                const u8 *cls; u32 n_decoded; u32 n_walk;
-               struct naf_gpu_ctx *aux; hipEvent_t decoded_ev; void *later; };
+               struct naf_gpu_ctx *aux; hipEvent_t decoded_ev; void *later;
+               SpanUni uni; };
 struct CtxOpts { std::vector<std::pair<std::string, std::string>> kv; std::string trace; bool tracing = false; };
 struct naf_gpu_ctx {
     int device = 0;
diff --git a/naf_amd/csrc/emit.hip b/naf_amd/csrc/emit.hip
--- a/naf_amd/csrc/emit.hip
+++ b/naf_amd/csrc/emit.hip
@@ -733,17 +733,9 @@
 }
 
 #define EMIT_TOG_LDS 256u
-struct TileIdx { u64 gline, k, khi; u32 col, fast; };
-#define TI_HDR 0xFFFFFFFFu
-struct TileFlat { u64 q0, A, q1, A1, q2, qf; };
-struct TileFlatE { u64 base, a1_addr; u32 a1_sh, K0, K1, d1, d2, qoff, par0, pad; };
-static_assert(sizeof(TileFlatE) == sizeof(TileFlat), "the derived record replaces the raw one in place");
-#define FLAT_QM 4096
 #define TILE_WG 255
-__global__ __launch_bounds__(256) void k_tile_index(EmitP P, u64 ntiles, TileIdx *ti, u64 *tr, u32 *list, u32 *count, TileFlat *tsig, u32 spare, u32 *list2)
-{
-    __shared__ u64 s_k[256], s_r[256];
-    const u64 t = (u64)blockIdx.x * TILE_WG + threadIdx.x;
+__device__ __forceinline__ void tile_index_one(const EmitP &P, u64 ntiles, u64 t, bool behind_only, bool keep_end, TileIdx *ti, u64 *tr, u32 *list, u32 *count, TileFlat *tsig, u32 spare, u32 *list2, u64 *s_k, u64 *s_r)
+{
     const u64 p = P.out_begin + t * 4096;
     TileIdx x; x.fast = 0; x.gline = 0; x.khi = 0; x.k = P.n_toggles; x.col = TI_HDR;
     TileFlat f; f.q0 = f.A = f.q1 = f.A1 = f.q2 = f.qf = 0;
@@ -791,7 +783,7 @@
     }
     s_k[threadIdx.x] = x.k; s_r[threadIdx.x] = r;
     __syncthreads();
-    if (threadIdx.x == TILE_WG) return;
+    if (behind_only && !(keep_end && t == ntiles)) return;
     TileFlatE e; e.base = (u64)P.fsrc; e.a1_addr = (u64)P.fsrc; e.a1_sh = 4; e.K0 = e.K1 = 0; e.d1 = e.d2 = 0x7FFFFFFFu; e.qoff = 0; e.par0 = 0; e.pad = 0;
     if (t >= ntiles) {
         if (t == ntiles) { tr[t] = ~0ull; ti[t] = x; if (tsig && spare) *(TileFlatE *)&tsig[t] = e; }
@@ -833,7 +825,44 @@
     ti[t] = x;
     if (!fast) { if (packed) list2[atomicAdd(count + 1, 1u)] = (u32)t; else list[atomicAdd(count, 1u)] = (u32)t; }
 }
-
+__global__ __launch_bounds__(256) void k_tile_index(EmitP P, u64 ntiles, TileIdx *ti, u64 *tr, u32 *list, u32 *count, TileFlat *tsig, u32 spare, u32 *list2)
+{
+    __shared__ u64 s_k[256], s_r[256];
+    tile_index_one(P, ntiles, (u64)blockIdx.x * TILE_WG + threadIdx.x, threadIdx.x == TILE_WG, false, ti, tr, list, count, tsig, spare, list2, s_k, s_r);
+}
+#define SPAN_LIST_WG 15u
+#define SPAN_LIST_GRID 1024u
+__global__ __launch_bounds__(256) void k_tile_index_spans(EmitP P, u64 ntiles, TileIdx *ti, u64 *tr, u32 *list, u32 *count, TileFlat *tsig, u32 spare, const u32 *slist, const u32 *scnt)
+{
+    __shared__ u64 s_k[256], s_r[256];
+    const u32 n = *scnt, grp = threadIdx.x / (SPAN_TILES + 1), l = threadIdx.x % (SPAN_TILES + 1);
+    for (u32 b = blockIdx.x * SPAN_LIST_WG; b < n; b += gridDim.x * SPAN_LIST_WG) {
+        const bool have = grp < SPAN_LIST_WG && b + grp < n;
+        const u64 t = have ? (u64)slist[b + grp] * SPAN_TILES + l : ~0ull >> 16;
+        tile_index_one(P, ntiles, t, !have || l == SPAN_TILES, true, ti, tr, list, count, tsig, spare, list, s_k, s_r);
+        __syncthreads();
+    }
+}
+
+__global__ __launch_bounds__(256) void k_span_index(EmitP P, SpanUni U, u64 nspans, SpanAnchor *an, u32 *slist, u32 *scnt)
+{
+    const u64 sp = (u64)blockIdx.x * 256 + threadIdx.x;
+    if (sp >= nspans) return;
+    const u64 p = P.out_begin + sp * SPAN_BYTES;
+    const bool seq = P.mode == EM_SEQ;
+    u64 ro = 0, rn = 0, rbase = 0; u32 hl = 0;
+    if (!seq) { const u64 r = upper_bound_u64(P.rec_out, 0, P.N + 1, p) - 1; ro = P.rec_out[r]; rn = P.rec_out[r + 1]; hl = P.hdr_len[r]; rbase = P.rec_base[r]; }
+    SpanAnchor a; u64 g0, gend;
+    bool ok = span_anchor(seq, P.mode == EM_FASTA && P.L != 0, P.L, p, P.out_end, ro, rn, hl, rbase, a, g0, gend);
+    if (ok && P.masking) {
+        const u64 k = upper_bound_u64(P.toggles, 0, P.n_toggles, g0);
+        ok = k == P.n_toggles || P.toggles[k] > gend;
+        if (k & 1) a.flags |= SPAN_MASKED;
+    }
+    if (ok) ok = span_reach_ok(U, g0, P.ftail != nullptr, P.ftail_q);
+    if (ok) a.flags |= SPAN_OK; else { a.flags = 0; slist[atomicAdd(scnt, 1u)] = (u32)sp; }
+    an[sp] = a;
+}
 template <bool FOURBIT>
 __device__ __forceinline__ void emit_tile_body(const EmitP &P, const TileIdx &a, u8 *out_tile)
 {
@@ -1105,32 +1134,11 @@
     }
 }
 
-template <u32 TW>
-__global__ __launch_bounds__(64) void k_emit_tile_flat_wave(EmitP P, const TileIdx *ti, const TileFlat *tsig, u8 *out, u64 ntiles, u32 xcd_chunk)
-{
-    u32 wg = blockIdx.x;
-    if (xcd_chunk) { wg = (blockIdx.x & 7u) * xcd_chunk + (blockIdx.x >> 3); if ((u64)wg * TW >= ntiles) return; }
-    __shared__ u64 s_tog[TW][EMIT_TOG_LDS];
-    __shared__ uint4 s_spl[32];
-    __shared__ u32 s_pair[256];
+template <u32 TW, bool TOG>
+__device__ __forceinline__ void emit_flat_wave_tiles(const EmitP &P, const TileIdx (&A)[TW], const TileFlatE (&F)[TW], const bool (&live)[TW], u64 t0, u8 *out,
+                                                     u64 (*s_tog)[EMIT_TOG_LDS], const uint4 *s_spl, const u32 *s_pair)
+{
     const u32 lane = threadIdx.x;
-    if (lane < 32) s_spl[lane] = ((const uint4 *)(P.fpair + 272))[lane];
-    ((uint4 *)s_pair)[lane] = ((const uint4 *)(P.fpair + 16))[lane];
-    TileIdx A[TW]; TileFlatE F[TW]; bool live[TW];
-    {
-        const u64 t0 = (u64)wg * TW;
-        const uint4 *pa = (const uint4 *)(ti + t0), *pf = (const uint4 *)(tsig + t0);
-        uint4 ra[2 * TW], rf[3 * TW];
-#pragma unroll
-        for (u32 i = 0; i < 2 * TW; i++) ra[i] = pa[i];
-#pragma unroll
-        for (u32 i = 0; i < 3 * TW; i++) rf[i] = pf[i];
-#pragma unroll
-        for (u32 j = 0; j < TW; j++) {
-            __builtin_memcpy(&A[j], &ra[2 * j], 32); __builtin_memcpy(&F[j], &rf[3 * j], 48);
-            live[j] = t0 + j < ntiles && A[j].fast == 1;
-        }
-    }
     u64 X[TW][4]; u32 grels[TW][4], pk[TW][4];
 #pragma unroll
     for (u32 j = 0; j < TW; j++) {
@@ -1160,7 +1168,7 @@
             pk[j][r] = nl_b | ((need > rem ? rem : 16u) << 8) | ((off & 7u) << 16);
         }
     }
-    if (P.masking) {
+    if (TOG && P.masking) {
 #pragma unroll
         for (u32 j = 0; j < TW; j++) {
             const u64 nt = A[j].khi - A[j].k;
@@ -1170,11 +1178,11 @@
     __syncthreads();
 #pragma unroll
     for (u32 j = 0; j < TW; j++) {
-        const u64 t = (u64)wg * TW + j;
+        const u64 t = t0 + j;
         if (!live[j]) continue;
         const TileIdx &a = A[j];
         const u32 ntog = (u32)(a.khi - a.k < EMIT_TOG_LDS ? a.khi - a.k : EMIT_TOG_LDS);
-        const bool use_tog = P.masking && a.k < a.khi && a.khi - a.k <= EMIT_TOG_LDS;
+        const bool use_tog = TOG && P.masking && a.k < a.khi && a.khi - a.k <= EMIT_TOG_LDS;
 #pragma unroll
         for (u32 r = 0; r < 4; r++) {
             const u64 g0 = a.gline + grels[j][r];
@@ -1209,6 +1217,74 @@
             st_text16(out + t * 4096 + (r * 64 + lane) * 16, v, P.nt_store);
         }
     }
+}
+__device__ __forceinline__ void emit_flat_wave_tables(const EmitP &P, uint4 *s_spl, u32 *s_pair)
+{
+    const u32 lane = threadIdx.x;
+    if (lane < 32) s_spl[lane] = ((const uint4 *)(P.fpair + 272))[lane];
+    ((uint4 *)s_pair)[lane] = ((const uint4 *)(P.fpair + 16))[lane];
+}
+template <u32 TW>
+__device__ __forceinline__ void emit_flat_wave_indexed(const EmitP &P, const TileIdx *ti, const TileFlat *tsig, u8 *out, u64 ntiles, u32 wg,
+                                                       u64 (*s_tog)[EMIT_TOG_LDS], const uint4 *s_spl, const u32 *s_pair)
+{
+    TileIdx A[TW]; TileFlatE F[TW]; bool live[TW];
+    {
+        const u64 t0 = (u64)wg * TW;
+        const uint4 *pa = (const uint4 *)(ti + t0), *pf = (const uint4 *)(tsig + t0);
+        uint4 ra[2 * TW], rf[3 * TW];
+#pragma unroll
+        for (u32 i = 0; i < 2 * TW; i++) ra[i] = pa[i];
+#pragma unroll
+        for (u32 i = 0; i < 3 * TW; i++) rf[i] = pf[i];
+#pragma unroll
+        for (u32 j = 0; j < TW; j++) {
+            __builtin_memcpy(&A[j], &ra[2 * j], 32); __builtin_memcpy(&F[j], &rf[3 * j], 48);
+            live[j] = t0 + j < ntiles && A[j].fast == 1;
+        }
+    }
+    emit_flat_wave_tiles<TW, true>(P, A, F, live, (u64)wg * TW, out, s_tog, s_spl, s_pair);
+}
+template <u32 TW>
+__global__ __launch_bounds__(64) void k_emit_tile_flat_wave(EmitP P, const TileIdx *ti, const TileFlat *tsig, u8 *out, u64 ntiles, u32 xcd_chunk)
+{
+    u32 wg = blockIdx.x;
+    if (xcd_chunk) { wg = (blockIdx.x & 7u) * xcd_chunk + (blockIdx.x >> 3); if ((u64)wg * TW >= ntiles) return; }
+    __shared__ u64 s_tog[TW][EMIT_TOG_LDS];
+    __shared__ uint4 s_spl[32];
+    __shared__ u32 s_pair[256];
+    emit_flat_wave_tables(P, s_spl, s_pair);
+    emit_flat_wave_indexed<TW>(P, ti, tsig, out, ntiles, wg, s_tog, s_spl, s_pair);
+}
+__global__ __launch_bounds__(64) void k_emit_tile_flat_wave_spans(EmitP P, const TileIdx *ti, const TileFlat *tsig, u8 *out, u64 ntiles, const u32 *slist, const u32 *scnt)
+{
+    __shared__ u64 s_tog[2][EMIT_TOG_LDS];
+    __shared__ uint4 s_spl[32];
+    __shared__ u32 s_pair[256];
+    emit_flat_wave_tables(P, s_spl, s_pair);
+    const u32 n = *scnt * (SPAN_TILES / 2);
+    for (u32 i = blockIdx.x; i < n; i += gridDim.x) {
+        const u32 wg = slist[i / (SPAN_TILES / 2)] * (SPAN_TILES / 2) + i % (SPAN_TILES / 2);
+        if ((u64)wg * 2 < ntiles) emit_flat_wave_indexed<2>(P, ti, tsig, out, ntiles, wg, s_tog, s_spl, s_pair);
+        __syncthreads();
+    }
+}
+__global__ __launch_bounds__(64) void k_emit_span_flat_wave(EmitP P, SpanUni U, const SpanAnchor *an, u8 *out, u64 ntiles, u32 xcd_chunk)
+{
+    constexpr u32 TW = 2;
+    static_assert(SPAN_TILES % TW == 0, "a wavefront's tiles lie in one span");
+    u32 wg = blockIdx.x;
+    if (xcd_chunk) { wg = (blockIdx.x & 7u) * xcd_chunk + (blockIdx.x >> 3); if ((u64)wg * TW >= ntiles) return; }
+    const SpanAnchor a = an[wg / (SPAN_TILES / TW)];
+    if (!(a.flags & SPAN_OK)) return;
+    __shared__ uint4 s_spl[32];
+    __shared__ u32 s_pair[256];
+    emit_flat_wave_tables(P, s_spl, s_pair);
+    const bool wrap = P.mode == EM_FASTA && P.L != 0;
+    TileIdx A[TW]; TileFlatE F[TW]; bool live[TW];
+#pragma unroll
+    for (u32 j = 0; j < TW; j++) { span_tile(a, U, (u64)P.fsrc, wrap, (u32)P.L, P.Ldiv_magic, (wg % (SPAN_TILES / TW)) * TW + j, A[j], F[j]); live[j] = true; }
+    emit_flat_wave_tiles<TW, false>(P, A, F, live, (u64)wg * TW, out, nullptr, s_spl, s_pair);
 }
 
 template <bool FOURBIT>
@@ -1852,7 +1928,7 @@
             else LAUNCH(c, "unnaf_emit", k_emit<false>, grid, 256, 0, pl.P, d_out);
         } else {
             u64 ntiles = cdiv(m_end - m_begin, 4096);
-            TileIdx *ti = arena_new<TileIdx>(c, ntiles + 2 + FLAT_TPW); u64 *tr = arena_new<u64>(c, ntiles + 2);
+            TileIdx *ti = arena_new<TileIdx>(c, ntiles + 2 + SPAN_TILES); u64 *tr = arena_new<u64>(c, ntiles + 2);
             u32 *list = arena_new<u32>(c, ntiles + 1), *cnt = arena_new<u32>(c, 2);
             u32 *list2 = (zflat.ready && zflat.cls) ? arena_new<u32>(c, ntiles + 1) : list;
             if (!ti || !tr || !list || !cnt || !list2) return NAF_GPU_ENOMEM;
@@ -1869,60 +1945,85 @@
             if (split.done) HIP_TRY(c, hipMemsetAsync(cnt, 0, 8, ic->stream));
             TileFlat *tsig = nullptr;
             if (zflat.ready) {
-                tsig = arena_new<TileFlat>(c, ntiles + 2 + FLAT_TPW); u32 *fpair = arena_new<u32>(c, 400); if (!tsig || !fpair) return NAF_GPU_ENOMEM;
+                tsig = arena_new<TileFlat>(c, ntiles + 2 + SPAN_TILES); u32 *fpair = arena_new<u32>(c, 400); if (!tsig || !fpair) return NAF_GPU_ENOMEM;
                 LAUNCH(ic, "unnaf_flat_pair", k_flat_pair, 1, 256, 0, pl.P, fpair);
                 pl.P.fpair = fpair;
             }
-            LAUNCH(ic, "unnaf_tile_index", k_tile_index, cdiv(ntiles + 1 + FLAT_TPW, TILE_WG), 256, 0, pl.P, ntiles, ti, tr, list, cnt, tsig, (u32)FLAT_TPW, list2);
-            naf_gpu_ctx *xc = c;
-            const bool flat_job = zflat.ready && zflat.later;
-            if (zflat.ready && zflat.aux) {
-                HIP_TRY(c, hipEventRecord(c->split_ev[0], c->stream));
-                if (!flat_job) { HIP_TRY(c, hipStreamWaitEvent(zflat.aux->stream, c->split_ev[0], 0)); xc = zflat.aux; }
-            }
-            u64 t_done = 0;
-            if (split.done) {
-                HIP_TRY(c, hipEventRecord(c->split_ev[ZSPLIT_MAX], ic->stream));
-                for (int k = 0; k + 1 < split.parts; k++) {
-                    u64 bases_ready = split.out_end[k] * (pl.fourbit ? 2u : 1u);
-                    u64 t_hi = bases_ready / 4096; t_hi = t_hi > 1 ? t_hi - 1 : 0;
-                    if (t_hi > ntiles) t_hi = ntiles;
-                    if (t_hi <= t_done) continue;
-                    HIP_TRY(c, hipStreamWaitEvent(ic->stream, split.ev[k], 0));
-                    emit_tiles(ic, t_done, t_hi);
-                    t_done = t_hi;
+            static_assert(SPAN_TILES >= FLAT_TPW, "spare records");
+            const u64 nspans = (ntiles + SPAN_TILES - 1) / SPAN_TILES;
+            const bool use_span = zflat.ready && !zflat.cls && !zflat.later && zflat.uni.ok && emit_wave && !split.done &&
+                                  (pl.P.mode == EM_FASTA || pl.P.mode == EM_SEQ) && (!pl.P.masking || pl.P.n_toggles < nspans) && !ctx_opt_is(c, "EMIT_SPAN", '0');
+            if (use_span) {
+                SpanAnchor *an = arena_new<SpanAnchor>(c, nspans); u32 *slist = arena_new<u32>(c, nspans + 1), *scnt = arena_new<u32>(c, 1);
+                if (!an || !slist || !scnt) return NAF_GPU_ENOMEM;
+                HIP_TRY(c, hipMemsetAsync(scnt, 0, 4, c->stream));
+                LAUNCH(c, "unnaf_span_index", k_span_index, cdiv(nspans, 256), 256, 0, pl.P, zflat.uni, nspans, an, slist, scnt);
+                const u32 lgrid = (u32)(nspans < SPAN_LIST_GRID ? nspans : SPAN_LIST_GRID);
+                LAUNCH(c, "unnaf_tile_index", k_tile_index_spans, lgrid, 256, 0, pl.P, ntiles, ti, tr, list, cnt, tsig, (u32)SPAN_TILES, (const u32 *)slist, (const u32 *)scnt);
+                naf_gpu_ctx *xc = c;
+                if (zflat.aux) { HIP_TRY(c, hipEventRecord(c->split_ev[0], c->stream)); HIP_TRY(c, hipStreamWaitEvent(zflat.aux->stream, c->split_ev[0], 0)); xc = zflat.aux; }
+                const u32 ch = (cdiv(ntiles, 2u) + 7) / 8;
+                LAUNCH(c, "unnaf_emit_flat", k_emit_span_flat_wave, ch * 8, 64, 0, pl.P, zflat.uni, (const SpanAnchor *)an, d_out, (u64)ntiles, ch);
+                LAUNCH(xc, "unnaf_emit_flat_listed", k_emit_tile_flat_wave_spans, lgrid * (SPAN_TILES / 2), 64, 0, pl.P, (const TileIdx *)ti, (const TileFlat *)tsig, d_out, (u64)ntiles, (const u32 *)slist, (const u32 *)scnt);
+                const u32 rest_grid = 4u * (u32)(ntiles < EMIT_REST_GRID ? ntiles : EMIT_REST_GRID);
+                LAUNCH(xc, "unnaf_emit_rest", k_emit_rest<true>, rest_grid, 64, 0, pl.P, (const TileIdx *)ti, (const u64 *)tr, (const u32 *)list, (const u32 *)cnt, d_out);
+                if (xc != c) { HIP_TRY(c, hipEventRecord(c->split_ev[1], xc->stream)); HIP_TRY(c, hipStreamWaitEvent(c->stream, c->split_ev[1], 0)); }
+                if (ctx_tracing(c)) {
+                    u32 hc[2] = { 0, 0 }, hs = 0;
+                    if (!ctx_readback2(c, hc, cnt, 8, &hs, scnt, 4)) ctx_trace(c, "[flat tiles] total %llu rest %u decoded %u spans %llu listed %u\n", (unsigned long long)ntiles, hc[0], hc[1], (unsigned long long)nspans, hs);
                 }
-                HIP_TRY(c, hipEventRecord(c->split_ev[ZSPLIT_MAX + 1], ic->stream));
-                HIP_TRY(c, hipStreamWaitEvent(c->stream, c->split_ev[ZSPLIT_MAX], 0));
-            }
-            if (zflat.ready) {
-                const u32 nwg = cdiv(ntiles, 4u), chunk = (nwg + 7) / 8;
-                const bool mixed = flat_job || (zflat.cls && zflat.n_decoded);
-                const bool wave = emit_wave && (!mixed || zflat.n_walk == 0);
-                if (wave && pl.P.masking && pl.P.n_toggles >= ntiles) { const u32 ch = ((u32)ntiles + 7) / 8; LAUNCH(c, "unnaf_emit_flat", k_emit_tile_flat_wave<1>, ch * 8, 64, 0, pl.P, (const TileIdx *)ti, (const TileFlat *)tsig, d_out, (u64)ntiles, ch); }
-                else if (wave) { const u32 ch = (cdiv(ntiles, 2u) + 7) / 8; LAUNCH(c, "unnaf_emit_flat", k_emit_tile_flat_wave<2>, ch * 8, 64, 0, pl.P, (const TileIdx *)ti, (const TileFlat *)tsig, d_out, (u64)ntiles, ch); }
-                else
-                LAUNCH(c, "unnaf_emit_flat", k_emit_tile_flat<4>, chunk * 8, 256, 0, pl.P, (const TileIdx *)ti, (const TileFlat *)tsig, d_out, (u64)ntiles, chunk);
-                if (flat_job) {
-                    if ((rc = zstd_flat_later(c, &zflat))) return rc;
-                    if (zflat.aux) xc = zflat.aux;
+            } else {
+                LAUNCH(ic, "unnaf_tile_index", k_tile_index, cdiv(ntiles + 1 + FLAT_TPW, TILE_WG), 256, 0, pl.P, ntiles, ti, tr, list, cnt, tsig, (u32)FLAT_TPW, list2);
+                naf_gpu_ctx *xc = c;
+                const bool flat_job = zflat.ready && zflat.later;
+                if (zflat.ready && zflat.aux) {
+                    HIP_TRY(c, hipEventRecord(c->split_ev[0], c->stream));
+                    if (!flat_job) { HIP_TRY(c, hipStreamWaitEvent(zflat.aux->stream, c->split_ev[0], 0)); xc = zflat.aux; }
                 }
-                if (zflat.cls && zflat.n_decoded) {
-                    const u64 est = (u64)zflat.n_decoded * 64 + 64;
-                    const u32 lgrid = (u32)(est < ntiles ? (est < 16384 ? est : 16384) : (ntiles < 16384 ? ntiles : 16384));
-                    if (wave) LAUNCH(xc, "unnaf_emit", k_emit_tile_list_wave<true>, lgrid, 64, 0, pl.P, (const TileIdx *)ti, (const u32 *)list2, (const u32 *)(cnt + 1), d_out);
-                    else LAUNCH(xc, "unnaf_emit", k_emit_tile_list<true>, lgrid, 256, 0, pl.P, (const TileIdx *)ti, (const u32 *)list2, (const u32 *)(cnt + 1), d_out);
+                u64 t_done = 0;
+                if (split.done) {
+                    HIP_TRY(c, hipEventRecord(c->split_ev[ZSPLIT_MAX], ic->stream));
+                    for (int k = 0; k + 1 < split.parts; k++) {
+                        u64 bases_ready = split.out_end[k] * (pl.fourbit ? 2u : 1u);
+                        u64 t_hi = bases_ready / 4096; t_hi = t_hi > 1 ? t_hi - 1 : 0;
+                        if (t_hi > ntiles) t_hi = ntiles;
+                        if (t_hi <= t_done) continue;
+                        HIP_TRY(c, hipStreamWaitEvent(ic->stream, split.ev[k], 0));
+                        emit_tiles(ic, t_done, t_hi);
+                        t_done = t_hi;
+                    }
+                    HIP_TRY(c, hipEventRecord(c->split_ev[ZSPLIT_MAX + 1], ic->stream));
+                    HIP_TRY(c, hipStreamWaitEvent(c->stream, c->split_ev[ZSPLIT_MAX], 0));
                 }
-            }
-            else if (t_done < ntiles) emit_tiles(c, t_done, ntiles);
-            const u32 rest_grid = 4u * (u32)(ntiles < EMIT_REST_GRID ? ntiles : EMIT_REST_GRID);
-            if (pl.fourbit) LAUNCH(xc, "unnaf_emit_rest", k_emit_rest<true>, rest_grid, 64, 0, pl.P, (const TileIdx *)ti, (const u64 *)tr, (const u32 *)list, (const u32 *)cnt, d_out);
-            else LAUNCH(xc, "unnaf_emit_rest", k_emit_rest<false>, rest_grid, 64, 0, pl.P, (const TileIdx *)ti, (const u64 *)tr, (const u32 *)list, (const u32 *)cnt, d_out);
-            if (xc != c) { HIP_TRY(c, hipEventRecord(c->split_ev[1], xc->stream)); HIP_TRY(c, hipStreamWaitEvent(c->stream, c->split_ev[1], 0)); }
-            if (split.done) HIP_TRY(c, hipStreamWaitEvent(c->stream, c->split_ev[ZSPLIT_MAX + 1], 0));
-            if (zflat.ready && ctx_tracing(c)) {
-                u32 hc[2] = { 0, 0 };
-                if (!ctx_readback(c, hc, cnt, 8)) ctx_trace(c, "[flat tiles] total %llu rest %u decoded %u\n", (unsigned long long)ntiles, hc[0], hc[1]);
+                if (zflat.ready) {
+                    const u32 nwg = cdiv(ntiles, 4u), chunk = (nwg + 7) / 8;
+                    const bool mixed = flat_job || (zflat.cls && zflat.n_decoded);
+                    const bool wave = emit_wave && (!mixed || zflat.n_walk == 0);
+                    if (wave && pl.P.masking && pl.P.n_toggles >= ntiles) { const u32 ch = ((u32)ntiles + 7) / 8; LAUNCH(c, "unnaf_emit_flat", k_emit_tile_flat_wave<1>, ch * 8, 64, 0, pl.P, (const TileIdx *)ti, (const TileFlat *)tsig, d_out, (u64)ntiles, ch); }
+                    else if (wave) { const u32 ch = (cdiv(ntiles, 2u) + 7) / 8; LAUNCH(c, "unnaf_emit_flat", k_emit_tile_flat_wave<2>, ch * 8, 64, 0, pl.P, (const TileIdx *)ti, (const TileFlat *)tsig, d_out, (u64)ntiles, ch); }
+                    else
+                    LAUNCH(c, "unnaf_emit_flat", k_emit_tile_flat<4>, chunk * 8, 256, 0, pl.P, (const TileIdx *)ti, (const TileFlat *)tsig, d_out, (u64)ntiles, chunk);
+                    if (flat_job) {
+                        if ((rc = zstd_flat_later(c, &zflat))) return rc;
+                        if (zflat.aux) xc = zflat.aux;
+                    }
+                    if (zflat.cls && zflat.n_decoded) {
+                        const u64 est = (u64)zflat.n_decoded * 64 + 64;
+                        const u32 lgrid = (u32)(est < ntiles ? (est < 16384 ? est : 16384) : (ntiles < 16384 ? ntiles : 16384));
+                        if (wave) LAUNCH(xc, "unnaf_emit", k_emit_tile_list_wave<true>, lgrid, 64, 0, pl.P, (const TileIdx *)ti, (const u32 *)list2, (const u32 *)(cnt + 1), d_out);
+                        else LAUNCH(xc, "unnaf_emit", k_emit_tile_list<true>, lgrid, 256, 0, pl.P, (const TileIdx *)ti, (const u32 *)list2, (const u32 *)(cnt + 1), d_out);
+                    }
+                }
+                else if (t_done < ntiles) emit_tiles(c, t_done, ntiles);
+                const u32 rest_grid = 4u * (u32)(ntiles < EMIT_REST_GRID ? ntiles : EMIT_REST_GRID);
+                if (pl.fourbit) LAUNCH(xc, "unnaf_emit_rest", k_emit_rest<true>, rest_grid, 64, 0, pl.P, (const TileIdx *)ti, (const u64 *)tr, (const u32 *)list, (const u32 *)cnt, d_out);
+                else LAUNCH(xc, "unnaf_emit_rest", k_emit_rest<false>, rest_grid, 64, 0, pl.P, (const TileIdx *)ti, (const u64 *)tr, (const u32 *)list, (const u32 *)cnt, d_out);
+                if (xc != c) { HIP_TRY(c, hipEventRecord(c->split_ev[1], xc->stream)); HIP_TRY(c, hipStreamWaitEvent(c->stream, c->split_ev[1], 0)); }
+                if (split.done) HIP_TRY(c, hipStreamWaitEvent(c->stream, c->split_ev[ZSPLIT_MAX + 1], 0));
+                if (zflat.ready && ctx_tracing(c)) {
+                    u32 hc[2] = { 0, 0 };
+                    if (!ctx_readback(c, hc, cnt, 8)) ctx_trace(c, "[flat tiles] total %llu rest %u decoded %u spans 0 listed 0\n", (unsigned long long)ntiles, hc[0], hc[1]);
+                }
             }
         }
     }
diff --git a/naf_amd/csrc/emit_span.h b/naf_amd/csrc/emit_span.h
--- /dev/null
+++ b/naf_amd/csrc/emit_span.h
@@ -0,0 +1,90 @@
+#pragma once
+#include "common.h"
+
+struct TileIdx { u64 gline, k, khi; u32 col, fast; };
+#define TI_HDR 0xFFFFFFFFu
+struct TileFlat { u64 q0, A, q1, A1, q2, qf; };
+struct TileFlatE { u64 base, a1_addr; u32 a1_sh, K0, K1, d1, d2, qoff, par0, pad; };
+static_assert(sizeof(TileFlatE) == sizeof(TileFlat), "the derived record replaces the raw one in place");
+#define FLAT_QM 4096
+
+#define SPAN_TILES 16u
+#define SPAN_BYTES (SPAN_TILES * 4096u)
+#define SPAN_LP1_MAX 32768u
+struct SpanAnchor { u64 gline; u32 col, flags; };
+#define SPAN_OK 1u
+#define SPAN_MASKED 2u
+static_assert(sizeof(SpanAnchor) == 16, "read with one 16-byte scalar load");
+struct SpanUni {
+    u64 C0;
+    u32 cs[4];
+    i32 dA[4];
+    u32 S, np, lgper, ok;
+};
+NAF_HD SpanUni span_uni_make(u64 off0, u32 S, u32 np, u32 regen0, u32 nstreams0, u32 per, u32 hso0, const u32 off[4], const u32 n[4])
+{
+    SpanUni U; memset(&U, 0, sizeof U);
+    if (nstreams0 != 4 || per < 4096 || per > (1u << 20) || (per & (per - 1)) || regen0 != 4 * per || S >= (1u << 24) || np < 1) return U;
+    for (u32 s = 0; s < 4; s++) if (n[s] != per || off[s] >= (1u << 24)) return U;
+    U.lgper = 0; while ((1u << U.lgper) < per) U.lgper++;
+    U.C0 = 8 * (off0 + 3 + hso0 + off[0]) + 4ull * per;
+    for (u32 s = 0; s < 4; s++) U.cs[s] = 8 * (off[s] - off[0]);
+    for (u32 s = 0; s < 3; s++) U.dA[s] = (i32)(U.cs[s + 1] - U.cs[s]);
+    U.dA[3] = (i32)(8 * S) - (i32)U.cs[3];
+    U.S = S; U.np = np; U.ok = 1;
+    return U;
+}
+NAF_HD u32 span_umulhi(u32 a, u32 b)
+{
+#if defined(__HIP_DEVICE_COMPILE__)
+    return __umulhi(a, b);
+#else
+    return (u32)(((u64)a * b) >> 32);
+#endif
+}
+NAF_HD u32 span_div_magic(u32 Lp1) { return (Lp1 >= 2 && Lp1 < SPAN_LP1_MAX) ? (u32)((1ull << 32) / Lp1 + 1) : 0; }
+NAF_HD bool span_reach_ok(const SpanUni &U, u64 g0, bool has_tail, u64 tail_q)
+{
+    const u64 qe = (g0 >> 1) + 2048ull * (SPAN_TILES - 1) + 2048 + 16;
+    if (has_tail && qe >= tail_q) return false;
+    return U.ok && (qe >> U.lgper) + 2 < 4ull * U.np;
+}
+NAF_HD bool span_wrap_ok(bool wrap, u64 L) { return !wrap || (L >= 16 && L + 1 < SPAN_LP1_MAX); }
+NAF_HD bool span_anchor(bool seq_mode, bool wrap, u64 L, u64 p, u64 out_end, u64 ro, u64 rn, u32 hl, u64 rbase, SpanAnchor &a, u64 &g0, u64 &gend)
+{
+    a.gline = 0; a.col = 0; a.flags = 0; g0 = gend = 0;
+    const u64 pe = p + SPAN_BYTES;
+    if (pe >= out_end || !span_wrap_ok(wrap, L)) return false;
+    if (seq_mode) { a.gline = g0 = p; gend = pe; return true; }
+    if (p < ro + hl || pe >= rn) return false;
+    const u64 q = p - ro - hl;
+    if (wrap) {
+        const u64 line = q / (L + 1), col = q - line * (L + 1), qe = q + SPAN_BYTES, linee = qe / (L + 1), cole = qe - linee * (L + 1);
+        a.gline = rbase + line * L; a.col = (u32)col;
+        g0 = a.gline + (col < L ? col : L); gend = rbase + linee * L + (cole < L ? cole : L);
+    } else { a.gline = g0 = rbase + q; gend = g0 + SPAN_BYTES; }
+    return true;
+}
+NAF_HD void span_tile(const SpanAnchor &an, const SpanUni &U, u64 fsrc, bool wrap, u32 L, u32 magic, u32 i, TileIdx &x, TileFlatE &e)
+{
+    u64 gline = an.gline, g; u32 col = 0;
+    if (wrap) {
+        const u32 c = an.col + 4096u * i, dl = span_umulhi(c, magic);
+        col = c - dl * (L + 1);
+        gline += (u64)dl * L;
+        g = gline + (col < L ? col : L);
+    } else { gline += 4096u * i; g = gline; }
+    x.gline = gline; x.col = col; x.fast = 1; x.k = x.khi = (an.flags & SPAN_MASKED) ? 1 : 0;
+    const u64 qf = g >> 1;
+    const u32 per = 1u << U.lgper, pos = (u32)qf & (per - 1), s = (u32)(qf >> U.lgper) & 3u, bi = (u32)(qf >> (U.lgper + 2));
+    const u64 A = 8 * ((u64)bi * U.S) + U.C0 + U.cs[s];
+    const i32 dA = U.dA[s], d = dA + (i32)(4 * per);
+    const u64 T0 = A - 4ull * pos;
+    const u64 ub = (T0 + (u64)(i64)(d < 0 ? d : 0) - 40 - 4ull * FLAT_QM) & ~7ull;
+    e.base = fsrc + (u64)((i64)ub >> 3);
+    e.K0 = (u32)(T0 - 40 - ub); e.K1 = e.K0 + (u32)d;
+    e.d1 = per - pos; e.d2 = 2 * per - pos;
+    e.qoff = (u32)((gline >> 1) - qf); e.par0 = (u32)gline & 1u;
+    const u64 t1 = A + (u64)(i64)dA - 40;
+    e.a1_addr = fsrc + (t1 >> 3); e.a1_sh = (u32)(t1 & 7) + 4; e.pad = 0;
+}
diff --git a/naf_amd/csrc/zstd_dec.hip b/naf_amd/csrc/zstd_dec.hip
--- a/naf_amd/csrc/zstd_dec.hip
+++ b/naf_amd/csrc/zstd_dec.hip
@@ -3412,9 +3412,10 @@
 static u32 split_part_end(u32 n, int parts, int k) { return k + 1 == parts ? n : (u32)((u64)n * (k + 1) / parts) & ~(HUF_BLOCKS_PER_WG - 1u); }
 
 struct FlatMixed { const u8 *cls; u32 n_decoded, n_walk; void *later; };
-static int flat_handoff(const ZFrame &F, const FlatStream *si, u64 nslots, const u8 *sym, u64 end_off, u64 total_out, u32 last_raw, const FlatMixed *mixed)
+static int flat_handoff(const ZFrame &F, const FlatStream *si, u64 nslots, const u8 *sym, u64 end_off, u64 total_out, u32 last_raw, const FlatMixed *mixed, const SpanUni *uni = nullptr)
 {
     naf_gpu_ctx *c = F.c; ZFlat *zf = c->zflat;
+    if (uni) zf->uni = *uni;
     if (mixed) { zf->cls = mixed->cls; zf->n_decoded = mixed->n_decoded; zf->n_walk = mixed->n_walk; zf->decoded_ev = nullptr; zf->later = mixed->later; }
     const size_t frame_end = end_off + (F.fh.checksum ? 4 : 0);
     if (frame_end > F.src_len) return zerr(c, ZE_TRUNC, "checksum");
@@ -3493,7 +3494,10 @@
     if (rc) return rc;
     if (ctx_tracing(c)) ctx_trace(c, "[stride] len %zu S %u nmax %u prefix %u verdict %u err %u nblk %u\n", src_len, S, nmax, res2[0], res2[1], hs.err, hs.nblk);
     if (ctx_tracing(c) && U) ctx_trace(c, "[uniform?] ok %u bad %u prefix %u blocks %u huffman %u regen %u total %llu\n", hu.ok, hu.bad, hu.np, hu.nblk, hu.nhb, hu.regen0, (unsigned long long)hu.total_out);
-    if (res2[1] == 1u && !hs.err && hs.nblk && hu.ok && !hu.bad) return flat_handoff(F, usi, 4ull * hu.nhb, usym, hs.end_off, hu.total_out, hu.last_raw, nullptr);
+    if (res2[1] == 1u && !hs.err && hs.nblk && hu.ok && !hu.bad) {
+        const SpanUni su = span_uni_make(fh.hdr_size, S, hu.np, hu.regen0, hu.nstreams0, hu.per, hu.hso0, hu.off, hu.n);
+        return flat_handoff(F, usi, 4ull * hu.nhb, usym, hs.end_off, hu.total_out, hu.last_raw, nullptr, &su);
+    }
     if (res2[1] == 1u && !hs.err && hs.nblk) F.blk = sblk;
     if (res2[1] == 2u && !hs.err && F.uni_wanted && !ctx_opt_is(c, "STRIDE_RUNS", '0')) return index_stride_runs(F, S, h0, nmax, sres);
     return 0;
```
